# bytedance/DeepSolid

Measured on AMD Instinct MI355X. Metric: local-energy evals/sec, higher is better.
Workload: dtype f64; 1 GPU; bcc_li 24 e- (12,12), total_energy primal (E_kin forward-Laplacian + Ewald), default detnet ((256,32),)*3, 8 dets; batch_per_gpu=4096, global_batch=4096, parallelism=walker-dp1

## Files before the change

deepsolid_amd/_lib.py:

```python
import ctypes as C
import os

_HERE = os.path.dirname(os.path.abspath(__file__))
LIB_PATH = os.environ.get('DEEPSOLID_HIP_LIB') or os.path.join(_HERE, 'libdeepsolid_hip.so')

DS_MAX_LAYERS = 8
DS_MAX_SYM = 6
_PD = C.POINTER(C.c_double)


class SystemDesc(C.Structure):
    _fields_ = [
        ('dtype', C.c_int32), ('n_up', C.c_int32), ('n_dn', C.c_int32), ('n_atoms_prim', C.c_int32),
        ('prim_atoms', _PD), ('prim_a', C.c_double * 9), ('sim_a', C.c_double * 9), ('n_sym', C.c_int32),
        ('prim_AV', C.c_double * (DS_MAX_SYM * 3)), ('prim_BV', C.c_double * (DS_MAX_SYM * 3)),
        ('sim_AV', C.c_double * (DS_MAX_SYM * 3)), ('sim_BV', C.c_double * (DS_MAX_SYM * 3)),
        ('n_layers', C.c_int32), ('hidden_single', C.c_int32 * DS_MAX_LAYERS),
        ('hidden_double', C.c_int32 * DS_MAX_LAYERS), ('n_det', C.c_int32), ('distance_type', C.c_int32),
        ('envelope_type', C.c_int32), ('full_det', C.c_int32), ('use_last_layer', C.c_int32),
        ('bias_orbitals', C.c_int32), ('klist_up', _PD), ('klist_dn', _PD),
        ('n_atoms_sim', C.c_int32), ('sim_atoms', _PD), ('sim_charges', _PD), ('dist_mode', C.c_int32),
        ('n_g', C.c_int32), ('gpoints', _PD), ('gweight', _PD), ('ion_exp_re', _PD), ('ion_exp_im', _PD),
        ('ewald_alpha', C.c_double), ('ee_const', C.c_double), ('ei_const', C.c_double), ('ii_total', C.c_double),
    ]


class ParamBlock(C.Structure):
    _fields_ = [('offset', C.c_int64), ('rows', C.c_int32), ('cols', C.c_int32)]


class KfacBlock(C.Structure):
    _fields_ = [('kind', C.c_int32), ('index', C.c_int32), ('n_param_blocks', C.c_int32), ('param_blocks', C.c_int32 * 3),
                ('has_bias', C.c_int32), ('d_in', C.c_int32), ('d_out', C.c_int32), ('repeats', C.c_int32),
                ('a_offset', C.c_int64), ('g_offset', C.c_int64)]


class HfDesc(C.Structure):
    _PI = C.POINTER(C.c_int32)
    _fields_ = [
        ('a', C.c_double * 9), ('n_atoms', C.c_int32), ('atoms', _PD), ('n_shells', C.c_int32), ('shell_atom', _PI),
        ('shell_l', _PI), ('shell_nprim', _PI), ('exps', _PD), ('coefs', _PD), ('n_k', C.c_int32), ('kpts', _PD),
        ('n_images', C.c_int32), ('images', _PD), ('n_up', C.c_int32), ('n_dn', C.c_int32), ('nocc_up', _PI), ('nocc_dn', _PI),
        ('mo_up', _PD), ('mo_dn', _PD),
    ]


class EcpDesc(C.Structure):
    _PI = C.POINTER(C.c_int32)
    _fields_ = [
        ('a', C.c_double * 9), ('n_atoms', C.c_int32), ('atoms', _PD), ('atom_species', _PI), ('n_species', C.c_int32),
        ('n_l', _PI), ('r_cut_loc', _PD), ('r_cut_nl', _PD), ('term_offset', _PI), ('term_n', _PI), ('term_zeta', _PD),
        ('term_c', _PD), ('n_quad', C.c_int32),
    ]


_VP = C.c_void_p
SIGNATURES = {
    'ds_device_widths': (C.c_int, [C.POINTER(C.c_int32), C.POINTER(C.c_int32), C.c_int32, C.c_int32, C.c_int32, C.c_int32,
                                   C.POINTER(C.c_int32), C.POINTER(C.c_int32), C.POINTER(C.c_int32), C.POINTER(C.c_int32)]),
    'ds_system_create': (C.c_int, [C.POINTER(SystemDesc), C.POINTER(_VP)]),
    'ds_system_destroy': (None, [_VP]),
    'ds_last_error': (C.c_char_p, []),
    'ds_param_count': (C.c_int64, [_VP]),
    'ds_int8_layers': (C.c_int, [_VP]),
    'ds_param_layout': (C.c_int, [_VP, C.POINTER(ParamBlock), C.c_int]),
    'ds_workspace_bytes': (C.c_int64, [_VP, C.c_int64]),
    'ds_logpsi': (C.c_int, [_VP, _VP, _VP, C.c_int64, _VP, _VP, _VP, C.c_int64, _VP]),
    'ds_logpsi_grad': (C.c_int, [_VP, _VP, _VP, C.c_int64, _VP, _VP, _VP, _VP, C.c_int64, _VP]),
    'ds_vjp_workspace_bytes': (C.c_int64, [_VP, C.c_int64]),
    'ds_logpsi_vjp': (C.c_int, [_VP, _VP, _VP, C.c_int64, _VP, _VP, _VP, _VP, _VP, C.c_int64, _VP]),
    'ds_pretrain_workspace_bytes': (C.c_int64, [_VP, C.c_int64]),
    'ds_pretrain_loss_vjp': (C.c_int, [_VP, _VP, _VP, C.c_int64, _VP, _VP, _VP, _VP, _VP, C.c_int64, _VP]),
    'ds_kfac_block_count': (C.c_int, [_VP]),
    'ds_kfac_layout': (C.c_int, [_VP, C.POINTER(KfacBlock), C.c_int]),
    'ds_kfac_workspace_bytes': (C.c_int64, [_VP, C.c_int64]),
    'ds_kfac_factors': (C.c_int, [_VP, _VP, _VP, C.c_int64, _VP, _VP, _VP, C.c_int64, _VP]),
    'ds_kfac_step_workspace_bytes': (C.c_int64, [_VP]),
    'ds_kfac_inverses': (C.c_int, [_VP, _VP, C.c_double, C.c_double, _VP, _VP, C.c_int64, _VP]),
    'ds_kfac_precondition': (C.c_int, [_VP, _VP, _VP, _VP, _VP, _VP, C.c_int64, _VP]),
    'ds_kfac_inverses_sized_workspace_bytes': (C.c_int64, [C.c_int, C.POINTER(C.c_int32), C.POINTER(C.c_int32)]),
    'ds_kfac_inverses_sized': (C.c_int, [C.c_int, C.c_int, C.POINTER(C.c_int32), C.POINTER(C.c_int32), C.POINTER(C.c_int32), _VP,
                                        C.c_double, C.c_double, _VP, _VP, C.c_int64, _VP]),
    'ds_orbitals': (C.c_int, [_VP, _VP, _VP, C.c_int64, _VP, _VP, _VP, C.c_int64, _VP]),
    'ds_ewald': (C.c_int, [_VP, _VP, C.c_int64, _VP, _VP]),
    'ds_local_energy': (C.c_int, [_VP, _VP, _VP, C.c_int64, _VP, _VP, _VP, _VP, _VP, C.c_int64, _VP]),
    'ds_enforce_pbc': (C.c_int, [_PD, C.c_int, _VP, C.c_int64, _VP, _VP, _VP]),
    'ds_observables_workspace_bytes': (C.c_int64, [C.c_int64, C.c_int]),
    'ds_observables': (C.c_int, [_PD, C.c_int, _VP, C.c_int64, C.c_int64, C.POINTER(C.c_int32), C.c_int, C.c_int, _VP, _VP,
                                 C.c_int64, _VP]),
    'ds_realspace_counts': (C.c_int, [_PD, C.POINTER(C.c_int32), _PD, _PD, C.c_double, C.c_int, C.c_int, _VP, C.c_int64, C.c_int64,
                                      C.c_int64, _VP, _VP, _VP]),
    'ds_mh_propose': (C.c_int, [_VP, _VP, _VP, C.c_double, C.c_int64, _VP, _VP]),
    'ds_mh_accept': (C.c_int, [_VP, _VP, _VP, _VP, _VP, _VP, C.c_int64, _VP, _VP]),
    'ds_mh_propose_ex': (C.c_int, [_VP, C.c_int, _VP, _VP, C.c_double, _VP, C.c_int, C.c_int64, _VP, _VP, _VP]),
    'ds_mh_accept_ex': (C.c_int, [_VP, C.c_int, _VP, _VP, _VP, _VP, _VP, _VP, C.c_double, _VP, _VP, C.c_int, C.c_int64, _VP, _VP, _VP]),
    'ds_mcmc_workspace_bytes': (C.c_int64, [_VP, C.c_int64]),
    'ds_mcmc_step': (C.c_int, [_VP, _VP, _VP, _VP, C.c_int64, C.c_int, C.c_double, C.c_uint64, C.c_uint64, _VP, _VP, C.c_int, _VP, _VP,
                              C.c_int64, _VP]),
    'ds_mcmc_step_one_electron': (C.c_int, [_VP, _VP, _VP, _VP, C.c_int64, C.c_int, C.c_int, C.c_double, C.c_uint64, C.c_uint64, _VP, _VP,
                                           C.c_int, _VP, _VP, C.c_int64, _VP]),
    'ds_mcmc_step_importance': (C.c_int, [_VP, _VP, _VP, _VP, C.c_int64, C.c_int, C.c_double, C.c_uint64, C.c_uint64, _VP, _VP, C.c_int,
                                         _VP, _VP, C.c_int64, _VP]),
    'ds_mcmc_step_asymmetric': (C.c_int, [_VP, _VP, _VP, _VP, C.c_int64, C.c_int, C.c_double, _VP, C.c_int, C.c_uint64, C.c_uint64, _VP, _VP,
                                         C.c_int, _VP, _VP, C.c_int64, _VP]),
    'ds_one_body_workspace_bytes': (C.c_int64, [_VP, C.c_int64, C.c_int]),
    'ds_one_body_ratios': (C.c_int, [_VP, _VP, _VP, C.c_int64, C.c_int, C.c_int, C.c_uint64, C.c_uint64, _VP, _VP, C.c_int, _VP, _VP, _VP,
                                     _VP, _VP, C.c_int64, _VP]),
    'ds_spin_exchange_workspace_bytes': (C.c_int64, [_VP, C.c_int64, C.c_int]),
    'ds_spin_exchange_ratios': (C.c_int, [_VP, _VP, _VP, C.c_int64, C.c_int, C.c_int, _VP, _VP, _VP, _VP, _VP, C.c_int64, _VP]),
    'ds_ecp_create': (C.c_int, [C.POINTER(EcpDesc), C.POINTER(_VP)]),
    'ds_ecp_destroy': (None, [_VP]),
    'ds_ecp_workspace_bytes': (C.c_int64, [_VP, _VP, C.c_int64, C.c_int64]),
    'ds_ecp_energy': (C.c_int, [_VP, _VP, _VP, _VP, C.c_int64, C.c_uint64, C.c_uint64, _VP, C.c_int64, _VP, _VP, _VP, _VP, _VP,
                               C.c_int64, _VP]),
    'ds_dmc_workspace_bytes': (C.c_int64, [_VP, C.c_int64]),
    'ds_dmc_step': (C.c_int, [_VP, _VP, _VP, _VP, _VP, _VP, _VP, _VP, C.c_int64, C.c_int, C.c_double, C.c_double, C.c_double, C.c_double,
                             C.c_double, C.c_int, C.c_int, C.c_uint64, C.c_uint64, _VP, _VP, _VP, C.c_int, _VP, _VP, _VP, C.c_int64, _VP]),
    'ds_dmc_noise': (C.c_int, [C.c_int, C.c_int, C.c_int64, C.c_int, C.c_uint64, C.c_uint64, _VP, _VP, _VP, _VP]),
    'ds_dmc_branch_workspace_bytes':(C.c_int64, [C.c_int, C.c_int, C.c_int64]),
    'ds_dmc_branch': (C.c_int, [C.c_int, C.c_int, C.c_int64, C.c_double, _VP, _VP, _VP, _VP, _VP, _VP, _VP, _VP, C.c_int64, _VP]),
    'ds_philox_host': (None,[C.c_uint64, C.c_uint64, C.c_uint64, C.c_uint64, C.c_int, C.POINTER(C.c_uint32)]),
    'ds_energy_stats': (C.c_int, [_VP, _VP, _VP, C.c_int64, _VP, _VP]),
    'ds_debug_stage': (C.c_int64, [_VP, _VP, _VP, C.c_int64, C.c_char_p, _VP, C.c_int64, _VP, C.c_int64, _VP]),
    'ds_profile_enable': (C.c_int, [_VP, C.c_int]),
    'ds_profile_read': (C.c_int, [_VP, C.POINTER(C.c_double), C.POINTER(C.c_int64)]),
    'ds_profile_read_clock': (C.c_int, [_VP, C.POINTER(C.c_double), C.POINTER(C.c_double)]),
    'ds_debug_timeline': (C.c_int, [_VP, C.POINTER(C.c_uint64), C.c_int]),
    'ds_calib_copy': (C.c_int, [_VP, _VP, C.c_int64, _VP]),
    'ds_mfma_f64_peak': (C.c_int64, [C.c_int64, C.c_int, C.c_int, _VP, _VP]),
    'ds_hf_create': (C.c_int, [C.POINTER(HfDesc), C.POINTER(_VP)]),
    'ds_hf_destroy': (None, [_VP]),
    'ds_hf_orbitals': (C.c_int, [_VP, C.c_int, _VP, C.c_int64, _VP, _VP, _VP]),
}

PROF_KINDS = ('features', 'm2_expand', 'two_layer', 'single_first', 'single_hidden', 'orbital', 'det_inverse',
              'det_trace', 'combine', 'ewald', 'shared_term', 'single_lr')

_lib = None


def load():
    global _lib
    if _lib is not None:
        return _lib
    if not os.path.exists(LIB_PATH):
        raise RuntimeError(
            f'{LIB_PATH} is missing: the HIP extension is not built and deepsolid_amd has no CPU '
            'fallback.  Run `make -C deepsolid_amd/csrc` (hipcc, --offload-arch=gfx950).')
    lib = C.CDLL(LIB_PATH)
    for name, (res, args) in SIGNATURES.items():
        fn = getattr(lib, name)
        fn.restype = res
        fn.argtypes = args
    _lib = lib
    return lib


def check(rc, what):
    if rc != 0:
        msg = load().ds_last_error()
        raise RuntimeError(f'{what} failed: {msg.decode() if msg else rc}')
```

deepsolid_amd/csrc/ds_api.hip:

```cpp
#include <cstdarg>

#include "ds_host.h"
#include "ds_tiles.h"

namespace ds {
#define DS_DECL(p) const TileOps<double>* tile_ops_f64_p##p(int); const TileOps<float>* tile_ops_f32_p##p(int);
DS_DECL(0) DS_DECL(1) DS_DECL(2) DS_DECL(3) DS_DECL(4)
#undef DS_DECL
template <> const TileOps<double>* tile_ops<double>(int st) {
    const TileOps<double>* (*parts[])(int) = {tile_ops_f64_p0, tile_ops_f64_p1, tile_ops_f64_p2, tile_ops_f64_p3, tile_ops_f64_p4};
    for (auto f : parts)
        if (const TileOps<double>* o = f(st)) return o;
    return nullptr;
}
template <> const TileOps<float>* tile_ops<float>(int st) {
    const TileOps<float>* (*parts[])(int) = {tile_ops_f32_p0, tile_ops_f32_p1, tile_ops_f32_p2, tile_ops_f32_p3, tile_ops_f32_p4};
    for (auto f : parts)
        if (const TileOps<float>* o = f(st)) return o;
    return nullptr;
}
}

namespace ds {
namespace host {
// ... 186 lines not shown
    for (int c = 0; c < 2; ++c) {
        const size_t n = c < S.n_detch ? S.det_n[c] : 0;
        v.mout_off[c] = mo;
        mo += (size_t)S.K * n * n * 2 * PV;
    }
    v.MOUT = mo; v.MINV = 0; v.TR = 0;
    v.DETS = w.DETS * PV;
    v.PARTM = (size_t)(PV / 5) * h2max * 5 * (S.NP / 16) * ds::PM_SLOTS;
    v.per_walker = measure([&](Arena<double>& a) { carve_value<double>(s, a, 1); });
}

int plan_widths(const int32_t* hs, const int32_t* hd, int n_layers, int n_in_single, int n_in_double, int n_double, int32_t* ps,
                int32_t* pd, int32_t* rs, int32_t* rd) {
    if (n_layers < 1 || n_layers > DS_MAX_LAYERS) return fail("bad n_layers");
    for (int l = 0; l < n_layers; ++l) {
        const int a = hs[l], b = hd[l];
        if (a < 1 || a > 1024) return fail("hidden_single: one-electron widths are supported in 1..1024 (layer %d: %d)", l, a);
        if (l < n_double && (b < 1 || b > 32)) return fail("hidden_double: pair-stream widths are supported in 1..32 (layer %d: %d)", l, b);
        ps[l] = rup(a, 64);
        pd[l] = (b >= 1 && b <= 16) ? 16 : 32;
        rs[l] = a == (l == 0 ? n_in_single : hs[l - 1]);
        rd[l] = l < n_double && b == (l == 0 ? n_in_double : hd[l - 1]);
    }
    return 0;
}

int check_arch(const ds_system_desc* d) {
    if (d->dtype != 0 && d->dtype != 1) return fail("dtype must be 0 (f64) or 1 (f32)");
    if (d->distance_type != 0 && d->distance_type != 1) return fail("Unrecognized distance function.");
    if (d->distance_type == 1 && d->envelope_type != 0) return fail("the 'tri' features support the isotropic envelope only");
    if (d->envelope_type < 0 || d->envelope_type > 2) return fail("unknown envelope_type");
    if (d->n_up < 0 || d->n_dn < 0) return fail("n_up and n_dn must be >= 0");
    if (d->n_up < 1) return fail("internal: n_up must be >= 1 here (ds_system_create swaps a spin-down-only cell)");
    if (d->n_layers < 1 || d->n_layers > DS_MAX_LAYERS) return fail("bad n_layers");
    if (d->n_det < 1 || d->n_det > DS_MAX_DETS) return fail("n_det must be in 1..%d", DS_MAX_DETS);
    if (d->n_sym < 3 || d->n_sym > DS_MAX_SYM) return fail("bad n_sym");
    const int N = d->n_up + d->n_dn, tiles = (3 * N + 2 + 15) / 16, nmat = d->full_det ? N : std::max(d->n_up, d->n_dn);
    if (nmat > 64) return fail("determinant matrices larger than 64 x 64 are not supported (n = %d): the trace kernels keep a matrix row per lane group", nmat);
    if (tiles < 1 || tiles > ds::DS_MAX_TILES)
        return fail("no kernel instance for %d jet-slot tiles (N = %d electrons): supported are N <= 128 (64 with full_det)", tiles, N);
    const int n_double = d->use_last_layer ? d->n_layers : d->n_layers - 1;
    const int nch = d->n_dn > 0 ? 2 : 1;
    for (int l = 0; l < d->n_layers; ++l) {
        if (d->hidden_single[l] % 64 || d->hidden_single[l] < 64 || d->hidden_single[l] > 1024)
            return fail("internal: device width %d of layer %d is not a multiple of 64 in 64..1024", d->hidden_single[l], l);
        if (l < n_double && d->hidden_double[l] != 16 && d->hidden_double[l] != 32)
            return fail("internal: device pair width %d of layer %d is not 16 or 32", d->hidden_double[l], l);
    }
    const int k_orb = d->hidden_single[d->n_layers - 1] + (d->use_last_layer ? nch * d->hidden_double[d->n_layers - 1] : 0);
    if (k_orb % 16) return fail("orbital head with K = %d input rows: the GEMM's operand ring needs K %% 16 == 0", k_orb);
    return 0;
}

template <typename T>
void enforce_pbc(const double* latvec, const double* inv, const void* x, int64_t n_elec, void* out_x, void* out_wrap, hipStream_t st) {
    ds::Lattice<T> L;
    for (int i = 0; i < 9; ++i) { L.a[i] = (T)latvec[i]; L.ainv[i] = (T)inv[i]; }
    hipLaunchKernelGGL((ds::k_enforce_pbc<T>), dim3((unsigned)((n_elec + 255) / 256)), dim3(256), 0, st, L, (const T*)x, (size_t)n_elec, (T*)out_x,
                       (T*)out_wrap);
}

}

void set_last_error(const char* msg) { host::g_err = msg; }

}

using namespace ds::host;

extern "C" {

const char* ds_last_error(void) { return g_err.c_str(); }

int ds_device_widths(const int32_t* hidden_single, const int32_t* hidden_double, int32_t n_layers, int32_t n_in_single, int32_t n_in_double,
                     int32_t n_double, int32_t* dev_single, int32_t* dev_double, int32_t* res_single, int32_t* res_double) {
    if (!hidden_single || !hidden_double || !dev_single || !dev_double || !res_single || !res_double) return fail("null argument");
    return plan_widths(hidden_single, hidden_double, n_layers, n_in_single, n_in_double, n_double, dev_single, dev_double, res_single, res_double);
}

int ds_system_create(const ds_system_desc* ref_desc, ds_system** out) {
    if (!ref_desc || !out) return fail("null argument");
    ds_system_desc dev_desc = *ref_desc;
    int32_t rs[DS_MAX_LAYERS] = {0}, rd[DS_MAX_LAYERS] = {0};
    {
        if (ref_desc->distance_type != 0 && ref_desc->distance_type != 1) return fail("Unrecognized distance function.");
        if (ref_desc->n_layers < 1 || ref_desc->n_layers > DS_MAX_LAYERS) return fail("bad n_layers");
        const int nf = ref_desc->distance_type == 0 ? 4 : 7;
        const int n_double = ref_desc->use_last_layer ? ref_desc->n_layers : ref_desc->n_layers - 1;
        if (int rc = plan_widths(ref_desc->hidden_single, ref_desc->hidden_double, ref_desc->n_layers, nf * ref_desc->n_atoms_prim, nf, n_double,
                                 dev_desc.hidden_single, dev_desc.hidden_double, rs, rd))
            return rc;
    }
    if (dev_desc.n_up == 0 && dev_desc.n_dn > 0) {
        dev_desc.n_up = dev_desc.n_dn;
        dev_desc.n_dn = 0;
        dev_desc.klist_up = dev_desc.klist_dn;
        dev_desc.klist_dn = nullptr;
    }
    if (dev_desc.n_up + dev_desc.n_dn < 1) return fail("n_up + n_dn must be >= 1");
    const ds_system_desc* desc = &dev_desc;
    if (int rc = check_arch(desc)) return rc;
    if (!desc->prim_atoms || !desc->klist_up || (desc->n_dn > 0 && !desc->klist_dn) || !desc->sim_atoms || !desc->sim_charges ||
        (desc->n_g > 0 && (!desc->gpoints || !desc->gweight || !desc->ion_exp_re || !desc->ion_exp_im)))
        return fail("null array pointer in ds_system_desc");
    ds_system* s = new ds_system();
    s->d = *desc;
    for (int l = 0; l < desc->n_layers; ++l) {
        s->ref_single[l] = ref_desc->hidden_single[l];
        s->ref_double[l] = ref_desc->hidden_double[l];
        s->res1[l] = rs[l] != 0;
        s->res2[l] = rd[l] != 0;
    }
    s->dtype = desc->dtype;
    s->use_last = desc->use_last_layer != 0;
    std::vector<double> h64;
    std::vector<float> h32;
    fill_tables<double>(s, desc, s->sd, h64);
    fill_tables<float>(s, desc, s->sf, h32);
    if (hipMalloc(&s->blob64, h64.size() * sizeof(double)) != hipSuccess || hipMalloc(&s->blob32, h32.size() * sizeof(float)) != hipSuccess) {
        delete s;
        return fail("hipMalloc of the system tables failed (is a GPU visible?)");
    }
    if (hipMemcpy(s->blob64, h64.data(), h64.size() * sizeof(double), hipMemcpyHostToDevice) != hipSuccess ||
        hipMemcpy(s->blob32, h32.data(), h32.size() * sizeof(float), hipMemcpyHostToDevice) != hipSuccess) {
        ds_system_destroy(s);
        return fail("upload of the system tables failed");
    }
    relocate<double>(s->sd, (const double*)s->blob64);
    relocate<float>(s->sf, (const float*)s->blob32);
    build_layouts(s);
    {
        int h1max = 0;
        for (int l = 0; l <= s->sd.n_layers; ++l) h1max = std::max(h1max, s->sd.h1[l]);
        if (hipMalloc(&s->lr_w0t, (size_t)h1max * 64 * sizeof(double)) != hipSuccess) {
            ds_system_destroy(s);
            return fail("hipMalloc of the low-rank layer's weight table failed");
        }
    }
    {
        hipDeviceProp_t prop;
        int devid = 0;
        if (hipGetDevice(&devid) == hipSuccess && hipGetDeviceProperties(&prop, devid) == hipSuccess && prop.multiProcessorCount > 0)
            s->n_cu = prop.multiProcessorCount;
    }
    if (hipMalloc((void**)&s->clk_dev, 1024 * sizeof(unsigned long long)) != hipSuccess ||
        hipMemset(s->clk_dev, 0, 1024 * sizeof(unsigned long long)) != hipSuccess) {
        ds_system_destroy(s);
        return fail("hipMalloc of the clock-probe counters failed");
    }
    s->det_valu = getenv("DS_DET_VALU") != nullptr;
    if (const char* e = getenv("DS_VAL_NB")) { const int v = atoi(e); s->val_nb = (v == 1 || v == 2 || v == 4) ? v : 0; }
    s->no_lu_wave = getenv("DS_NO_LU_WAVE") != nullptr;
    s->use_lr = getenv("DS_NO_LOWRANK") == nullptr;
    s->use_pm_skip = getenv("DS_NO_PM_SKIP") == nullptr;
    s->use_pair_expand = getenv("DS_NO_PAIR_EXPAND") == nullptr;
    s->use_g4 = getenv("DS_NO_G4") == nullptr;
    s->use_i8 = getenv("DS_I8") != nullptr && getenv("DS_NO_I8") == nullptr;
    s->use_ldsb = getenv("DS_NO_LDSB") == nullptr;
    s->use_pair_fuse = getenv("DS_NO_PAIR_FUSE") == nullptr;
    s->use_i8_val = getenv("DS_NO_I8_VAL") == nullptr;
    for (int l = 0; l < DS_MAX_LAYERS; ++l) s->i8_prepped[l] = ~(uint64_t)0;
    if (const char* e = getenv("DS_I8_VAL_MIN_TILES")) s->val_i8_min_tiles = atoll(e);
    if (const char* e = getenv("DS_DBG")) s->dbg = atoi(e);
    s->use_wide = getenv("DS_NO_WIDE") == nullptr;
    s->wide_all = getenv("DS_WIDE_ALL") != nullptr;
    {
        const size_t bytes = i8_planes_bytes(s);
        if (bytes && hipMalloc(&s->i8_wp, bytes) != hipSuccess) {
            ds_system_destroy(s);
            return fail("hipMalloc of the int8 layer's weight planes failed");
        }
    }
    if (const char* e = getenv("DS_CHUNK_WALKERS")) s->chunk_cap = std::min<int64_t>(65535, std::max<int64_t>(1, atol(e)));
    *out = s;
    return 0;
}

void ds_system_destroy(ds_system* s) {
    if (!s) return;
    if (s->clk_dev) (void)hipFree(s->clk_dev);
    if (s->lr_w0t) (void)hipFree(s->lr_w0t);
    if (s->i8_wp) (void)hipFree(s->i8_wp);
    if (s->blob64) (void)hipFree(s->blob64);
    if (s->blob32) (void)hipFree(s->blob32);
    delete s;
}

int64_t ds_param_count(const ds_system* s) { return s ? s->nparams : -1; }

int ds_param_layout(const ds_system* s, ds_param_block* blocks, int max_blocks) {
    if (!s) return -1;
    const int n = (int)s->blocks.size();
    for (int i = 0; i < n && i < max_blocks; ++i) blocks[i] = s->blocks[i];
    return n;
}

int64_t ds_workspace_bytes(const ds_system* s, int64_t B) {
    if (!s) return -1;
    const int64_t esz = s->dtype == 0 ? 8 : 4;
    const int64_t budget = workspace_budget();
    const int64_t cap = s->chunk_cap;
    int64_t chunk = std::min<int64_t>(std::max<int64_t>(B, 1), cap);
    chunk = std::max<int64_t>(1, std::min<int64_t>(chunk, budget / ((int64_t)s->ws.per_walker * esz)));
    const int64_t groups = groups_per_pass(B, esz, PassSize{0, s->wsv.per_walker}, budget);
    return std::max((int64_t)s->ws.per_walker * esz * chunk, (int64_t)s->wsv.per_walker * esz * groups) + 256;
}

int ds_enforce_pbc(const double* latvec, int dtype, const void* x, int64_t n_elec, void* out_x, void* out_wrap, void* stream) {
    if (!latvec || !x || !out_x) return fail("null argument");
    if (n_elec <= 0) return 0;
    hipStream_t st = (hipStream_t)stream;
    double inv[9];
    inv3(latvec, inv);
    if (dtype != 0 && dtype != 1) return fail("dtype must be 0 or 1");
    DS_BY_DTYPE(dtype, enforce_pbc, latvec, inv, x, n_elec, out_x, out_wrap, st);
    HIP_OK(hipGetLastError());
    return 0;
}

int ds_profile_enable(ds_system* s, int on) {
    if (!s) return fail("null argument");
    for (auto& v : s->prof_ev) {
        for (auto& p : v) { s->prof_pool.push_back(p.first); s->prof_pool.push_back(p.second); }
        v.clear();
    }
    s->prof_on = on != 0;
    s->prof_only = on >= 2 ? on - 2 : -1;
    if (on) HIP_OK(hipMemset(s->clk_dev, 0, 1024 * sizeof(unsigned long long)));
    return 0;
}

int ds_debug_timeline(ds_system* s, uint64_t* out, int n) {
    if (!s || !out || n < 0 || n > 1022) return fail("bad argument");
    HIP_OK(hipDeviceSynchronize());
    HIP_OK(hipMemcpy(out, s->clk_dev + 2, (size_t)n * sizeof(uint64_t), hipMemcpyDeviceToHost));
    return 0;
}

int ds_profile_read_clock(ds_system* s, double* shader_cycles, double* ref_ticks) {
    if (!s || !shader_cycles || !ref_ticks) return fail("null argument");
    unsigned long long h[2] = {0, 0};
    HIP_OK(hipDeviceSynchronize());
    HIP_OK(hipMemcpy(h, s->clk_dev, sizeof h, hipMemcpyDeviceToHost));
    *shader_cycles = (double)h[0];
    *ref_ticks = (double)h[1];
    return 0;
}

int ds_profile_read(ds_system* s, double* ms_total, int64_t* launches) {
    if (!s || !ms_total || !launches) return fail("null argument");
    if (s->prof_failed) { s->prof_failed = false; return fail("profiling: a HIP event could not be created or recorded; the timings are incomplete"); }
    for (int k = 0; k < DS_PROF_KINDS; ++k) {
        double tot = 0;
        for (auto& p : s->prof_ev[k]) {
            HIP_OK(hipEventSynchronize(p.second));
            float ms = 0;
            HIP_OK(hipEventElapsedTime(&ms, p.first, p.second));
            tot += ms;
        }
        ms_total[k] = tot;
        launches[k] = (int64_t)s->prof_ev[k].size();
    }
    return 0;
}

int ds_calib_copy(const void* src, void* dst, int64_t n_elems, void* stream) {
    if (!src || !dst) return fail("null argument");
    hipLaunchKernelGGL(ds::k_calib_copy, dim3(256 * 8), dim3(256), 0, (hipStream_t)stream, (const double*)src, (double*)dst, (size_t)n_elems);
    HIP_OK(hipGetLastError());
    return 0;
}

int64_t ds_mfma_f64_peak(int64_t iters, int blocks_per_cu, int n_acc, void* scratch, void* stream) {
    const int blocks = 256 * blocks_per_cu;
    hipStream_t st = (hipStream_t)stream;
    switch (n_acc) {
        case 1: hipLaunchKernelGGL(ds::k_mfma_peak<1>, dim3(blocks), dim3(256), 0, st, (long)iters, (double*)scratch); break;
        case 2: hipLaunchKernelGGL(ds::k_mfma_peak<2>, dim3(blocks), dim3(256), 0, st, (long)iters, (double*)scratch); break;
        case 4: hipLaunchKernelGGL(ds::k_mfma_peak<4>, dim3(blocks), dim3(256), 0, st, (long)iters, (double*)scratch); break;
        case 8: hipLaunchKernelGGL(ds::k_mfma_peak<8>, dim3(blocks), dim3(256), 0, st, (long)iters, (double*)scratch); break;
        case 16: hipLaunchKernelGGL(ds::k_mfma_peak<16>, dim3(blocks), dim3(256), 0, st, (long)iters, (double*)scratch); break;
        default: fail("n_acc must be 1, 2, 4, 8 or 16"); return -1;
    }
    return (int64_t)blocks * 4 * iters * n_acc * 2048;
}

}
```

deepsolid_amd/csrc/ds_chain.hip:

```cpp
#include "ds_host.h"
#include "ds_tiles.h"

namespace ds {
namespace host {

template <typename T> inline unsigned m2_split(int K2, int N) {
    unsigned z = 1;
    while (z < 8 && K2 % (2 * z) == 0 && (size_t)(K2 / z) * 5 * N * sizeof(T) > 8192) z *= 2;
    return z;
}

enum Stop { STOP_NONE = 0, STOP_G0, STOP_G1, STOP_G2, STOP_G3, STOP_H2_0, STOP_H2_1, STOP_H2_2, STOP_MEAN0, STOP_Q,
            STOP_MOUT, STOP_MINV, STOP_DETS, STOP_TR };

template <typename T> struct DumpReq { int stop; T* out; int64_t cap; int64_t written; };

template <typename T>
int copy_out(DumpReq<T>* dr, const T* src, size_t n, hipStream_t st) {
    size_t m = std::min<size_t>(n, (size_t)dr->cap);
    HIP_OK(hipMemcpyAsync(dr->out, src, m * sizeof(T), hipMemcpyDeviceToDevice, st));
    dr->written = (int64_t)m;
    return 0;
}

enum class LayerKind {
    Dense,
    DenseRes,
    L0Stats,
    L0Epi9Means,
    LowRank1,
    Int8
};
struct PairPlan {
    bool res, res_sep;
    bool expand;
    bool write_out;
    unsigned xz; int EW, NW; size_t xlds;
};
struct LayerPlan {
    LayerKind kind;
    bool res_sep;
    bool wide;
    bool pm_mask;
    bool pm_unwritten;
    int prof_kind;
    PairPlan pair;
};
enum class OrbKind { Orb3, Wide, Ldsb, Gemm };
template <typename T> struct ChainPlan {
    const ds::TileOps<T>* to;
    bool lr_on;
    int lr_nc;
    int g4;
    LayerPlan layer[DS_MAX_LAYERS];
    OrbKind orb[2];
    int count(LayerKind k, int n_layers) const {
        int n = 0;
        for (int l = 0; l < n_layers; ++l) n += layer[l].kind == k ? 1 : 0;
        return n;
    }
};

template <typename T>
int plan_chain(const ds_system* s, bool dump, ChainPlan<T>* p) {
    const ds::SysDev<double>& S = s->sd;
    const ds::TileOps<T>* to = p->to = ds::tile_ops<T>(S.P / 16);
    if (!to) return fail("no kernel instance for %d slot tiles (N = %d electrons)", S.P / 16, S.N);
    const int ST = to->ST;
    const bool wide = s->use_wide && to->gemm_wide != nullptr;
    auto gemm_wide = [&](int epi) { return wide && (s->wide_all || ds::gemm_wide_faster<T>(epi)); };
    const int K0loc = S.h1[0] + S.nch * S.h2[0], K0sh = S.nch * S.h1[0];
    p->lr_nc = std::max(2, (K0loc + K0sh + 4 + 15) / 16);
    p->lr_on = !dump && s->use_lr && S.n_layers >= 2 && !s->res1[0] && p->lr_nc <= 4 && S.h1[1] % 16 == 0 && (S.nch * S.h2[1]) % 4 == 0 &&
               3 * (K0loc + K0sh + 4) <= S.h1[1] && p->lr_nc * S.h1[1] < (S.h1[1] - K0loc - K0sh - 4) * ST;
    const int used = S.D - 16 * (ST - 1);
    p->g4 = !s->use_g4 ? 0 : (ST == 5 && used > 8 && used <= 12) ? 3 : (ST == 10 && used <= 4) ? 1 : 0;
    for (int l = 0; l < S.n_layers; ++l) {
        const int Kh = S.h1[l], K2 = S.h2[l], Nout = S.h1[l + 1], Kloc = Kh + S.nch * K2;
        LayerPlan& lp = p->layer[l];
        lp = LayerPlan{};
        if (Nout % 64 || Nout > 1024) return fail("hidden_single must be a multiple of 64 and <= 1024 (got %d)", Nout);
        if (l < S.n_double) {
            PairPlan& pp = lp.pair;
            const int K2o = S.h2[l + 1];
            if (K2o != 32 && K2o != 16) return fail("hidden_double must be 16 or 32 (got %d)", K2o);
            if (K2 % 4) return fail("pair-stream width %d is not a multiple of 4", K2);
            pp.res_sep = s->res2[l] && l == 0;
            pp.res = s->res2[l] && !pp.res_sep;
            pp.xz = (!pp.res && K2o == 32) ? 2 : 1;
            pp.write_out = l + 1 < S.n_double || s->use_last;
            pp.EW = (pp.write_out && S.N % 16 == 8 && pp.xz == 2) ? 2 : 1;
            pp.NW = (pp.EW * S.N + 15) / 16;
            pp.xlds = ((size_t)(K2o / pp.xz) * 5 * pp.EW * S.N + (size_t)pp.EW * S.nch * (K2o / pp.xz) * 5) * sizeof(T);
            pp.expand = !dump && s->use_pair_expand && !pp.res_sep && l + 1 < S.n_layers && pp.NW <= 8 && pp.xlds <= 150 * 1024;
        }
        const bool res = s->res1[l];
        lp.res_sep = res && l == 0 && (Kloc % 16 != 0 || S.nf * S.A != Nout);
        if (res && !lp.res_sep && Kloc % 16) return fail("residual layer with K = %d: the GEMM's operand ring needs K %% 16 == 0", Kloc);
        if (p->lr_on && l == 1) {
            lp.kind = LayerKind::LowRank1;
            lp.wide = wide && (s->wide_all || ds::lr_wide_faster<T>(p->lr_nc));
        } else if (p->lr_on && l == 0) {
            const bool one_kernel = to->layer0_stats && ds::layer0_stats_instance(ST, K0loc / 4);
            lp.kind = one_kernel ? LayerKind::L0Stats : LayerKind::L0Epi9Means;
            lp.wide = !one_kernel && gemm_wide(9);
        } else if (int8_energy_layer(s, l)) {
            lp.kind = LayerKind::Int8;
        } else if (res && !lp.res_sep) {
            lp.kind = LayerKind::DenseRes;
            lp.wide = gemm_wide(2);
        } else {
            lp.kind = LayerKind::Dense;
            lp.wide = gemm_wide(1);
        }
        lp.prof_kind = l == 0 ? DS_PROF_SINGLE_FIRST : (lp.kind == LayerKind::LowRank1 ? DS_PROF_SINGLE_LR : DS_PROF_SINGLE_HIDDEN);
        lp.pm_mask = s->use_pm_skip && (l == 0 || (lp.kind == LayerKind::DenseRes && Kh % 16 == 0 && K2 % 16 == 0));
        lp.pm_unwritten = !dump && l >= 1 && !lp.wide &&
                          (lp.kind == LayerKind::LowRank1 ? s->use_pm_skip : (lp.pm_mask && ds::pm_instance<T>(ST)));
    }
    const int Korb = S.h1[S.n_layers] + (s->use_last ? S.nch * S.h2[S.n_layers] : 0);
    if (Korb % 16) return fail("orbital head with K = %d: the GEMM's operand ring needs K %% 16 == 0", Korb);
    for (int sp = 0; sp < S.nch; ++sp) {
        const int OC = S.ocols[sp];
        if (to->gemm_orb3 && OC % 256 != 0 && OC % 192 == 0) p->orb[sp] = OrbKind::Orb3;
        else if (gemm_wide(5)) p->orb[sp] = OrbKind::Wide;
        else if (to->orbital_lb && s->use_ldsb && OC % 64 == 0) p->orb[sp] = OrbKind::Ldsb;
        else p->orb[sp] = OrbKind::Gemm;
    }
    return 0;
}

template <typename T>
int run_chain(ds_system* s, const T* params, const T* x, int64_t Bc, Arena<T> ws, hipStream_t st, T* out_ke, T* out_logabs,
              T* out_phase, DumpReq<T>* dr, T* out_grad = nullptr) {
    const ds::SysDev<T>& S = dev<T>(s);
    const WsLayout& L = s->ws;
    const Carve<T> c = carve<T>(s, ws, Bc);
    if (!ws.ok) return carve_fail("forward-Laplacian chain");
    auto blk = [&](int i) { return params + s->blocks[i].offset; };
    const int stop = dr ? dr->stop : STOP_NONE;
    ChainPlan<T> plan;
    if (int rc = plan_chain<T>(s, dr != nullptr, &plan)) return rc;
    const ds::TileOps<T>* to = plan.to;
    const int NB = to->NB, ST = to->ST, lr_nc = plan.lr_nc;
    const bool lr_on = plan.lr_on;
    const int K0loc = S.h1[0] + S.nch * S.h2[0], K0sh = S.nch * S.h1[0];
    {
        ProfScope ps(s, DS_PROF_FEATURES, st);
        size_t sh = (size_t)(9 * S.N) * sizeof(T) + (size_t)S.N * S.A * S.nf * sizeof(ds::Jet5<T>);
        hipLaunchKernelGGL((ds::k_features<T>), dim3((unsigned)Bc), dim3(256), sh, st, S, x, blk(s->i_pi[0]), blk(s->i_sg[0]),
                           blk(s->i_pi[S.nch - 1]), blk(s->i_sg[S.nch - 1]), lr_on ? c.XL : c.G[0], lr_on ? K0loc : S.ldk, c.MEAN[0], c.H2[0], c.Q);
    }
    if (lr_on) {
        const int n = S.h1[1] * 16 * lr_nc;
        hipLaunchKernelGGL((ds::k_lr_w0t<T>), dim3((unsigned)((n + 255) / 256)), dim3(256), 0, st, blk(s->i_wloc[0]), blk(s->i_wsh[0]), K0loc, K0sh,
                           S.h1[1], 16 * lr_nc, (T*)s->lr_w0t);
    }
    if (stop == STOP_MEAN0) return copy_out(dr, c.MEAN[0], (size_t)S.nch * S.h1[0] * S.P * Bc, st);
    if (stop == STOP_H2_0) return copy_out(dr, c.H2[0], (size_t)S.h2[0] * 5 * S.NP * Bc, st);
    if (stop == STOP_Q) return copy_out(dr, c.Q, L.Q * Bc, st);
    int gi = 0, hi = 0;
    for (int l = 0; l < S.n_layers; ++l) {
        const LayerPlan& lp = plan.layer[l];
        const int Kh = S.h1[l], K2 = S.h2[l], Nout = S.h1[l + 1];
        if (!(l > 0 && plan.layer[l - 1].pair.expand)) {
            ProfScope ps(s, DS_PROF_M2_EXPAND, st);
            const bool xl = lr_on && l == 0;
            hipLaunchKernelGGL((ds::k_m2_expand<T>), dim3(S.N, (unsigned)Bc, m2_split<T>(K2, S.N)), dim3(256), (size_t)(K2 * 5 * S.N + S.nch * K2 * 5) / m2_split<T>(K2, S.N) * sizeof(T), st, S,
                               c.H2[hi], K2, xl ? c.XL : c.G[gi], Kh, xl ? K0loc : S.ldk, lp.pm_unwritten ? 1 : 0);
        }
        if (stop == STOP_G0 + l) return copy_out(dr, c.G[gi], L.G * Bc, st);
        if (l < S.n_double) {
            const PairPlan& pp = lp.pair;
            const int K2o = S.h2[l + 1];
            const T* W2 = blk(s->i_w2[l]); const T* b2 = blk(s->i_b2[l]);
            ProfScope ps(s, DS_PROF_TWO_LAYER, st);
            if (pp.expand) {
#define DS_TWOX(NT2, RES) hipLaunchKernelGGL((ds::k_two_layer_expand<T, NT2, RES>), dim3(S.N / pp.EW, (unsigned)Bc, pp.xz), dim3(64 * pp.NW), pp.xlds, st, S, c.H2[hi], K2, W2, b2, \
                                             pp.write_out ? c.H2[hi ^ 1] : (T*)nullptr, c.G[gi ^ 1], S.h1[l + 1], S.ldk, plan.layer[l + 1].pm_unwritten ? 1 : 0, pp.EW)
                if (K2o == 32 && pp.res) DS_TWOX(2, true);
                else if (pp.res) DS_TWOX(1, true);
                else DS_TWOX(1, false);
#undef DS_TWOX
            } else {
                const dim3 grid((S.NP / 16 + 3) / 4, (unsigned)Bc);
#define DS_TWO(NT2, RES) hipLaunchKernelGGL((ds::k_two_layer<T, NT2, RES, false>), grid, dim3(256), 0, st, S, c.H2[hi], K2, W2, b2, c.H2[hi ^ 1])
                if (K2o == 32) { if (pp.res) DS_TWO(2, true); else DS_TWO(2, false); }
                else { if (pp.res) DS_TWO(1, true); else DS_TWO(1, false); }
#undef DS_TWO
            }
            if (pp.res_sep)
                launch_pair_res_add<T>(dim3((unsigned)(((size_t)K2o * 5 * S.NP + 255) / 256), (unsigned)Bc), st, c.H2[hi], K2, c.H2[hi ^ 1], K2o, S.nf, S.NP);
        }
        const int Kloc = Kh + S.nch * K2, Ksh = S.nch * Kh;
        {
            dim3 block; unsigned gz;
            gemm_geom(Nout, NB, &block, &gz, ST);
            dim3 wblock; unsigned wgz;
            gemm_geom(Nout, 4, &wblock, &wgz, 6);
            const size_t gws = (size_t)S.N * S.ldk * S.P, gts = (size_t)S.ldk * S.P;
            const bool lr1 = lp.kind == LayerKind::LowRank1;
            T* Sl = lr1 ? c.ZB + (size_t)Bc * S.h1[1] * S.P : c.ZB;
            {
                ProfScope ps(s, DS_PROF_SHARED_TERM, st);
                if (l == 0 || lr1) {
                    const ds::GemmArgs<T> ga{nullptr, 0, 0, nullptr, 0, l == 0 ? c.MEAN[0] : c.MEAN[1], (size_t)Ksh * S.P, blk(s->i_wsh[l]), Ksh, 0,
                                             Sl, (size_t)Nout * S.P, 0, Nout, S.P, nullptr, blk(s->i_b[l]), ds::OrbEpi<T>{}};
                    to->gemm(6, dim3(1, (unsigned)Bc, gz), block, st, ga);
                } else {
                    dim3 sblock; unsigned sgz;
                    gemm_geom(Nout, NB, &sblock, &sgz);
                    if (ST > 10 && sblock.x > 512) { sblock = dim3(512); sgz = (unsigned)((Nout / (16 * NB) + 7) / 8); }
                    to->shared_term(dim3(1, (unsigned)Bc, sgz), sblock, 2 * 16 * S.P * sizeof(T), st, S, c.G[gi], blk(s->i_wsh[l]), Kh, Sl, Nout, S.P,
                                    blk(s->i_b[l]), 0);
                }
            }
            ProfScope ps(s, lp.prof_kind, st);
            const T* Xin = (lr_on && l == 0) ? c.XL : c.G[gi];
            const size_t xws = (lr_on && l == 0) ? (size_t)S.N * K0loc * S.P : gws, xts = (lr_on && l == 0) ? (size_t)K0loc * S.P : gts;
            const dim3 lgrid(S.N * gz, (unsigned)Bc, 1), wgrid(S.N * wgz, (unsigned)Bc, 1);
            auto layer_gemm = [&](int epi, const ds::GemmArgs<T>& g) {
                if (lp.wide) to->gemm_wide(epi, wgrid, wblock, st, g); else to->gemm(epi, lgrid, block, st, g);
            };
            ds::GemmArgs<T> ga{Xin, xws, xts, blk(s->i_wloc[l]), Kloc, nullptr, 0, nullptr, 0, S.N, c.G[gi ^ 1], gws, gts, Nout, S.P, c.ZB, blk(s->i_b[l]),
                               ds::OrbEpi<T>{}};
            if (lp.pm_mask) { ga.oe.pm_k0 = Kh / 4; ga.oe.pm_ks = K2 / 4; ga.oe.pm_nup = S.n_up; ga.oe.pm_nch = S.nch; }
            switch (lp.kind) {
            case LayerKind::LowRank1: {
                const ds::LrArgs<T> la{c.XL, (size_t)S.N * K0loc * S.P, (size_t)K0loc * S.P, c.MEAN[0], (size_t)K0sh * S.P, K0loc, K0sh,
                                       (const T*)s->lr_w0t, c.G[gi], gws, gts, blk(s->i_wloc[l]), Kh, S.nch * K2, c.G[gi ^ 1], gws, gts, Sl,
                                       Nout, S.P, S.N, c.YO, L.YO, blk(s->i_wloc[0]), c.ZB, s->dbg >> 8, S.n_up, S.nch};
                if (lp.wide) to->layer1_lr_wide(lr_nc, s->res1[l], wgrid, wblock, st, la); else to->layer1_lr(lr_nc, s->res1[l], lgrid, block, st, la);
                break;
            }
            case LayerKind::L0Stats:
                to->layer0_stats(K0loc / 4, dim3(S.nch * (unsigned)((Nout + 63) / 64), (unsigned)Bc), st, S, c.XL, (size_t)S.N * K0loc * S.P,
                                 (size_t)K0loc * S.P, blk(s->i_wloc[0]), c.ZB, Nout, S.P, c.YO, c.MEAN[1]);
                break;
            case LayerKind::L0Epi9Means: {
                ga.Z = c.YO; ga.zws = L.YO; ga.zts = (size_t)2 * Nout;
                layer_gemm(9, ga);
                constexpr int STC = 5;
                const unsigned nfb = (unsigned)((Nout + 63) / 64), nck = (unsigned)((S.P / 16 + STC - 1) / STC);
                hipLaunchKernelGGL((ds::k_layer0_means<T, STC>), dim3(S.nch * nfb * nck, (unsigned)Bc), dim3(256), 0, st, S, c.XL,
                                   (size_t)S.N * K0loc * S.P, (size_t)K0loc * S.P, blk(s->i_wloc[0]), K0loc, c.ZB, Nout, S.P, c.YO, c.MEAN[1]);
                break;
            }
            case LayerKind::Int8: {
                launch_layer_i8(s, l, false, (const double*)blk(s->i_wloc[l]), Kloc, Nout, (const double*)c.G[gi], gts, (const double*)Sl,
                                (double*)c.G[gi ^ 1], (int)(Bc * S.N), st);
                break;
            }
            case LayerKind::DenseRes:
                ga.oe.dbg = s->dbg & 3;
                ga.oe.g4 = plan.g4;
                if (l > 0 && s->prof_on && (s->prof_only < 0 || s->prof_only == DS_PROF_SINGLE_HIDDEN)) { ga.oe.clk = s->clk_dev; ga.oe.dbg = s->dbg; }
                layer_gemm(2, ga);
                break;
            case LayerKind::Dense:
                layer_gemm(1, ga);
                if (lp.res_sep)
                    launch_layer_res_add<T>(dim3(S.N, (unsigned)Bc), st, Xin, xws, xts, c.G[gi ^ 1], gws, gts, S.nf * S.A, Nout, S.P);
                break;
            }
        }
        gi ^= 1;
        if (l < S.n_double) {
            hi ^= 1;
            if (stop == STOP_H2_1 + l) return copy_out(dr, c.H2[hi], (size_t)S.h2[l + 1] * 5 * S.NP * Bc, st);
        }
    }
    if (stop == STOP_G0 + S.n_layers) return copy_out(dr, c.G[gi], L.G * Bc, st);
    const int Kl = S.h1[S.n_layers], K2l = S.h2[S.n_layers];
    if (s->use_last) {
        ProfScope ps(s, DS_PROF_M2_EXPAND, st);
        hipLaunchKernelGGL((ds::k_m2_expand<T>), dim3(S.N, (unsigned)Bc, m2_split<T>(K2l, S.N)), dim3(256), (size_t)(K2l * 5 * S.N + S.nch * K2l * 5) / m2_split<T>(K2l, S.N) * sizeof(T), st, S,
                           c.H2[hi], K2l, c.G[gi], Kl, S.ldk, 0);
    }
    for (int sp = 0; sp < S.nch; ++sp) {
        const int ns = sp == 0 ? S.n_up : S.n_dn, i0 = sp == 0 ? 0 : S.n_up, OC = S.ocols[sp];
        const int Korb = Kl + (s->use_last ? S.nch * K2l : 0);
        dim3 block; unsigned gz;
        gemm_geom(OC, NB, &block, &gz, ST);
        if (s->use_last) {
            ProfScope ps(s, DS_PROF_SHARED_TERM, st);
            to->shared_term(dim3(1, (unsigned)Bc, gz), block, 2 * 16 * S.P * sizeof(T), st, S, c.G[gi], blk(s->i_wsh_orb[sp]), Kl, c.ZB, OC, S.P,
                            (const T*)nullptr, 0);
        }
        ProfScope ps(s, DS_PROF_ORBITAL, st);
        const int ch = S.mat_ch[sp];
        ds::OrbEpi<T> oe{c.Q, c.MOUT, L.MOUT, L.mout_off[ch], S.N, i0, S.nparam[sp], S.nparam_max, S.norb[sp], S.det_n[ch],
                         S.row_off[sp], S.bias_orb ? blk(s->i_borb[sp]) : (const T*)nullptr, nullptr};
        oe.g4 = plan.g4;
        const ds::GemmArgs<T> ga{c.G[gi] + (size_t)i0 * S.ldk * S.P, (size_t)S.N * S.ldk * S.P, (size_t)S.ldk * S.P, blk(s->i_worb[sp]), Korb,
                                 nullptr, 0, nullptr, 0, ns, nullptr, 0, 0, OC, S.P, s->use_last ? (const T*)c.ZB : (const T*)nullptr, nullptr, oe};
        dim3 ob; unsigned oz;
        switch (plan.orb[sp]) {
        case OrbKind::Orb3:
            gemm_geom(OC, 3, &ob, &oz);
            to->gemm_orb3(dim3(ns * oz, (unsigned)Bc, 1), ob, st, ga);
            break;
        case OrbKind::Wide:
            gemm_geom(OC, 4, &ob, &oz, 6);
            to->gemm_wide(5, dim3(ns * oz, (unsigned)Bc, 1), ob, st, ga);
            break;
        case OrbKind::Ldsb:
            to->orbital_lb(dim3(ns * (unsigned)(OC / 64), (unsigned)Bc, 1), st, ga);
            break;
        case OrbKind::Gemm:
            to->gemm(5, dim3(ns * gz, (unsigned)Bc, 1), block, st, ga);
            break;
        }
    }
    if (stop == STOP_MOUT) return copy_out(dr, c.MOUT, L.MOUT * Bc, st);
    for (int ch = 0; ch < S.n_detch; ++ch) {
        ProfScope ps(s, DS_PROF_DET_INVERSE, st);
        launch_det_inverse<T>(s, S, c, ch, Bc, st);
    }
    if (stop == STOP_MINV) return copy_out(dr, c.MINV, L.MINV * Bc, st);
    for (int ch = 0; ch < S.n_detch; ++ch) {
        ProfScope ps(s, DS_PROF_DET_TRACE, st);
        if (int rc = launch_det_trace<T>(s, S, c, ch, Bc, st)) return rc;
    }
    if (stop == STOP_DETS) return copy_out(dr, c.DETS, L.DETS * Bc, st);
    if (stop == STOP_TR) return copy_out(dr, c.TR, L.TR * Bc, st);
    {
        ProfScope ps(s, DS_PROF_COMBINE, st);
        hipLaunchKernelGGL((ds::k_combine<T>), dim3((unsigned)Bc), dim3(64), 0, st, S, c.TR, L.TR, L.tr_off[1], c.DETS, L.DETS,
                           L.dets_off[1], out_ke, out_logabs, out_phase, out_grad);
    }
    HIP_OK(hipGetLastError());
    return 0;
}

template <typename T>
int local_energy_impl(ds_system* s, const void* params, const void* x, int64_t B, void* out_ke, void* out_ewald, void* out_logabs,
                      void* out_phase, void* ws, int64_t ws_bytes, hipStream_t st) {
    const ds::SysDev<T>& S = dev<T>(s);
    int64_t chunk = ws_bytes / (int64_t)(s->ws.per_walker * sizeof(T));
    if (chunk < 1) return fail("workspace too small: %lld bytes < %zu per walker", (long long)ws_bytes, s->ws.per_walker * sizeof(T));
    chunk = std::min<int64_t>(chunk, 65535);
    for (int64_t b0 = 0; b0 < B; b0 += chunk) {
        const int64_t Bc = std::min(chunk, B - b0);
        const T* xb = (const T*)x + b0 * 3 * S.N;
        int rc = run_chain<T>(s, (const T*)params, xb, Bc, arena_of<T>(ws, ws_bytes), st, out_ke ? (T*)out_ke + 2 * b0 : nullptr,
                              out_logabs ? (T*)out_logabs + b0 : nullptr, out_phase ? (T*)out_phase + 2 * b0 : nullptr, nullptr);
        if (rc) return rc;
    }
    if (out_ewald) {
        T* tmp = (T*)ws;
        for (int64_t b0 = 0; b0 < B; b0 += chunk) {
            const int64_t Bc = std::min(chunk, B - b0);
            size_t sh = ds::ewald_lds_bytes(S);
            ProfScope ps(s, DS_PROF_EWALD, st);
            hipLaunchKernelGGL((ds::k_ewald<T>), dim3((unsigned)Bc), dim3(256), sh, st, S, (const T*)x + b0 * 3 * S.N, tmp);
            hipLaunchKernelGGL((ds::k_sum3<T>), dim3((unsigned)((Bc + 255) / 256)), dim3(256), 0, st, tmp, Bc, (T*)out_ewald + b0);
        }
    }
    HIP_OK(hipGetLastError());
    return 0;
}

template <typename T>
int logpsi_grad_impl(ds_system* s, const void* params, const void* x, int64_t B, void* out_logabs, void* out_phase, void* out_grad,
                     void* ws, int64_t ws_bytes, hipStream_t st) {
    const ds::SysDev<T>& S = dev<T>(s);
    const int64_t chunk = std::min<int64_t>(ws_bytes / (int64_t)(s->ws.per_walker * sizeof(T)), 65535);
    if (chunk < 1) return fail("workspace too small");
    for (int64_t b0 = 0; b0 < B; b0 += chunk) {
        const int64_t Bc = std::min(chunk, B - b0);
        int rc = run_chain<T>(s, (const T*)params, (const T*)x + b0 * 3 * S.N, Bc, arena_of<T>(ws, ws_bytes), st, nullptr, out_logabs ? (T*)out_logabs + b0 : nullptr,
                              out_phase ? (T*)out_phase + 2 * b0 : nullptr, nullptr, (T*)out_grad + b0 * 3 * S.N * 2);
        if (rc) return rc;
    }
    return 0;
}
template <typename T>
int energy_grad_impl(ds_system* s, const void* params, const void* x, int64_t B, void* out_ke, void* out_ew3, void* out_logabs,
                     void* out_phase, void* out_grad, void* ws, int64_t ws_bytes, hipStream_t st) {
    const ds::SysDev<T>& S = dev<T>(s);
    const int64_t chunk = std::min<int64_t>(ws_bytes / (int64_t)(s->ws.per_walker * sizeof(T)), 65535);
    if (chunk < 1) return fail("workspace too small: %lld bytes < %zu per walker", (long long)ws_bytes, s->ws.per_walker * sizeof(T));
    for (int64_t b0 = 0; b0 < B; b0 += chunk) {
        const int64_t Bc = std::min(chunk, B - b0);
        int rc = run_chain<T>(s, (const T*)params, (const T*)x + b0 * 3 * S.N, Bc, arena_of<T>(ws, ws_bytes), st, (T*)out_ke + 2 * b0,
                              (T*)out_logabs + b0, (T*)out_phase + 2 * b0, nullptr, (T*)out_grad + b0 * 3 * S.N * 2);
        if (rc) return rc;
    }
    {
        ProfScope ps(s, DS_PROF_EWALD, st);
        hipLaunchKernelGGL((ds::k_ewald<T>), dim3((unsigned)B), dim3(256), ds::ewald_lds_bytes(S), st, S, (const T*)x, (T*)out_ew3);
    }
    HIP_OK(hipGetLastError());
    return 0;
}
int energy_grad_forward(ds_system* s, const void* params, const void* x, int64_t B, void* out_ke, void* out_ew3, void* out_logabs,
                        void* out_phase, void* out_grad, void* ws, int64_t ws_bytes, hipStream_t st) {
    return DS_BY_DTYPE(s->dtype, energy_grad_impl, s, params, x, B, out_ke, out_ew3, out_logabs, out_phase, out_grad, ws, ws_bytes, st);
}

template <typename T> void ewald_triple(ds_system* s, const void* x, int64_t B, void* out, hipStream_t st) {
    const ds::SysDev<T>& S = dev<T>(s);
    size_t sh = ds::ewald_lds_bytes(S);
    hipLaunchKernelGGL((ds::k_ewald<T>), dim3((unsigned)B), dim3(256), sh, st, S, (const T*)x, (T*)out);
}

template <typename T>
int64_t debug_stage_impl(ds_system* s, const void* params, const void* x, int64_t B, int stop, void* out, int64_t out_elems, void* ws,
                         int64_t ws_bytes, hipStream_t st) {
    DumpReq<T> dr{stop, (T*)out, out_elems, 0};
    const int rc = run_chain<T>(s, (const T*)params, (const T*)x, B, arena_of<T>(ws, ws_bytes), st, nullptr, nullptr, nullptr, &dr);
    return rc ? -1 : dr.written;
}

int logpsi_grad_forward(ds_system* s, const void* params, const void* x, int64_t B, void* out_logabs, void* out_phase, void* out_grad,
                        void* ws, int64_t ws_bytes, hipStream_t st) {
    return DS_BY_DTYPE(s->dtype, logpsi_grad_impl, s, params, x, B, out_logabs, out_phase, out_grad, ws, ws_bytes, st);
}

int int8_energy_layers(const ds_system* s, bool dump) {
    ChainPlan<double> plan;
    return plan_chain<double>(s, dump, &plan) == 0 ? plan.count(LayerKind::Int8, s->sd.n_layers) : 0;
}

template <typename T> void launch_pair_res_add(dim3 grid, hipStream_t st, const T* Hin, int Kin, T* Hout, int Kout, int n_res, int NP) {
    hipLaunchKernelGGL((ds::k_pair_res_add<T>), grid, dim3(256), 0, st, Hin, Kin, Hout, Kout, n_res, NP);
}

template <typename T>
void launch_layer_res_add(dim3 grid, hipStream_t st, const T* Xin, size_t x_ws, size_t x_ts, T* Gout, size_t g_ws, size_t g_ts, int n_res,
                          int Nout, int P) {
    hipLaunchKernelGGL((ds::k_layer_res_add<T>), grid, dim3(256), 0, st, Xin, x_ws, x_ts, Gout, g_ws, g_ts, n_res, Nout, P);
}

#define DS_INST(T)                                                                                      \
    template void launch_pair_res_add<T>(dim3, hipStream_t, const T*, int, T*, int, int, int);          \
    template void launch_layer_res_add<T>(dim3, hipStream_t, const T*, size_t, size_t, T*, size_t, size_t, int, int, int);
DS_INST(double) DS_INST(float)
#undef DS_INST

}
}

using namespace ds::host;

extern "C" {

int ds_int8_layers(const ds_system* s) {
    if (!s) return -1;
    return int8_energy_layers(s, false);
}

int ds_local_energy(ds_system* s, const void* params, const void* x, int64_t B, void* out_ke, void* out_ewald, void* out_logabs,
                    void* out_phase, void* ws, int64_t ws_bytes, void* stream) {
    if (s) ++s->call_seq;
    if (!s || !params || !x || !ws) return fail("null argument");
    if (B <= 0) return 0;
    hipStream_t st = (hipStream_t)stream;
    return DS_BY_DTYPE(s->dtype, local_energy_impl, s, params, x, B, out_ke, out_ewald, out_logabs, out_phase, ws, ws_bytes, st);
}

int ds_logpsi_grad(ds_system* s, const void* params, const void* x, int64_t B, void* out_logabs, void* out_phase, void* out_grad,
                   void* ws, int64_t ws_bytes, void* stream) {
    if (s) ++s->call_seq;
    if (!s || !params || !x || !ws || !out_grad) return fail("null argument");
    if (B <= 0) return 0;
    hipStream_t st = (hipStream_t)stream;
    return logpsi_grad_forward(s, params, x, B, out_logabs, out_phase, out_grad, ws, ws_bytes, st);
}

int ds_ewald(ds_system* s, const void* x, int64_t B, void* out, void* stream) {
    if (!s || !x || !out) return fail("null argument");
    if (B <= 0) return 0;
    hipStream_t st = (hipStream_t)stream;
    DS_BY_DTYPE(s->dtype, ewald_triple, s, x, B, out, st);
    HIP_OK(hipGetLastError());
    return 0;
}

int64_t ds_debug_stage(ds_system* s, const void* params, const void* x, int64_t B, const char* stage, void* out, int64_t out_elems,
                       void* ws, int64_t ws_bytes, void* stream) {
    if (s) ++s->call_seq;
    if (!s || !params || !x || !stage || !out || !ws) { fail("null argument"); return -1; }
    static const struct { const char* name; int stop; } names[] = {
        {"g0", STOP_G0}, {"g1", STOP_G1}, {"g2", STOP_G2}, {"g3", STOP_G3}, {"h2_0", STOP_H2_0}, {"h2_1", STOP_H2_1},
        {"h2_2", STOP_H2_2}, {"mean0", STOP_MEAN0}, {"q", STOP_Q}, {"mout", STOP_MOUT},
        {"minv", STOP_MINV}, {"dets", STOP_DETS}, {"tr", STOP_TR}};
    int stop = -1;
    for (auto& n : names)
        if (!strcmp(n.name, stage)) stop = n.stop;
    if (stop < 0) { fail("unknown stage '%s'", stage); return -1; }
    hipStream_t st = (hipStream_t)stream;
    const int64_t esz = s->dtype == 0 ? 8 : 4;
    const int64_t chunk = ws_bytes / (int64_t)(s->ws.per_walker * esz);
    if (chunk < B) { fail("debug stage needs the whole batch in one chunk"); return -1; }
    return DS_BY_DTYPE(s->dtype, debug_stage_impl, s, params, x, B, stop, out, out_elems, ws, ws_bytes, st);
}

}
```

deepsolid_amd/csrc/ds_gemm.h:

```cpp
#pragma once
#include <type_traits>

#include "ds_kernels.h"

#ifndef DS_SADD
#define DS_SADD 1
#endif
#ifndef DS_SADD_NSF
#define DS_SADD_NSF 2
#endif

namespace ds {

template <typename T> __device__ __forceinline__ int orb_col(int p, int part) {
    const int t = p >> 3, q = p & 3, r = 2 * ((p >> 2) & 1) + part;
    return 16 * t + acc_row<T>(q << 4, r);
}

template <typename T> struct OrbEpi {
    const T* Q;
    T* MOUT;
    size_t mout_stride, mout_off;
    int N, i0, nparam, nparam_max;
    int norb, n, row0;
// ... 422 lines not shown
        else step(u, k);
    };
    if (gemm_uses_ring(EPI) || ((EPI == 6 || EPI == 7) && (nks & 3) == 0)) {
#pragma unroll
        for (int u = 0; u < NSET; ++u) load_set(u);
        stamp();
        int ks = 0;
        if (NSET == 4) {
            for (; ks + 4 < ((PMASK && pm_k0 < nks) ? pm_k0 + 1 : nks); ks += 4) {
#pragma unroll
                for (int u = 0; u < 4; ++u) { step(u, ks + u); load_set(u); }
            }
            if constexpr (PMASK) {
                for (; ks + 4 < nks; ks += 4) {
                    const unsigned m = tmask[(ks - pm_k0) >= oe.pm_ks ? 1 : 0];
#pragma unroll
                    for (int u = 0; u < 4; ++u) { step_m(u, m); load_set(u); }
                }
            }
            if constexpr (SADD) {
                const T* Sp0 = Sb + (size_t)w * Nout * P + lr;
                auto srow = [&](int q) { return Sp0 + (size_t)(n0 + 16 * (q >> 2) + acc_row<T>(lane, q & 3)) * P; };
                auto lfull = [&](int q) {
                    const T* p = srow(q);
#pragma unroll
                    for (int s = 0; s < ST; ++s) sfull[q][s] = p[16 * s];
                    s0[q] = sfull[q][0];
                };
                const unsigned mlast = (PMASK && pm_k0 < nks) ? pm_mask(ks) : ~0u;
#pragma unroll
                for (int u = 0; u < 4; ++u) {
                    if constexpr (PMASK) step_m(u, mlast); else step(u, ks + u);
#pragma unroll
                    for (int q = 0; q < NB * 4; ++q)
                        if ((q & 3) == u) { if (q < NSF) lfull(q); else s0[q] = srow(q)[0]; }
                }
            } else if constexpr (PMASK) {
                const unsigned m = pm_k0 < nks ? pm_mask(ks) : ~0u;
#pragma unroll
                for (int u = 0; u < 4; ++u) { park(u, ks + u); step_m(u, m); }
            } else {
#pragma unroll
                for (int u = 0; u < 4; ++u) step(u, ks + u);
            }
        } else {
            for (; ks + 2 * NSET <= nks && (!PMASK || ks + NSET <= pm_k0); ks += NSET) {
#pragma unroll
                for (int u = 0; u < NSET; ++u) { step(u, ks + u); load_set(u); }
            }
            if constexpr (PMASK) {
                for (; ks + 2 * NSET <= nks; ks += NSET) {
#pragma unroll
                    for (int u = 0; u < NSET; ++u) { step_g(u, ks + u); load_set(u); }
                }
            }
#pragma unroll
            for (int u = 0; u < NSET; ++u) {
                step_g(u, ks + u);
                if (ks + u + NSET < nks) load_set(u);
            }
            ks += NSET;
#pragma unroll
            for (int u = 0; u < NSET; ++u)
                if (ks + u < nks) step_g(u, ks + u);
        }
    } else {
        if constexpr (PM0) {
            for (int ks = 0; ks < nks; ++ks) { load_set(0); step_m(0, pm_k0 < nks ? (ks < pm_k0 ? own0 : pm_mask(ks)) : ~0u); }
        } else {
            for (int ks = 0; ks < nks; ++ks) { load_set(0); step(0, ks); }
        }
    }
    if constexpr (G4 > 0) {
        if constexpr (GQ_STASH) gq[GQS * (lr >> 2)] = T(0);
#pragma unroll
        for (int a = 0; a < NB; ++a) {
            acc[a][ST - 1][0] = quads_to_tile<G4, 0>(c4[a]);
            acc[a][ST - 1][1] = quads_to_tile<G4, 1>(c4[a]);
            acc[a][ST - 1][2] = quads_to_tile<G4, 2>(c4[a]);
            acc[a][ST - 1][3] = quads_to_tile<G4, 3>(c4[a]);
        }
    }
    stamp();
    if (EPI == 0 || EPI == 6 || EPI == 7) {
        T* Zp = Z + (size_t)w * z_walker_stride + (EPI == 7 ? (size_t)tile * z_tile_stride : (size_t)tile * Nout * P);
#pragma unroll
        for (int a = 0; a < NB; ++a)
#pragma unroll
            for (int r = 0; r < 4; ++r) {
                const int n = n0 + 16 * a + acc_row<T>(lane, r);
                const T bn = EPI == 0 ? T(0) : bias[n];
#pragma unroll
                for (int s = 0; s < ST; ++s)
                    Zp[(size_t)n * P + 16 * s + lr] = acc[a][s][r] + ((EPI == 7 || (EPI == 6 && s == 0 && lr == 0)) ? bn : T(0));
            }
    } else if (EPI == 5) {
        orbital_epilogue<T, NB, ST>(acc, oe, tile, w, n0, lane, Sb, Nout, P);
    } else if (EPI == 8) {
        const int i = oe.i0 + tile;
        T* Mw = oe.MOUT + (size_t)w * oe.mout_stride + oe.mout_off;
#pragma unroll
        for (int a = 0; a < NB; ++a)
#pragma unroll
            for (int ab = 0; ab < 2; ++ab) {
                const int p = 8 * (n0 / 16 + a) + lq + 4 * ab;
                if (p >= oe.nparam) continue;
                const T* q = oe.Q + ((size_t)(w * oe.N + i) * oe.nparam_max + p) * 2 * P + lr;
                T* mo = Mw + (((size_t)((p / oe.norb) * oe.n + oe.row0 + tile) * oe.n + p % oe.norb) * 2) * P + lr;
                const int cr = n0 + 16 * a + acc_row<T>(lane, 2 * ab), ci = n0 + 16 * a + acc_row<T>(lane, 2 * ab + 1);
#pragma unroll
                for (int s = 0; s < ST; ++s) {
                    Cx<T> phi(acc[a][s][2 * ab], acc[a][s][2 * ab + 1]);
                    if (Sb) { phi.re += Sb[((size_t)w * Nout + cr) * P + 16 * s + lr]; phi.im += Sb[((size_t)w * Nout + ci) * P + 16 * s + lr]; }
                    if (oe.bias) { phi.re += oe.bias[p]; phi.im += oe.bias[oe.nparam + p]; }
                    const Cx<T> v = phi * Cx<T>(q[16 * s], q[P + 16 * s]);
                    mo[16 * s] = v.re;
                    mo[P + 16 * s] = v.im;
                }
            }
    } else if (EPI == 2 && DS_EXP(oe.dbg & 1)) {
        T v = 0;
#pragma unroll
        for (int a = 0; a < NB; ++a)
#pragma unroll
            for (int s = 0; s < ST; ++s) v += acc[a][s][0] + acc[a][s][1] + acc[a][s][2] + acc[a][s][3];
        if (v == T(12345.678)) Z[0] = v;
    } else {
        const T* Gi = X + (size_t)w * x_walker_stride + (size_t)tile * x_tile_stride + lr;
        T* Go = Z + (size_t)w * z_walker_stride + (size_t)tile * z_tile_stride + lr;
        if constexpr (SADD) layer_epilogue_sadd<T, NB, ST, NA, NSF>(acc, Gi, Go, stash, n0, lane, P, Sb + (size_t)w * Nout * P + lr, sfull, s0);
        else layer_epilogue<T, NB, ST, EPI, NA>(acc, Gi, Go, stash, n0, lane, P);
    }
    stamp();
    if (EPI == 2 && DS_EXP(oe.clk != nullptr) && wave == 0 && lane == 0) {
        atomicAdd(oe.clk, (unsigned long long)(clock64() - clk_c0));
        atomicAdd(oe.clk + 1, (unsigned long long)(wall_clock64() - clk_r0));
    }
}

template <typename T> struct LrArgs {
    const T* XL; size_t xl_ws, xl_ts;
    const T* M0; size_t m0_ws;
    int K0loc, K0sh;
    const T* W0T;
    const T* G1; size_t g_ws, g_ts;
    const T* W1; int Kh, Km2;
    T* Gout; size_t go_ws, go_ts;
    const T* S1;
    int Nout, P, n_tiles;
    const T* YO; size_t yo_ws;
    const T* W0; const T* S0;
    int dbg;
    int n_up, nch;
};
template <int NB, int NC, int NG = 0> constexpr int lr_ncp() { return 16 * NC + 4 * NG + 1; }
template <typename T, int NB, int NC, int NG = 0> inline size_t lr_lds_bytes(unsigned threads, int Kh) {
    return ((size_t)2 * Kh + (size_t)(threads / 64) * 16 * NB * lr_ncp<NB, NC, NG>()) * sizeof(T);
}

template <typename T, int NB, int ST, int NC, bool RES, int NG = 0>
__global__ void __launch_bounds__((ST > 5 ? 256 : 1024 / NB), (ST <= 10 ? 2 : 1)) k_layer1_lr(LrArgs<T> A) {
    typedef typename Acc4<T>::type acc_t;
    static_assert(NG == 0 || sizeof(T) == 8, "column groups: float64 only");
    constexpr int NCP = lr_ncp<NB, NC, NG>(), LDW = 16 * (NC + (NG > 0 ? 1 : 0));
    int tile = blockIdx.x, w = blockIdx.y;
    if ((gridDim.y & 7) == 0) {
        const unsigned b = blockIdx.y * gridDim.x + blockIdx.x, q = b >> 3;
        w = (q / gridDim.x) * 8 + (b & 7);
        tile = q % gridDim.x;
    }
    const int wave = __builtin_amdgcn_readfirstlane(threadIdx.x >> 6), lane = threadIdx.x & 63;
    int zb = 0;
    if (gridDim.x > (unsigned)A.n_tiles) {
        const int gzf = gridDim.x / A.n_tiles;
        zb = tile % gzf;
        tile /= gzf;
    }
    const int lr = lane & 15, lq = lane >> 4, n0 = (zb * (blockDim.x >> 6) + wave) * 16 * NB;
    const int P = A.P, Nout = A.Nout, Kh = A.Kh, K0 = A.K0loc + A.K0sh;
    extern __shared__ __attribute__((aligned(16))) char lr_smem[];
    T* yl = reinterpret_cast<T*>(lr_smem);
    T* Cl = yl + 2 * Kh + (size_t)wave * (16 * NB * NCP);
    const T* G1t = A.G1 + (size_t)w * A.g_ws + (size_t)tile * A.g_ts;
    {
        typedef T vec2 __attribute__((ext_vector_type(2)));
        const T* yo = A.YO + (size_t)w * A.yo_ws + (size_t)tile * 2 * Kh;
        for (int n = threadIdx.x; n < Kh; n += blockDim.x)
            *reinterpret_cast<vec2*>(yl + 2 * n) = *reinterpret_cast<const vec2*>(yo + 2 * n);
    }
    __syncthreads();
    if (n0 >= Nout) return;
    acc_t c1[NB][NC];
    T c4[NB][NG > 0 ? NG : 1];
#pragma unroll
    for (int a = 0; a < NB; ++a) {
#pragma unroll
        for (int s = 0; s < NC; ++s) c1[a][s] = acc_t{0, 0, 0, 0};
#pragma unroll
        for (int g = 0; g < NG; ++g) c4[a][g] = 0;
    }
    {
        T av[4][NB], wv[4][NC], w4[4][NG > 0 ? NG : 1];
        const T* Wl = A.W1 + n0 + (size_t)lq * Nout + lr;
        const T* Tl = A.W0T + lq * LDW + lr;
        const T* T4 = A.W0T + lq * LDW + 16 * NC + (lr & 3);
        auto load_set = [&](int u) {
#pragma unroll
            for (int a = 0; a < NB; ++a) av[u][a] = Wl[16 * a];
#pragma unroll
            for (int s = 0; s < NC; ++s) wv[u][s] = Tl[16 * s];
#pragma unroll
            for (int g = 0; g < NG; ++g) w4[u][g] = T4[4 * g];
            Wl += (size_t)4 * Nout;
            Tl += 4 * LDW;
            T4 += 4 * LDW;
        };
        auto step = [&](int u, int ks) {
            typedef T vec2 __attribute__((ext_vector_type(2)));
            const vec2 yo = *reinterpret_cast<const vec2*>(yl + 2 * (4 * ks + lq));
            const T y = yo[0], d1 = 1 - y * y;
            T bv[NC];
#pragma unroll
            for (int s = 0; s < NC; ++s) {
                const int c = 16 * s + lr;
                bv[s] = c == K0 ? y : (c == K0 + 1 ? yo[1] : d1 * wv[u][s]);
            }
#pragma unroll
            for (int a = 0; a < NB; ++a)
#pragma unroll
                for (int s = 0; s < NC; ++s) c1[a][s] = mfma16(av[u][a], bv[s], c1[a][s]);
            if constexpr (NG > 0) {
#pragma unroll
                for (int g = 0; g < NG; ++g) {
                    const int c = 16 * NC + 4 * g + (lr & 3);
                    const T b4 = c == K0 ? y : (c == K0 + 1 ? yo[1] : d1 * w4[u][g]);
#pragma unroll
                    for (int a = 0; a < NB; ++a) c4[a][g] = __builtin_amdgcn_mfma_f64_4x4x4f64(av[u][a], b4, c4[a][g], 0, 0, 0);
                }
            }
        };
        const int nks = DS_EXP(A.dbg & 2) ? 4 : Kh / 4;
#pragma unroll
        for (int u = 0; u < 4; ++u) load_set(u);
        int ks = 0;
        for (; ks + 4 < nks; ks += 4) {
#pragma unroll
            for (int u = 0; u < 4; ++u) { step(u, ks + u); load_set(u); }
        }
#pragma unroll
        for (int u = 0; u < 4; ++u) step(u, ks + u);
    }
#pragma unroll
    for (int a = 0; a < NB; ++a)
#pragma unroll
        for (int s = 0; s < NC; ++s)
#pragma unroll
            for (int r = 0; r < 4; ++r) Cl[(16 * a + acc_row<T>(lane, r)) * NCP + 16 * s + lr] = c1[a][s][r];
#pragma unroll
    for (int a = 0; a < NB; ++a)
#pragma unroll
        for (int g = 0; g < NG; ++g) Cl[(16 * a + 4 * ((lane >> 2) & 3) + lq) * NCP + 16 * NC + 4 * g + (lane & 3)] = c4[a][g];
    __builtin_amdgcn_fence(__ATOMIC_ACQ_REL, "wavefront");
    __builtin_amdgcn_wave_barrier();
    acc_t acc[NB][ST];
    if (DS_EXP(A.dbg & 8)) {
#pragma unroll
        for (int a = 0; a < NB; ++a)
#pragma unroll
            for (int s = 0; s < ST; ++s) acc[a][s] = acc_t{0, 0, 0, 0};
    } else {
        const T* Sp0 = A.S1 + (size_t)w * Nout * P + lr;
#pragma unroll
        for (int a = 0; a < NB; ++a)
#pragma unroll
            for (int r = 0; r < 4; ++r) {
                const int n = n0 + 16 * a + acc_row<T>(lane, r);
#pragma unroll
                for (int s = 0; s < ST; ++s) acc[a][s][r] = Sp0[n * P + 16 * s];
            }
    }
    const T* Ca = Cl + lr * NCP + lq;
    {
        constexpr int NSET = ring_sets<T, NB, ST>();
        T av[NSET][NB], bv[NSET][ST];
        const int nm2 = A.Km2 / 4, nl = A.K0loc / 4, nk = DS_EXP(A.dbg & 4) ? 4 : nm2 + K0 / 4;
        const T* Wm = A.W1 + (size_t)(Kh + lq) * Nout + n0 + lr;
        const T* Xm = G1t + (size_t)(Kh + lq) * P + lr;
        const T* Xl = A.XL + (size_t)w * A.xl_ws + (size_t)tile * A.xl_ts + (size_t)lq * P + lr;
        const T* Ml = A.M0 + (size_t)w * A.m0_ws + (size_t)lq * P + lr;
        int kl = 0;
        auto load_set = [&](int u) {
            const int km = kl < nm2 ? kl : nm2 - 1;
            const T* wp = Wm + (size_t)(4 * km) * Nout;
            const T* xp = kl < nm2 ? Xm + (size_t)(4 * kl) * P : (kl - nm2 < nl ? Xl + (size_t)(4 * (kl - nm2)) * P : Ml + (size_t)(4 * (kl - nm2 - nl)) * P);
#pragma unroll
            for (int a = 0; a < NB; ++a) av[u][a] = wp[16 * a];
#pragma unroll
            for (int s = 0; s < ST; ++s) bv[u][s] = xp[16 * s];
            ++kl;
        };
        unsigned tmask[2], lmask[2];
        const unsigned own = (1u << ((2 + 3 * tile) >> 4)) | (1u << ((4 + 3 * tile) >> 4));
        {
            const int n_dn = A.n_tiles - A.n_up;
#pragma unroll
            for (int sp = 0; sp < 2; ++sp) {
                const int j0 = sp == 0 ? 0 : A.n_up, ns = (sp == 0 || A.nch == 1) ? (A.nch == 1 ? A.n_tiles : A.n_up) : n_dn;
                const int lo = (2 + 3 * j0) >> 4, hi = (4 + 3 * (j0 + ns - 1)) >> 4;
                lmask[sp] = own | (((2u << hi) - 1u) & ~((1u << lo) - 1u));
                tmask[sp] = 1u | lmask[sp];
            }
        }
        const int nm2s = A.nch > 1 ? nm2 / 2 : nm2;
        const int h10 = A.K0sh / A.nch / 4, h20 = (nl - h10) / A.nch;
        auto low_mask = [&](int kk) -> unsigned {
            if (kk < h10) return own;
            if (kk < nl) return lmask[(kk - h10) >= h20 ? 1 : 0];
            return lmask[(kk - nl) >= h10 ? 1 : 0];
        };
        auto step = [&](int u, int k) {
            const bool low = k >= nm2;
            const int c = low ? 4 * (k - nm2) : 0;
            const unsigned m = low ? (sizeof(T) == 8 ? low_mask(k - nm2) : ~0u) : tmask[k < nm2s ? 0 : 1];
            T b0 = bv[u][0];
            b0 = (low && lr < 2) ? T(0) : b0;
            T aa[NB];
#pragma unroll
            for (int a = 0; a < NB; ++a) {
                const T cl = Ca[16 * a * NCP + c];
                aa[a] = low ? cl : av[u][a];
            }
#pragma unroll
            for (int s = 0; s < ST; ++s)
                if ((m >> s) & 1) {
#pragma unroll
                    for (int a = 0; a < NB; ++a) acc[a][s] = mfma16(aa[a], s == 0 ? b0 : bv[u][s], acc[a][s]);
                }
        };
#pragma unroll
        for (int u = 0; u < NSET; ++u) load_set(u);
        int ks = 0;
        for (; ks + 2 * NSET <= nk; ks += NSET) {
#pragma unroll
            for (int u = 0; u < NSET; ++u) { step(u, ks + u); load_set(u); }
        }
#pragma unroll
        for (int u = 0; u < NSET; ++u) {
            if (ks + u < nk) step(u, ks + u);
            if (ks + u + NSET < nk) load_set(u);
        }
        ks += NSET;
#pragma unroll
        for (int u = 0; u < NSET; ++u)
            if (ks + u < nk) step(u, ks + u);
        const T one = (lq == 0 && lr == 0) || (lq == 1 && lr == 1) ? T(1) : T(0);
#pragma unroll
        for (int a = 0; a < NB; ++a) acc[a][0] = mfma16(Ca[16 * a * NCP + K0], one, acc[a][0]);
    }
    T* Got = A.Gout + (size_t)w * A.go_ws + (size_t)tile * A.go_ts + lr;
    if (DS_EXP(A.dbg & 1)) {
        T v = 0;
#pragma unroll
        for (int a = 0; a < NB; ++a)
#pragma unroll
            for (int s = 0; s < ST; ++s) v += acc[a][s][0] + acc[a][s][1] + acc[a][s][2] + acc[a][s][3];
        if (v == T(12345.678)) Got[0] = v;
        return;
    }
    if constexpr (RES) {
        const T* Xl = A.XL + (size_t)w * A.xl_ws + (size_t)tile * A.xl_ts + (size_t)lq * P + lr;
        const T* S0p = A.S0 + (size_t)w * Kh * P + lr;
        unsigned rm_sp[2];
        const unsigned rm_own = (1u << ((2 + 3 * tile) >> 4)) | (1u << ((4 + 3 * tile) >> 4));
        {
#pragma unroll
            for (int sp = 0; sp < 2; ++sp) {
                const int j0 = sp == 0 ? 0 : A.n_up, ns = (sp == 0 || A.nch == 1) ? (A.nch == 1 ? A.n_tiles : A.n_up) : A.n_tiles - A.n_up;
                const int lo = (2 + 3 * j0) >> 4, hi = (4 + 3 * (j0 + ns - 1)) >> 4;
                rm_sp[sp] = rm_own | (((2u << hi) - 1u) & ~((1u << lo) - 1u));
            }
        }
        const int rh10 = A.K0sh / A.nch / 4, rh20 = (A.K0loc / 4 - rh10) / A.nch;
        auto rmask = [&](int ks) -> unsigned { return sizeof(T) == 4 ? ~0u : (ks < rh10 ? rm_own : rm_sp[(ks - rh10) >= rh20 ? 1 : 0]); };
        auto rf = [&](int a) {
            const T rs2 = T(0.70710678118654752440);
#pragma unroll
            for (int c0 = 0; c0 < ST; c0 += 5) {
                constexpr int CWMAX = ST < 5 ? ST : 5;
                const int cw = ST - c0 < 5 ? ST - c0 : 5;
                acc_t racc[CWMAX];
#pragma unroll
                for (int rr = 0; rr < 4; ++rr) {
                    const int n = n0 + 16 * a + acc_row<T>(lane, rr);
#pragma unroll
                    for (int s = 0; s < CWMAX; ++s)
                        if (s < cw) racc[s][rr] = S0p[(size_t)n * P + 16 * (c0 + s)];
                }
                for (int ks = 0; ks < A.K0loc / 4; ++ks) {
                    const T av = A.W0[(size_t)(4 * ks + lq) * Kh + n0 + 16 * a + lr];
                    const unsigned mr = rmask(ks) >> c0;
#pragma unroll
                    for (int s = 0; s < CWMAX; ++s)
                        if (s < cw && ((mr >> s) & 1)) racc[s] = mfma16(av, Xl[(size_t)(4 * ks) * P + 16 * (c0 + s)], racc[s]);
                }
#pragma unroll
                for (int r = 0; r < 4; ++r) {
                    const int n = n0 + 16 * a + acc_row<T>(lane, r);
                    typedef T vec2 __attribute__((ext_vector_type(2)));
                    const vec2 yo = *reinterpret_cast<const vec2*>(yl + 2 * n);
                    const T d1 = 1 - yo[0] * yo[0];
#pragma unroll
                    for (int s = 0; s < CWMAX; ++s)
                        if (s < cw) {
                            T hv = d1 * racc[s][r];
                            if (c0 + s == 0) hv = lr == 0 ? yo[0] : (lr == 1 ? yo[1] : hv);
                            __builtin_nontemporal_store((hv + acc[a][c0 + s][r]) * rs2, &Got[(size_t)n * P + 16 * (c0 + s)]);
                        }
                }
            }
        };
        layer_epilogue<T, NB, ST, 2, 0>(acc, (const T*)nullptr, Got, (const T*)nullptr, n0, lane, P, rf);
    } else
        layer_epilogue<T, NB, ST, 1, 0>(acc, (const T*)nullptr, Got, (const T*)nullptr, n0, lane, P);
}

template <typename T, int STC>
__global__ void __launch_bounds__(256, (sizeof(T) == 8 ? 3 : 4))
k_layer0_means(SysDev<T> S, const T* __restrict__ XL, size_t xl_ws, size_t xl_ts, const T* __restrict__ W0, int K0loc,
               const T* __restrict__ S0, int Nout, int P, const T* __restrict__ YO, T* __restrict__ MEAN1) {
    typedef typename Acc4<T>::type acc_t;
    typedef T vec2 __attribute__((ext_vector_type(2)));
    const int ntile = P / 16, nck = (ntile + STC - 1) / STC, nfb = gridDim.x / (S.nch * nck);
    const int chunk = blockIdx.x % nck, fb = (blockIdx.x / nck) % nfb, sp = blockIdx.x / (nck * nfb), w = blockIdx.y;
    const int wave = threadIdx.x >> 6, lane = threadIdx.x & 63, lr = lane & 15, lq = lane >> 4;
    const int n0 = (fb * 4 + wave) * 16, nks = K0loc / 4, t0 = chunk * STC;
    if (n0 >= Nout) return;
    const int i0 = sp == 0 ? 0 : S.n_up, ns = sp == 0 ? S.n_up : S.n_dn;
    const T* W0p = W0 + (size_t)lq * Nout + n0 + lr;
    acc_t s0[STC], macc[STC];
#pragma unroll
    for (int s = 0; s < STC; ++s) {
        const int t = t0 + s < ntile ? t0 + s : ntile - 1;
#pragma unroll
        for (int r = 0; r < 4; ++r) s0[s][r] = S0[(size_t)w * Nout * P + (size_t)(n0 + acc_row<T>(lane, r)) * P + 16 * t + lr];
        macc[s] = acc_t{0, 0, 0, 0};
    }
    const int h10 = S.h1[0] / 4, h20 = S.h2[0] / 4;
    unsigned prange[2];
#pragma unroll
    for (int sp2 = 0; sp2 < 2; ++sp2) {
        const int j0 = sp2 == 0 ? 0 : S.n_up, nsp = sp2 == 0 ? S.n_up : (S.n_dn > 0 ? S.n_dn : S.n_up);
        const int lo = (2 + 3 * j0) >> 4, hi = (4 + 3 * (j0 + nsp - 1)) >> 4;
        prange[sp2] = ((2u << hi) - 1u) & ~((1u << lo) - 1u);
    }
    for (int e = 0; e < ns; ++e) {
        const int i = i0 + e;
        const T* Xl = XL + (size_t)w * xl_ws + (size_t)i * xl_ts + (size_t)lq * P + lr;
        const T* yo = YO + ((size_t)w * S.N + i) * 2 * Nout;
        vec2 yv[4];
#pragma unroll
        for (int r = 0; r < 4; ++r) yv[r] = *reinterpret_cast<const vec2*>(yo + 2 * (n0 + acc_row<T>(lane, r)));
        acc_t acc[STC];
#pragma unroll
        for (int s = 0; s < STC; ++s) acc[s] = s0[s];
        const unsigned own = 1u | (1u << ((2 + 3 * i) >> 4)) | (1u << ((4 + 3 * i) >> 4));
        for (int ks = 0; ks < nks; ++ks) {
            const T wv = W0p[(size_t)(4 * ks) * Nout];
            T xv[STC];
#pragma unroll
            for (int s = 0; s < STC; ++s) xv[s] = Xl[(size_t)(4 * ks) * P + 16 * (t0 + s < ntile ? t0 + s : ntile - 1)];
            const unsigned m = sizeof(T) == 8 ? ((ks < h10 ? own : (own | prange[(ks - h10) >= h20 ? 1 : 0])) >> t0) : ~0u;
#pragma unroll
            for (int s = 0; s < STC; ++s)
                if ((m >> s) & 1) acc[s] = mfma16(wv, xv[s], acc[s]);
        }
#pragma unroll
        for (int r = 0; r < 4; ++r) {
            const T y = yv[r][0], d1 = 1 - y * y;
#pragma unroll
            for (int s = 0; s < STC; ++s) {
                T o = d1 * acc[s][r];
                if (s == 0 && chunk == 0) o = lr == 0 ? y : (lr == 1 ? yv[r][1] : o);
                macc[s][r] += o;
            }
        }
    }
    const T inv = T(1) / T(ns);
    T* Mp = MEAN1 + ((size_t)w * S.nch + sp) * Nout * P + lr;
#pragma unroll
    for (int r = 0; r < 4; ++r) {
        const int n = n0 + acc_row<T>(lane, r);
#pragma unroll
        for (int s = 0; s < STC; ++s)
            if (t0 + s < ntile) Mp[(size_t)n * P + 16 * (t0 + s)] = macc[s][r] * inv;
    }
}

template <typename T, int ST, int NKS>
__global__ void __launch_bounds__(256, 2)
k_layer0_stats(SysDev<T> S, const T* __restrict__ XL, size_t xl_ws, size_t xl_ts, const T* __restrict__ W0,
               const T* __restrict__ S0, int Nout, int P, T* __restrict__ YO, T* __restrict__ MEAN1) {
    typedef typename Acc4<T>::type acc_t;
    const int nfb = gridDim.x / S.nch, sp = blockIdx.x / nfb, fb = blockIdx.x - sp * nfb, w = blockIdx.y;
    const int wave = threadIdx.x >> 6, lane = threadIdx.x & 63, lr = lane & 15, lq = lane >> 4;
    const int n0 = (fb * 4 + wave) * 16;
    if (n0 >= Nout) return;
    const int i0 = sp == 0 ? 0 : S.n_up, ns = sp == 0 ? S.n_up : S.n_dn;
    T wv[NKS];
#pragma unroll
    for (int ks = 0; ks < NKS; ++ks) wv[ks] = W0[(size_t)(4 * ks + lq) * Nout + n0 + lr];
    acc_t s0[ST], macc[ST];
#pragma unroll
    for (int t = 0; t < ST; ++t) {
#pragma unroll
        for (int r = 0; r < 4; ++r) s0[t][r] = S0[(size_t)w * Nout * P + (size_t)(n0 + acc_row<T>(lane, r)) * P + 16 * t + lr];
        macc[t] = acc_t{0, 0, 0, 0};
    }
    const T* Xw = XL + (size_t)w * xl_ws + (size_t)lq * P + lr;
    T xn[NKS][ST];
    auto load_x = [&](int i) {
        const T* Xl = Xw + (size_t)i * xl_ts;
#pragma unroll
        for (int ks = 0; ks < NKS; ++ks)
#pragma unroll
            for (int t = 0; t < ST; ++t) xn[ks][t] = Xl[(size_t)(4 * ks) * P + 16 * t];
    };
    load_x(i0);
    const int h10 = S.h1[0] / 4, h20 = S.h2[0] / 4;
    unsigned prange[2];
#pragma unroll
    for (int sp2 = 0; sp2 < 2; ++sp2) {
        const int j0 = sp2 == 0 ? 0 : S.n_up, nsp = sp2 == 0 ? S.n_up : (S.n_dn > 0 ? S.n_dn : S.n_up);
        const int lo = (2 + 3 * j0) >> 4, hi = (4 + 3 * (j0 + nsp - 1)) >> 4;
        prange[sp2] = ((2u << hi) - 1u) & ~((1u << lo) - 1u);
    }
    for (int e = 0; e < ns; ++e) {
        const int i = i0 + e;
        acc_t acc[ST];
#pragma unroll
        for (int t = 0; t < ST; ++t) acc[t] = s0[t];
        T xc[NKS][ST];
#pragma unroll
        for (int ks = 0; ks < NKS; ++ks)
#pragma unroll
            for (int t = 0; t < ST; ++t) xc[ks][t] = xn[ks][t];
        load_x(i0 + (e + 1 < ns ? e + 1 : e));
        const unsigned own = 1u | (1u << ((2 + 3 * i) >> 4)) | (1u << ((4 + 3 * i) >> 4));
#pragma unroll
        for (int ks = 0; ks < NKS; ++ks) {
            const unsigned m = ks < h10 ? own : (own | prange[(ks - h10) >= h20 ? 1 : 0]);
#pragma unroll
            for (int t = 0; t < ST; ++t)
                if ((m >> t) & 1) acc[t] = mfma16(wv[ks], xc[ks][t], acc[t]);
        }
        T* yo = YO + ((size_t)w * S.N + i) * 2 * Nout;
        T zsel = 0;
#pragma unroll
        for (int r = 0; r < 4; ++r) {
            const T v = row16_bcast<0>(acc[0][r]);
            zsel = lr == r ? v : zsel;
        }
        const T yall = ds_tanh(zsel);
#pragma unroll
        for (int r = 0; r < 4; ++r) {
            const int n = n0 + acc_row<T>(lane, r);
            T ss = 0;
#pragma unroll
            for (int t = 0; t < ST; ++t) ss += (16 * t + lr >= 2) ? acc[t][r] * acc[t][r] : T(0);
            ss = row16_sum(ss);
            const T y = row16_bcast_dyn<4>(yall, r), d1 = 1 - y * y, d2 = -2 * y * d1;
            const T oL = d1 * row16_bcast<1>(acc[0][r]) + d2 * ss;
            if (lr < 2) yo[2 * n + lr] = lr == 0 ? y : oL;
#pragma unroll
            for (int t = 0; t < ST; ++t) {
                T o = d1 * acc[t][r];
                if (t == 0) o = lr == 0 ? y : (lr == 1 ? oL : o);
                macc[t][r] += o;
            }
        }
    }
    const T inv = T(1) / T(ns);
    T* Mp = MEAN1 + ((size_t)w * S.nch + sp) * Nout * P + lr;
#pragma unroll
    for (int r = 0; r < 4; ++r) {
        const int n = n0 + acc_row<T>(lane, r);
#pragma unroll
        for (int t = 0; t < ST; ++t) Mp[(size_t)n * P + 16 * t] = macc[t][r] * inv;
    }
}

template <typename T>
__global__ void k_lr_w0t(const T* __restrict__ Wloc0, const T* __restrict__ Wsh0, int K0loc, int K0sh, int Kh, int NCW, T* __restrict__ W0T) {
    const int idx = blockIdx.x * blockDim.x + threadIdx.x;
    if (idx >= Kh * NCW) return;
    const int n = idx / NCW, c = idx - n * NCW;
    W0T[idx] = c < K0loc ? Wloc0[(size_t)c * Kh + n] : (c < K0loc + K0sh ? Wsh0[(size_t)(c - K0loc) * Kh + n] : T(0));
}

template <typename T, int NB, int ST>
__global__ void __launch_bounds__((ST > 10 ? 512 : 1024 / NB), (NB == 4 ? 2 : 1))
k_shared_term(SysDev<T> S, const T* __restrict__ G, const T* __restrict__ Wsh, int Kh, T* __restrict__ Sb, int Nout, int P,
              const T* __restrict__ bias, int bias_all_slots) {
    typedef typename Acc4<T>::type acc_t;
    constexpr int KC = 16;
    extern __shared__ __attribute__((aligned(32))) char smem_raw[];
    T* mbuf = reinterpret_cast<T*>(smem_raw);
    const int w = blockIdx.y, tid = threadIdx.x, nthr = blockDim.x, wave = tid >> 6, lane = tid & 63;
    const int lr = lane & 15, lq = lane >> 4, n0 = (blockIdx.z * (nthr >> 6) + wave) * 16 * NB;
    const bool active = n0 < Nout;
    const T* Gw = G + (size_t)w * S.N * S.ldk * P;
    const int nchunk = S.nch * Kh / KC;
    acc_t acc[NB][ST];
#pragma unroll
    for (int a = 0; a < NB; ++a)
#pragma unroll
        for (int s = 0; s < ST; ++s) acc[a][s] = acc_t{0, 0, 0, 0};
    auto fill = [&](int c, T* dst) {
        const int sp = (c * KC) / Kh, k0 = (c * KC) % Kh;
        const int i0 = sp == 0 ? 0 : S.n_up, ns = sp == 0 ? S.n_up : S.n_dn;
        const T inv = T(1) / T(ns);
        const T* g0 = Gw + ((size_t)i0 * S.ldk + k0) * P;
        typedef T vec4 __attribute__((ext_vector_type(4)));
        for (int e = tid; e < KC * P / 4; e += nthr) {
            vec4 v = {0, 0, 0, 0};
#pragma unroll 6
            for (int i = 0; i < ns; ++i) v += *reinterpret_cast<const vec4*>(g0 + (size_t)i * S.ldk * P + 4 * e);
            *reinterpret_cast<vec4*>(dst + 4 * e) = v * inv;
        }
    };
    fill(0, mbuf);
    __syncthreads();
    for (int c = 0; c < nchunk; ++c) {
        const T* cur = mbuf + (c & 1) * KC * P;
        if (c + 1 < nchunk) fill(c + 1, mbuf + ((c + 1) & 1) * KC * P);
        if (active) {
            const T* Wp = Wsh + (size_t)(c * KC + lq) * Nout + n0 + lr;
#pragma unroll
            for (int ks = 0; ks < KC / 4; ++ks) {
                T av[NB], bv[ST];
#pragma unroll
                for (int a = 0; a < NB; ++a) av[a] = Wp[(size_t)(4 * ks) * Nout + 16 * a];
#pragma unroll
                for (int s = 0; s < ST; ++s) bv[s] = cur[(4 * ks + lq) * P + 16 * s + lr];
#pragma unroll
                for (int a = 0; a < NB; ++a)
#pragma unroll
                    for (int s = 0; s < ST; ++s) acc[a][s] = mfma16(av[a], bv[s], acc[a][s]);
            }
        }
        __syncthreads();
    }
    if (!active) return;
    T* Sp = Sb + (size_t)w * Nout * P;
#pragma unroll
    for (int a = 0; a < NB; ++a)
#pragma unroll
        for (int r = 0; r < 4; ++r) {
            const int n = n0 + 16 * a + acc_row<T>(lane, r);
            const T bn = bias ? bias[n] : T(0);
#pragma unroll
            for (int s = 0; s < ST; ++s) Sp[(size_t)n * P + 16 * s + lr] = acc[a][s][r] + ((bias_all_slots || (s == 0 && lr == 0)) ? bn : T(0));
        }
}

}
```

deepsolid_amd/csrc/ds_host.h:

```cpp
#pragma once
#include "ds_base.h"
#include "ds_value.h"

namespace ds {
namespace host {

template <typename I> inline I rup(I x, int m) { return (x + m - 1) / m * m; }

template <typename T> struct Arena {
    T* base = nullptr;
    size_t cap = SIZE_MAX, used = 0;
    bool ok = true;
    T* take(size_t n) { T* p = base ? base + used : nullptr; used += n; ok = ok && used <= cap; return p; }
    void align(size_t k) { take((k - used % k) % k); }
    template <typename F> void part(T* buf, size_t n, F&& carve) { Arena a{buf, n}; carve(a); ok = ok && a.ok; }
};
template <typename T> Arena<T> arena_of(void* ws, int64_t ws_bytes) { return Arena<T>{(T*)ws, (size_t)std::max<int64_t>(ws_bytes, 0) / sizeof(T)}; }
template <typename F> size_t measure(F&& layout) { Arena<double> a; layout(a); return a.used; }

struct PassSize { size_t fixed, per_group; };
inline int64_t groups_per_pass(int64_t B, int64_t esz, const PassSize& z, int64_t budget) {
    const int64_t groups = std::min<int64_t>((std::max<int64_t>(B, 1) + ds::PV - 1) / ds::PV, 64);
    return std::max<int64_t>(1, std::min<int64_t>(groups, budget / ((int64_t)z.per_group * esz)));
}
inline int64_t groups_that_fit(int64_t ws_bytes, int64_t esz, const PassSize& z) {
    return (ws_bytes / esz - (int64_t)z.fixed) / (int64_t)z.per_group;
}

inline int carve_fail(const char* what) { return fail("internal: %s: workspace carve exceeds its size", what); }

struct WsLayout {
    size_t G, MEAN, ZB, H2, Q, MOUT, MINV, DETS, TR;
    size_t PARTM = 0;
    size_t XL = 0;
    size_t YO = 0;
    size_t mout_off[2], minv_off[2], dets_off[2], tr_off[2];
    size_t per_walker;
};

}
}

struct ds_system {
    ds_system_desc d;
    int dtype;
    ds::SysDev<double> sd;
    ds::SysDev<float> sf;
    void* blob64 = nullptr;
    void* blob32 = nullptr;
    std::vector<ds_param_block> blocks;
    int64_t nparams = 0;
    ds::host::WsLayout ws;
    ds::host::WsLayout wsv;
    std::vector<int> i_wloc, i_wsh, i_b, i_w2, i_b2, i_worb, i_wsh_orb, i_borb, i_pi, i_sg;
    bool use_last = false;
    int32_t ref_single[DS_MAX_LAYERS] = {0}, ref_double[DS_MAX_LAYERS] = {0};
    bool res1[DS_MAX_LAYERS] = {false}, res2[DS_MAX_LAYERS] = {false};
    bool no_lu_wave = false;
    int val_nb = 0;
    bool det_valu = false;
    int64_t chunk_cap = 4096;
    bool use_g4 = true;
    bool use_pair_expand = true;
    bool use_pm_skip = true;
    bool use_lr = true;
    void* lr_w0t = nullptr;
    int64_t val_i8_min_tiles = 512;
    bool use_i8_val = true;
    bool use_pair_fuse = true;
    bool use_ldsb = true;
    bool use_i8 = false;
    void* i8_wp = nullptr;
    uint64_t call_seq = 0;
    uint64_t i8_prepped[DS_MAX_LAYERS];
    int n_cu = 256;
    bool use_wide = true;
    bool wide_all = false;
    int dbg = 0;
    bool prof_on = false;
    int prof_only = -1;
    std::vector<std::pair<hipEvent_t, hipEvent_t>> prof_ev[DS_PROF_KINDS];
    std::vector<hipEvent_t> prof_pool;
    unsigned long long* clk_dev = nullptr;
    bool prof_failed = false;
};

namespace ds {
namespace host {

struct ProfScope {
    ds_system* s; int kind; hipStream_t st; hipEvent_t e0 = nullptr, e1 = nullptr;
    static hipEvent_t get(ds_system* s) {
        if (!s->prof_pool.empty()) { hipEvent_t e = s->prof_pool.back(); s->prof_pool.pop_back(); return e; }
        hipEvent_t e = nullptr;
        if (hipEventCreate(&e) != hipSuccess) { s->prof_failed = true; return nullptr; }
        return e;
    }
    ProfScope(ds_system* s_, int kind_, hipStream_t st_) : s(s_), kind(kind_), st(st_) {
        if (s->prof_on && (s->prof_only < 0 || s->prof_only == kind)) {
            e0 = get(s); e1 = get(s);
            if (!e0 || !e1 || hipEventRecord(e0, st) != hipSuccess) { s->prof_failed = true; recycle(); }
        }
    }
    void recycle() {
        if (e0) s->prof_pool.push_back(e0);
        if (e1) s->prof_pool.push_back(e1);
        e0 = e1 = nullptr;
    }
    ~ProfScope() {
        if (e0) {
            if (hipEventRecord(e1, st) == hipSuccess) s->prof_ev[kind].push_back({e0, e1});
            else { s->prof_failed = true; recycle(); }
        }
    }
};

template <typename T> ds::SysDev<T>& dev(ds_system* s);
template <> inline ds::SysDev<double>& dev<double>(ds_system* s) { return s->sd; }
template <> inline ds::SysDev<float>& dev<float>(ds_system* s) { return s->sf; }

template <typename T> struct Carve {
    T *G[2], *MEAN[2], *ZB, *H2[2], *Q, *MOUT, *MINV, *DETS, *TR, *XL, *YO;
};
template <typename T> Carve<T> carve(const ds_system* s, Arena<T>& a, int64_t Bc) {
    const WsLayout& w = s->ws;
    Carve<T> c;
    for (T*& g : c.G) g = a.take(w.G * Bc);
    for (T*& m : c.MEAN) m = a.take(w.MEAN * Bc);
    c.ZB = a.take(w.ZB * Bc);
    for (T*& h : c.H2) h = a.take(w.H2 * Bc);
    c.Q = a.take(w.Q * Bc);
    c.MOUT = a.take(w.MOUT * Bc); c.MINV = a.take(w.MINV * Bc);
    c.DETS = a.take(w.DETS * Bc); c.TR = a.take(w.TR * Bc);
    c.XL = a.take(w.XL * Bc); c.YO = a.take(w.YO * Bc);
    return c;
}

template <typename T> struct ValBufs {
    T* Gl[DS_MAX_LAYERS + 1];
    T* H2l[DS_MAX_LAYERS + 1];
    T *MEAN0, *MEANS, *ZB, *Q, *MOUT, *DETS, *PARTM;
    T* PHI[2];
    T* SORB[2];
    T* MINV;
    T* PM[DS_MAX_LAYERS];
    bool pm_fit;
    bool keep;
};

template <typename T>
ValBufs<T> carve_value(const ds_system* s, Arena<T>& a, int64_t ng) {
    const ds::SysDev<double>& S = s->sd;
    const WsLayout& L = s->wsv;
    ValBufs<T> b{};
    T* G[2]; T* MEAN[2]; T* H2[2];
    for (T*& g : G) g = a.take(L.G * ng);
    for (T*& m : MEAN) m = a.take(L.MEAN * ng);
    b.ZB = a.take(L.ZB * ng);
    for (T*& h : H2) h = a.take(L.H2 * ng);
    b.Q = a.take(L.Q * ng); b.MOUT = a.take(L.MOUT * ng);
    b.DETS = a.take(L.DETS * ng); b.PARTM = a.take(L.PARTM * ng);
    b.MEAN0 = MEAN[0]; b.MEANS = MEAN[1];
    for (int l = 0; l <= S.n_layers; ++l) { b.Gl[l] = G[l & 1]; b.H2l[l] = H2[l & 1]; }
    for (int sp = 0; sp < 2; ++sp)
        a.part(b.ZB, L.ZB * ng, [&](Arena<T>& z) {
            b.PHI[sp] = z.take((size_t)(sp == 0 ? S.n_up : S.n_dn) * S.ocols[sp] * ds::PV * ng);
            b.SORB[sp] = z.take((size_t)S.ocols[sp] * ds::PV * ng);
        });
    Arena<T> idle{H2[1], L.H2 * ng};
    b.PM[0] = b.PARTM;
    for (int l = 1; l < S.n_double && l < DS_MAX_LAYERS; ++l) b.PM[l] = idle.take(L.PARTM * ng);
    b.pm_fit = idle.ok;
    b.MINV = nullptr;
    return b;
}

inline void gemm_geom(int Nout, int NB, dim3* block, unsigned* gz, int ST = 0) {
    const int nw = Nout / (16 * NB), wmax = (NB == 3 || ST > 5) ? 4 : 1024 / NB / 64;
    int wpb = nw < wmax ? nw : wmax;
    for (int c = wpb - wpb % 4; c >= 4; c -= 4)
        if (nw % c == 0) { wpb = c; break; }
    *block = dim3(wpb * 64);
    *gz = (unsigned)((nw + wpb - 1) / wpb);
}


int64_t workspace_budget();

int logpsi_forward(ds_system* s, const void* params, const void* x, int64_t B, void* out_logabs, void* out_phase, void* ws, int64_t ws_bytes,
                   hipStream_t st);
template <typename T>
int run_value_chain(ds_system* s, const T* params, const T* x, int64_t Bc, const ValBufs<T>& vb, hipStream_t st, T* out_logabs, T* out_phase);
template <typename T>
void launch_gemm_plain(dim3 grid, dim3 block, hipStream_t st, const T* X, size_t x_walker_stride, size_t x_tile_stride, const T* W, int K,
                       const T* X2, size_t x2_walker_stride, const T* W2, int K2, int n_tiles, T* Z, size_t z_walker_stride,
                       size_t z_tile_stride, int Nout, int P, const T* Sb, const T* bias, const ds::OrbEpi<T>& oe);
bool int8_energy_layer(const ds_system* s, int l);
bool int8_value_layer(const ds_system* s, int l);
size_t i8_planes_bytes(const ds_system* s);
void launch_layer_i8(ds_system* s, int l, bool value_epilogue, const double* Wloc, int Kloc, int Nout, const double* Gin, size_t tile_stride,
                     const double* Sb, double* Gout, int ntiles, hipStream_t st);

template <typename T> void launch_spin_mean(dim3 grid, hipStream_t st, const ds::SysDev<T>& S, const T* G, int Kh, T* MEAN);

int logpsi_grad_forward(ds_system* s, const void* params, const void* x, int64_t B, void* out_logabs, void* out_phase, void* out_grad,
                        void* ws, int64_t ws_bytes, hipStream_t st);
int energy_grad_forward(ds_system* s, const void* params, const void* x, int64_t B, void* out_ke, void* out_ew3, void* out_logabs,
                        void* out_phase, void* out_grad, void* ws, int64_t ws_bytes, hipStream_t st);
int int8_energy_layers(const ds_system* s, bool dump);
template <typename T> void launch_pair_res_add(dim3 grid, hipStream_t st, const T* Hin, int Kin, T* Hout, int Kout, int n_res, int NP);
template <typename T>
void launch_layer_res_add(dim3 grid, hipStream_t st, const T* Xin, size_t x_ws, size_t x_ts, T* Gout, size_t g_ws, size_t g_ts, int n_res,
                          int Nout, int P);

template <typename T>
void launch_det_inverse(const ds_system* s, const ds::SysDev<T>& S, const Carve<T>& c, int ch, int64_t Bc, hipStream_t st);
template <typename T>
int launch_det_trace(const ds_system* s, const ds::SysDev<T>& S, const Carve<T>& c, int ch, int64_t Bc, hipStream_t st);
template <typename T>
void launch_det_value(const ds_system* s, const ds::SysDev<T>& S, const ValBufs<T>& vb, int64_t Bc, hipStream_t st);

}
}
```

deepsolid_amd/csrc/ds_tiles.h:

```cpp
#pragma once
#include "ds_gemm.h"
#include "ds_wide.h"
#include "ds_ldsb.h"

namespace ds {

template <typename T> struct GemmArgs {
    const T* X; size_t xws, xts; const T* W; int K; const T* X2; size_t x2ws; const T* W2; int K2; int n_tiles;
    T* Z; size_t zws, zts; int Nout, P; const T* Sb; const T* bias; OrbEpi<T> oe;
};

template <typename T> struct TileOps {
    int NB, ST;
    void (*gemm)(int epi, dim3 grid, dim3 block, hipStream_t st, const GemmArgs<T>& a);
    void (*gemm_orb3)(dim3 grid, dim3 block, hipStream_t st, const GemmArgs<T>& a);
    void (*shared_term)(dim3 grid, dim3 block, size_t lds, hipStream_t st, const SysDev<T>& S, const T* G, const T* Wsh, int Kh, T* Sb,
                        int Nout, int P, const T* bias, int bias_all_slots);
    void (*layer1_lr)(int nc, bool res, dim3 grid, dim3 block, hipStream_t st, const LrArgs<T>& a);
    void (*layer0_stats)(int nks, dim3 grid, hipStream_t st, const SysDev<T>& S, const T* XL, size_t xl_ws, size_t xl_ts, const T* W0,
                         const T* S0, int Nout, int P, T* YO, T* MEAN1);
    void (*gemm_wide)(int epi, dim3 grid, dim3 block, hipStream_t st, const GemmArgs<T>& a);
    void (*layer1_lr_wide)(int nc, bool res, dim3 grid, dim3 block, hipStream_t st, const LrArgs<T>& a);
    void (*orbital_lb)(dim3 grid, hipStream_t st, const GemmArgs<T>& a);
};

constexpr int DS_MAX_TILES = 25;
constexpr int tile_nb(int st, int elem_bytes) { return st <= 5 ? 4 : (st <= 10 ? 2 : (elem_bytes == 4 ? 2 : 1)); }

constexpr bool layer0_stats_instance(int st, int nks) { return st <= 5 && nks >= 2 && nks <= 4; }
template <typename T> constexpr bool gemm_wide_faster(int epi) { return sizeof(T) == 8 || epi == 1 || epi == 9; }
template <typename T> constexpr bool lr_wide_faster(int nc) { return sizeof(T) == 8 && nc <= 2; }

template <typename T> const TileOps<T>* tile_ops(int st_tiles);

template <typename T>
bool launch_det_inv_wave(int n, dim3 grid, hipStream_t st, const SysDev<T>& S, const T* MOUT, size_t mout_stride, size_t mout_off, int ch, int es,
                         T* MINV, size_t minv_stride, size_t minv_off, T* DETS, size_t dets_stride, size_t dets_off, int P);

}
```

deepsolid_amd/csrc/ds_tiles_inst.hip:

```cpp
#include <hip/hip_runtime.h>

#include "ds_tiles.h"

#if DS_F32
typedef float DS_T;
#else
typedef double DS_T;
#endif

#if DS_PART == 0
#define DS_ST_LIST(X) X(1) X(2) X(3) X(4) X(5)
#elif DS_PART == 1
#define DS_ST_LIST(X) X(6) X(7) X(8) X(9) X(10)
#elif DS_PART == 2
#define DS_ST_LIST(X) X(11) X(12) X(13) X(14) X(15)
#elif DS_PART == 3
#define DS_ST_LIST(X) X(16) X(17) X(18) X(19) X(20)
#elif DS_PART == 4
#define DS_ST_LIST(X) X(21) X(22) X(23) X(24) X(25)
#else
#error "DS_PART must be 0..4"
#endif

namespace ds {

template <typename T, int NB, int ST> struct TileImpl {
    static void gemm(int epi, dim3 grid, dim3 block, hipStream_t st, const GemmArgs<T>& a) {
#define DS_G(E, LDS) hipLaunchKernelGGL((k_jet_gemm<T, NB, ST, E>), grid, block, (LDS), st, a.X, a.xws, a.xts, a.W, a.K, a.X2, a.x2ws, a.W2, a.K2, \
                                        a.n_tiles, a.Z, a.zws, a.zts, a.Nout, a.P, a.Sb, a.bias, a.oe)
        switch (epi) {
            case 1: DS_G(1, 0); break;
            case 2:
                if constexpr (NB == 4 && ST == 5 && sizeof(T) == 8) {
                    if (a.oe.g4 == 3) {
                        hipLaunchKernelGGL((k_jet_gemm<T, NB, ST, 2, 3>), grid, block, (gemm_stash_bytes<T, NB, ST>(block.x)), st, a.X, a.xws, a.xts, a.W, a.K, a.X2, a.x2ws,
                                           a.W2, a.K2, a.n_tiles, a.Z, a.zws, a.zts, a.Nout, a.P, a.Sb, a.bias, a.oe);
                        break;
                    }
                }
                if constexpr (NB == 2 && ST == 10 && sizeof(T) == 8) {
                    if (a.oe.g4 == 1) {
                        hipLaunchKernelGGL((k_jet_gemm<T, NB, ST, 2, 1>), grid, block, (gemm_stash_bytes<T, NB, ST>(block.x)), st, a.X, a.xws, a.xts, a.W, a.K, a.X2, a.x2ws, a.W2, a.K2,
                                           a.n_tiles, a.Z, a.zws, a.zts, a.Nout, a.P, a.Sb, a.bias, a.oe);
                        break;
                    }
                }
                DS_G(2, (gemm_stash_bytes<T, NB, ST>(block.x)));
                break;
            case 5:
                if constexpr (ST == 10 && sizeof(T) == 8) {
                    if (a.oe.g4 == 1) {
                        hipLaunchKernelGGL((k_jet_gemm<T, NB, ST, 5, 1>), grid, block, (block.x / 64) * 64 * sizeof(T), st, a.X, a.xws, a.xts, a.W, a.K, a.X2, a.x2ws, a.W2, a.K2,
                                           a.n_tiles, a.Z, a.zws, a.zts, a.Nout, a.P, a.Sb, a.bias, a.oe);
                        break;
                    }
                }
                DS_G(5, 0);
                break;
            case 6: DS_G(6, 0); break;
            case 9: DS_G(9, 0); break;
            default: break;
        }
#undef DS_G
    }
    static void gemm_orb3(dim3 grid, dim3 block, hipStream_t st, const GemmArgs<T>& a) {
        if constexpr (ST == 5 && sizeof(T) == 8) {
            if (a.oe.g4 == 3) {
                hipLaunchKernelGGL((k_jet_gemm<T, 3, ST, 5, 3>), grid, block, (block.x / 64) * 64 * sizeof(T), st, a.X, a.xws, a.xts, a.W, a.K, a.X2, a.x2ws, a.W2, a.K2,
                                   a.n_tiles, a.Z, a.zws, a.zts, a.Nout, a.P, a.Sb, a.bias, a.oe);
                return;
            }
        }
        if constexpr (ST <= 5)
            hipLaunchKernelGGL((k_jet_gemm<T, 3, ST, 5>), grid, block, 0, st, a.X, a.xws, a.xts, a.W, a.K, a.X2, a.x2ws, a.W2, a.K2, a.n_tiles, a.Z,
                               a.zws, a.zts, a.Nout, a.P, a.Sb, a.bias, a.oe);
    }
    static void shared_term(dim3 grid, dim3 block, size_t lds, hipStream_t st, const SysDev<T>& S, const T* G, const T* Wsh, int Kh, T* Sb,
                            int Nout, int P, const T* bias, int bias_all_slots) {
        hipLaunchKernelGGL((k_shared_term<T, NB, ST>), grid, block, lds, st, S, G, Wsh, Kh, Sb, Nout, P, bias, bias_all_slots);
    }
    static void layer1_lr(int nc, bool res, dim3 grid, dim3 block, hipStream_t st, const LrArgs<T>& a) {
        if constexpr (sizeof(T) == 8 && ST <= 10) {
            const int rem = a.K0loc + a.K0sh + 4 - 16 * (nc - 1);
            if (nc >= 2 && nc <= 3 && (rem == 4 || rem == 8)) {
#define DS_LRG(NCV, NGV, RESV) hipLaunchKernelGGL((k_layer1_lr<T, NB, ST, NCV, RESV, NGV>), grid, block, (lr_lds_bytes<T, NB, NCV, NGV>(block.x, a.Kh)), st, a)
                if (nc == 2) { if (rem == 4) { if (res) DS_LRG(1, 1, true); else DS_LRG(1, 1, false); } else { if (res) DS_LRG(1, 2, true); else DS_LRG(1, 2, false); } }
                else { if (rem == 4) { if (res) DS_LRG(2, 1, true); else DS_LRG(2, 1, false); } else { if (res) DS_LRG(2, 2, true); else DS_LRG(2, 2, false); } }
#undef DS_LRG
                return;
            }
        }
#define DS_LR(NCV, RESV) hipLaunchKernelGGL((k_layer1_lr<T, NB, ST, NCV, RESV>), grid, block, (lr_lds_bytes<T, NB, NCV>(block.x, a.Kh)), st, a)
        if (nc <= 2) { if (res) DS_LR(2, true); else DS_LR(2, false); }
        else if (nc == 3) { if (res) DS_LR(3, true); else DS_LR(3, false); }
        else { if (res) DS_LR(4, true); else DS_LR(4, false); }
#undef DS_LR
    }
    static void layer0_stats(int nks, dim3 grid, hipStream_t st, const SysDev<T>& S, const T* XL, size_t xl_ws, size_t xl_ts, const T* W0,
                             const T* S0, int Nout, int P, T* YO, T* MEAN1) {
        if constexpr (ST <= 5) {
#define DS_L0S(NKSV) hipLaunchKernelGGL((k_layer0_stats<T, ST, NKSV>), grid, dim3(256), 0, st, S, XL, xl_ws, xl_ts, W0, S0, Nout, P, YO, MEAN1)
            if (nks == 2) DS_L0S(2);
            else if (nks == 3) DS_L0S(3);
            else if (nks == 4) DS_L0S(4);
#undef DS_L0S
        }
    }
    static constexpr int STCW = sizeof(T) == 4 ? 5 : 4, STCO = sizeof(T) == 4 ? 7 : 4;
    static void gemm_wide(int epi, dim3 grid, dim3 block, hipStream_t st, const GemmArgs<T>& a) {
        if constexpr (ST > 10) {
#define DS_GW(STCV, E, LDS) hipLaunchKernelGGL((k_jet_gemm_wide<T, STCV, E>), grid, block, (LDS), st, a.X, a.xws, a.xts, a.W, a.K, a.n_tiles, a.Z, a.zws, a.zts, \
                                               a.Nout, a.P, a.Sb, a.oe)
            switch (epi) {
                case 1: DS_GW(STCW, 1, 0); break;
                case 2: DS_GW(STCW, 2, (wide_stash_bytes<T, STCW>(block.x))); break;
                case 5: DS_GW(STCO, 5, 0); break;
                case 9: DS_GW(STCW, 9, 0); break;
                default: break;
            }
#undef DS_GW
        }
    }
    static void layer1_lr_wide(int nc, bool res, dim3 grid, dim3 block, hipStream_t st, const LrArgs<T>& a) {
        if constexpr (ST > 10) {
#define DS_LRW(NCV, RESV) hipLaunchKernelGGL((k_layer1_lr_wide<T, STCW, NCV, RESV>), grid, block, (lr_lds_bytes<T, 4, NCV>(block.x, a.Kh)), st, a)
            if (nc <= 2) { if (res) DS_LRW(2, true); else DS_LRW(2, false); }
            else if (nc == 3) { if (res) DS_LRW(3, true); else DS_LRW(3, false); }
            else { if (res) DS_LRW(4, true); else DS_LRW(4, false); }
#undef DS_LRW
        }
    }
    static void orbital_lb(dim3 grid, hipStream_t st, const GemmArgs<T>& a) {
        if constexpr (ST > 10 && sizeof(T) == 4)
            hipLaunchKernelGGL((k_jet_gemm_lb<T, ST, 5, 4>), grid, dim3(256), ldsb_bytes<T>(a.P), st, a.X, a.xws, a.xts, a.W, a.K, a.n_tiles, a.Z, a.zws,
                               a.zts, a.Nout, a.P, a.Sb, a.oe);
    }
    static const TileOps<T>* ops() {
        static const TileOps<T> o = {NB, ST, &gemm, (ST <= 5 ? &gemm_orb3 : nullptr), &shared_term, &layer1_lr, (ST <= 5 ? &layer0_stats : nullptr),
                                      (ST > 10 ? &gemm_wide : nullptr), (ST > 10 ? &layer1_lr_wide : nullptr),
                                      ((ST > 10 && sizeof(T) == 4) ? &orbital_lb : nullptr)};
        return &o;
    }
};

#define DS_CAT2(a, b, c) a##b##c
#define DS_CAT(a, b, c) DS_CAT2(a, b, c)
#if DS_F32
#define DS_PART_FN DS_CAT(tile_ops_f32_p, DS_PART, )
#else
#define DS_PART_FN DS_CAT(tile_ops_f64_p, DS_PART, )
#endif

const TileOps<DS_T>* DS_PART_FN(int st_tiles) {
    switch (st_tiles) {
#define DS_CASE(STV) case STV: return TileImpl<DS_T, tile_nb(STV, (int)sizeof(DS_T)), STV>::ops();
        DS_ST_LIST(DS_CASE)
#undef DS_CASE
        default: return nullptr;
    }
}

}
```

deepsolid_amd/csrc/ds_value.hip:

```cpp
#include "ds_host.h"
#include "ds_i8.h"

namespace ds {
namespace host {

inline int val_nb(int forced, int64_t wgs64) { return forced ? forced : (wgs64 >= 1024 ? 4 : (wgs64 >= 448 ? 2 : 1)); }
inline void val_geom(int Nout, int NB, dim3* block, unsigned* gz) {
    if (NB >= 3) { gemm_geom(Nout, NB, block, gz); return; }
    *block = dim3(256);
    *gz = (unsigned)((Nout + 64 * NB - 1) / (64 * NB));
}

inline int m2_rc(int K2) { return K2 % 16 == 0 ? 16 : K2; }

inline bool i8_shape(const ds_system* s, int l) {
    const ds::SysDev<double>& S = s->sd;
    return s->dtype == 0 && l >= 1 && s->res1[l] && S.h1[l + 1] == ds::i8::NOUT && S.h1[l] + S.nch * S.h2[l] == 320;
}
bool int8_energy_layer(const ds_system* s, int l) { return s->use_i8 && s->sd.P == ds::i8::P && i8_shape(s, l); }
bool int8_value_layer(const ds_system* s, int l) { return s->use_i8_val && ds::PV == ds::i8::P && i8_shape(s, l); }

inline size_t i8_slot_bytes() { return ds::i8::wp_bytes(64 * 5) + ds::i8::NOUT * sizeof(double); }
inline void i8_prepare(ds_system* s, int l, const double* Wloc, int Kloc, int Nout, hipStream_t st, uint8_t** wp, double** sw) {
    *wp = (uint8_t*)s->i8_wp + (size_t)l * i8_slot_bytes();
    *sw = (double*)(*wp + ds::i8::wp_bytes(64 * 5));
    if (s->i8_prepped[l] != s->call_seq) {
        hipLaunchKernelGGL(ds::i8::k_i8_prep_w, dim3(ds::i8::NOUT / 16), dim3(256), 0, st, Wloc, Kloc, Nout, *wp, *sw);
        s->i8_prepped[l] = s->call_seq;
    }
}

size_t i8_planes_bytes(const ds_system* s) {
    bool need = int8_energy_layers(s, true) > 0;
    for (int l = 1; l < s->sd.n_layers; ++l) need = need || int8_value_layer(s, l);
    return need ? (size_t)DS_MAX_LAYERS * i8_slot_bytes() : 0;
}

void launch_layer_i8(ds_system* s, int l, bool value_epilogue, const double* Wloc, int Kloc, int Nout, const double* Gin, size_t tile_stride,
                     const double* Sb, double* Gout, int ntiles, hipStream_t st) {
    uint8_t* wp; double* sw;
    i8_prepare(s, l, Wloc, Kloc, Nout, st, &wp, &sw);
    const dim3 grid((unsigned)std::min<int64_t>(ntiles, s->n_cu));
    if (value_epilogue)
        hipLaunchKernelGGL((ds::i8::k_layer_i8<5, 4>), grid, dim3(512), ds::i8::lds_bytes(), st, Gin, tile_stride, (const uint4*)wp, sw, Sb, s->sd.N,
                           Gout, ntiles);
    else
        hipLaunchKernelGGL((ds::i8::k_layer_i8<5, 2>), grid, dim3(512), ds::i8::lds_bytes(), st, Gin, tile_stride, (const uint4*)wp, sw, Sb, s->sd.N,
                           Gout, ntiles);
}

template <typename T>
int run_value_chain(ds_system* s, const T* params, const T* x, int64_t Bc, const ValBufs<T>& vb, hipStream_t st, T* out_logabs,
                    T* out_phase) {
    const ds::SysDev<T>& S = dev<T>(s);
    const WsLayout& L = s->wsv;
    const int PV = ds::PV;
    const int64_t ng = (Bc + PV - 1) / PV;
    T* ZB = vb.ZB; T* Q = vb.Q; T* MOUT = vb.MOUT; T* DETS = vb.DETS;
    auto blk = [&](int i) { return params + s->blocks[i].offset; };
    const unsigned fsplit = (unsigned)std::min<int64_t>(256, std::max<int64_t>(ds::FV_SPLIT, (2048 + ng - 1) / ng));
    hipLaunchKernelGGL((ds::k_features_val<T, 0>), dim3((unsigned)ng, fsplit), dim3(256), 0, st, S, x, (long)Bc, blk(s->i_pi[0]),
                       blk(s->i_sg[0]), blk(s->i_pi[S.nch - 1]), blk(s->i_sg[S.nch - 1]), vb.Gl[0], vb.MEAN0, vb.H2l[0], Q);
    hipLaunchKernelGGL((ds::k_features_val<T, 1>), dim3((unsigned)ng, fsplit), dim3(256), 0, st, S, x, (long)Bc, blk(s->i_pi[0]),
                       blk(s->i_sg[0]), blk(s->i_pi[S.nch - 1]), blk(s->i_sg[S.nch - 1]), vb.Gl[0], vb.MEAN0, vb.H2l[0], Q);
    const size_t gws = (size_t)S.N * S.ldk * PV, gts = (size_t)S.ldk * PV;
    const bool fuse_means = S.n_up >= 8 && (S.n_dn >= 8 || S.n_dn == 0) && !(S.n_double >= 1 && s->res2[0]);
    bool fuse_pairs = fuse_means && !vb.keep && s->use_pair_fuse && S.n_double >= 1 && S.n_double <= ds::PS_MAX_LAYERS && !s->res2[0] &&
                      S.h2[0] % 4 == 0 && (S.h2[1] == 16 || S.h2[1] == 32) && vb.pm_fit;
    for (int l = 1; l < S.n_double; ++l) fuse_pairs = fuse_pairs && S.h2[l + 1] == S.h2[1];
    auto pm_of = [&](int l) -> T* { return fuse_pairs ? vb.PM[l] : vb.PARTM; };
    if (fuse_pairs) {
        ds::PairStreamArgs<T> pa{};
        pa.H0 = vb.H2l[0]; pa.Kin0 = S.h2[0]; pa.nl = S.n_double;
        for (int l = 0; l < S.n_double; ++l) { pa.W[l] = blk(s->i_w2[l]); pa.b[l] = blk(s->i_b2[l]); pa.res[l] = s->res2[l] ? 1 : 0; pa.PM[l] = pm_of(l); }
        dim3 grid((S.NP / 16 + 3) / 4, (unsigned)(ng * (PV / 5)));
        if (S.h2[1] == 32) hipLaunchKernelGGL((ds::k_pair_stream_val<T, 2>), grid, dim3(256), 0, st, S, pa);
        else hipLaunchKernelGGL((ds::k_pair_stream_val<T, 1>), grid, dim3(256), 0, st, S, pa);
    }
    for (int l = 0; l < S.n_layers; ++l) {
        const int Kh = S.h1[l], K2 = S.h2[l], Nout = S.h1[l + 1];
        T* Gin = vb.Gl[l]; T* Gout = vb.Gl[l + 1];
        T* Hin = vb.H2l[l < S.n_double ? l : S.n_double];
        if (l > 0 && l <= S.n_double && fuse_means)
            hipLaunchKernelGGL((ds::k_m2_combine_val<T>), dim3(S.N, (unsigned)ng, (unsigned)(S.nch * K2 / m2_rc(K2))), dim3(256), (size_t)m2_rc(K2) * PV * sizeof(T), st, S, pm_of(l - 1), K2, Gin, Kh, m2_rc(K2));
        else
            hipLaunchKernelGGL((ds::k_m2_expand_val<T>), dim3(S.N, (unsigned)ng), dim3(256), 0, st, S, Hin, K2, Gin, Kh);
        if (l < S.n_double && !fuse_pairs) {
            const int K2o = S.h2[l + 1];
            if (K2o != 32 && K2o != 16) return fail("hidden_double must be 16 or 32 (got %d)", K2o);
            dim3 grid((S.NP / 16 + 3) / 4, (unsigned)(ng * (PV / 5)));
            const bool res_sep = s->res2[l] && l == 0;
            const bool res = s->res2[l] && !res_sep;
            const T* W2 = blk(s->i_w2[l]); const T* b2 = blk(s->i_b2[l]);
            T* Hnext = (fuse_means && !vb.keep && l + 1 == S.n_double) ? (T*)nullptr : vb.H2l[l + 1];
            T* pmv = fuse_means ? vb.PARTM : (T*)nullptr;
#define DS_TWO(NT2, RES) hipLaunchKernelGGL((ds::k_two_layer<T, NT2, RES, true>), grid, dim3(256), 0, st, S, Hin, K2, W2, b2, Hnext, pmv)
            if (K2o == 32) { if (res) DS_TWO(2, true); else DS_TWO(2, false); }
            else { if (res) DS_TWO(1, true); else DS_TWO(1, false); }
#undef DS_TWO
            if (res_sep)
                launch_pair_res_add<T>(dim3((unsigned)(((size_t)K2o * 5 * S.NP + 255) / 256), (unsigned)(ng * (PV / 5))), st, Hin, K2, Hnext, K2o, S.nf, S.NP);
        }
        if (Nout % 64 || Nout > 1024) return fail("hidden_single must be a multiple of 64 and <= 1024 (got %d)", Nout);
        const int Kloc = Kh + S.nch * K2, Ksh = S.nch * Kh;
        const bool res_sep = s->res1[l] && l == 0 && (Kloc % 16 != 0 || S.nf * S.A != Nout);
        if (s->res1[l] && !res_sep && Kloc % 16) return fail("residual layer with K = %d: the GEMM's operand ring needs K %% 16 == 0", Kloc);
        dim3 block; unsigned gz;
        gemm_geom(Nout, 4, &block, &gz);
        const int nbh = val_nb(s->val_nb, (int64_t)S.N * ng * gz / (sizeof(T) == 4 ? 2 : 1));
        if (l == 0)
            hipLaunchKernelGGL((ds::k_jet_gemm<T, 4, 5, 7>), dim3(1, (unsigned)ng, gz), block, 0, st, (const T*)nullptr, (size_t)0, (size_t)0,
                               (const T*)nullptr, 0, vb.MEAN0, (size_t)Ksh * PV, blk(s->i_wsh[l]), Ksh, 0, ZB, (size_t)Nout * PV, (size_t)0, Nout, PV,
                               (const T*)nullptr, blk(s->i_b[l]), ds::OrbEpi<T>{});
        else {
            launch_spin_mean<T>(dim3((unsigned)((Ksh * PV + 255) / 256), (unsigned)ng), st, S, Gin, Kh, vb.MEANS);
            if (nbh < 4 && Ksh % 16 == 0)
                hipLaunchKernelGGL((ds::k_jet_gemm<T, 1, 1, 7>), dim3(PV / 16, (unsigned)ng, (unsigned)(Nout / 64)), dim3(256), 0, st, (const T*)nullptr, (size_t)0, (size_t)16,
                                   (const T*)nullptr, 0, vb.MEANS, (size_t)Ksh * PV, blk(s->i_wsh[l]), Ksh, 0, ZB, (size_t)Nout * PV, (size_t)16, Nout, PV,
                                   (const T*)nullptr, blk(s->i_b[l]), ds::OrbEpi<T>{});
            else
                hipLaunchKernelGGL((ds::k_jet_gemm<T, 1, 5, 7>), dim3(1, (unsigned)ng, (unsigned)(Nout / 64)), dim3(256), 0, st, (const T*)nullptr, (size_t)0, (size_t)0,
                                   (const T*)nullptr, 0, vb.MEANS, (size_t)Ksh * PV, blk(s->i_wsh[l]), Ksh, 0, ZB, (size_t)Nout * PV, (size_t)0, Nout, PV,
                                   (const T*)nullptr, blk(s->i_b[l]), ds::OrbEpi<T>{});
        }
#define DS_VHID(NBV) { dim3 hb; unsigned hz; val_geom(Nout, NBV, &hb, &hz); \
            hipLaunchKernelGGL((ds::k_jet_gemm<T, NBV, 5, 4>), dim3(S.N, (unsigned)ng, hz), hb, (ds::gemm_stash_bytes<T, NBV, 5>(hb.x)), st, Gin, gws, gts, blk(s->i_wloc[l]), Kloc, \
                               (const T*)nullptr, (size_t)0, (const T*)nullptr, 0, S.N, Gout, gws, gts, Nout, PV, ZB, blk(s->i_b[l]), ds::OrbEpi<T>{}); }
        if (sizeof(T) == 8 && int8_value_layer(s, l) && (int64_t)S.N * ng >= (int64_t)s->val_i8_min_tiles) {
            launch_layer_i8(s, l, true, (const double*)blk(s->i_wloc[l]), Kloc, Nout, (const double*)Gin, gts, (const double*)ZB, (double*)Gout,
                                  (int)(S.N * ng), st);
        } else if (s->res1[l] && !res_sep) {
            if (nbh == 4) DS_VHID(4) else if (nbh == 2) DS_VHID(2) else DS_VHID(1)
        } else {
#undef DS_VHID
            hipLaunchKernelGGL((ds::k_jet_gemm<T, 4, 5, 3>), dim3(S.N, (unsigned)ng, gz), block, 0, st, Gin, gws, gts, blk(s->i_wloc[l]), Kloc,
                               (const T*)nullptr, (size_t)0, (const T*)nullptr, 0, S.N, Gout, gws, gts, Nout, PV, ZB, blk(s->i_b[l]), ds::OrbEpi<T>{});
            if (res_sep)
                launch_layer_res_add<T>(dim3(S.N, (unsigned)ng), st, (const T*)Gin, gws, gts, Gout, gws, gts, S.nf * S.A, Nout, PV);
        }
    }
    T* Gl = vb.Gl[S.n_layers];
    const int Kl = S.h1[S.n_layers], K2l = S.h2[S.n_layers];
    if (s->use_last) {
        if (fuse_means) hipLaunchKernelGGL((ds::k_m2_combine_val<T>), dim3(S.N, (unsigned)ng, (unsigned)(S.nch * K2l / m2_rc(K2l))), dim3(256), (size_t)m2_rc(K2l) * PV * sizeof(T), st, S, pm_of(S.n_double - 1), K2l, Gl, Kl, m2_rc(K2l));
        else hipLaunchKernelGGL((ds::k_m2_expand_val<T>), dim3(S.N, (unsigned)ng), dim3(256), 0, st, S, vb.H2l[S.n_double], K2l, Gl, Kl);
    }
    for (int sp = 0; sp < S.nch; ++sp) {
        const int ns = sp == 0 ? S.n_up : S.n_dn, i0 = sp == 0 ? 0 : S.n_up, OC = S.ocols[sp];
        const int Korb = Kl + (s->use_last ? S.nch * K2l : 0);
        if (Korb % 16) return fail("orbital head with K = %d: the GEMM's operand ring needs K %% 16 == 0", Korb);
        dim3 oblock; unsigned ogz;
        gemm_geom(OC, 4, &oblock, &ogz);
        T* Sorb = vb.SORB[sp];
        if (s->use_last)
            hipLaunchKernelGGL((ds::k_shared_term<T, 4, 5>), dim3(1, (unsigned)ng, ogz), oblock, 2 * 16 * PV * sizeof(T), st, S, Gl,
                               blk(s->i_wsh_orb[sp]), Kl, Sorb, OC, PV, (const T*)nullptr, 0);
        if (vb.keep) {
            launch_gemm_plain<T>(dim3(ns, (unsigned)ng, ogz), oblock, st, Gl + (size_t)i0 * S.ldk * PV,
                               gws, gts, blk(s->i_worb[sp]), Korb, (const T*)nullptr, (size_t)0, (const T*)nullptr, 0, ns, vb.PHI[sp], (size_t)ns * OC * PV, (size_t)0,
                               OC, PV, (const T*)nullptr, (const T*)nullptr, ds::OrbEpi<T>{});
            if (MOUT)
                hipLaunchKernelGGL((ds::k_orbital_epilogue_val<T>), dim3(ns, (unsigned)ng), dim3(256), 0, st, S, vb.PHI[sp], (size_t)ns * OC * PV, Q, MOUT, sp,
                                   L.MOUT, L.mout_off[S.mat_ch[sp]], S.bias_orb ? blk(s->i_borb[sp]) : (const T*)nullptr,
                                   s->use_last ? (const T*)Sorb : (const T*)nullptr);
            continue;
        }
        ds::OrbEpi<T> oe{Q, MOUT, L.MOUT, L.mout_off[S.mat_ch[sp]], S.N, i0, S.nparam[sp], S.nparam_max, S.norb[sp], S.det_n[S.mat_ch[sp]],
                         S.row_off[sp], S.bias_orb ? blk(s->i_borb[sp]) : (const T*)nullptr, nullptr};
#define DS_VORB(NBV, BLK, GZ) hipLaunchKernelGGL((ds::k_jet_gemm<T, NBV, 5, 8>), dim3(ns, (unsigned)ng, GZ), BLK, 0, st, Gl + (size_t)i0 * S.ldk * PV, \
                           gws, gts, blk(s->i_worb[sp]), Korb, (const T*)nullptr, (size_t)0, (const T*)nullptr, 0, ns, (T*)nullptr, (size_t)0, (size_t)0, \
                           OC, PV, s->use_last ? (const T*)Sorb : (const T*)nullptr, (const T*)nullptr, oe)
        const bool w48 = OC % 256 != 0 && OC % 192 == 0;
        const int nbo = val_nb(s->val_nb, (int64_t)ns * ng * (w48 ? OC / 192 : ogz) / (sizeof(T) == 4 ? 2 : 1));
        if (nbo < 4) DS_VORB(1, dim3(256), (unsigned)((OC + 63) / 64));
        else if (w48) DS_VORB(3, dim3(256), (unsigned)(OC / 192));
        else DS_VORB(4, oblock, ogz);
#undef DS_VORB
    }
    if (out_logabs || out_phase || vb.MINV) {
        const size_t dstride = s->ws.DETS;
        launch_det_value<T>(s, S, vb, Bc, st);
        if (out_logabs || out_phase)
            hipLaunchKernelGGL((ds::k_combine_val<T>), dim3((unsigned)((Bc + 255) / 256)), dim3(256), 0, st, S, DETS, dstride, s->ws.dets_off[1], (long)Bc,
                               out_logabs, out_phase);
    }
    HIP_OK(hipGetLastError());
    return 0;
}

template <typename T>
int logpsi_impl(ds_system* s, const void* params, const void* x, int64_t B, void* out_logabs, void* out_phase, void* ws, int64_t ws_bytes,
                hipStream_t st) {
    const ds::SysDev<T>& S = dev<T>(s);
    const int64_t cg = groups_that_fit(ws_bytes, sizeof(T), PassSize{0, s->wsv.per_walker});
    if (cg < 1) return fail("workspace too small for the value chain: %lld bytes < %zu per group", (long long)ws_bytes, s->wsv.per_walker * sizeof(T));
    const int64_t chunk = cg * ds::PV;
    for (int64_t b0 = 0; b0 < B; b0 += chunk) {
        const int64_t Bc = std::min(chunk, B - b0);
        Arena<T> a = arena_of<T>(ws, ws_bytes);
        const ValBufs<T> vb = carve_value<T>(s, a, (Bc + ds::PV - 1) / ds::PV);
        if (!a.ok) return carve_fail("value chain");
        int rc = run_value_chain<T>(s, (const T*)params, (const T*)x + b0 * 3 * S.N, Bc, vb, st, out_logabs ? (T*)out_logabs + b0 : nullptr,
                                    out_phase ? (T*)out_phase + 2 * b0 : nullptr);
        if (rc) return rc;
    }
    return 0;
}

template <typename T>
int orbitals_impl(ds_system* s, const void* params, const void* x, int64_t B, void* out_up, void* out_dn, void* ws, int64_t ws_bytes,
                  hipStream_t st) {
    const ds::SysDev<T>& S = dev<T>(s);
    const int64_t cg = groups_that_fit(ws_bytes, sizeof(T), PassSize{0, s->wsv.per_walker});
    if (cg < 1) return fail("workspace too small for the value chain");
    const int64_t chunk = cg * ds::PV;
    for (int64_t b0 = 0; b0 < B; b0 += chunk) {
        const int64_t Bc = std::min(chunk, B - b0);
        Arena<T> a = arena_of<T>(ws, ws_bytes);
        const ValBufs<T> vb = carve_value<T>(s, a, (Bc + ds::PV - 1) / ds::PV);
        if (!a.ok) return carve_fail("value chain");
        T* mout = vb.MOUT;
        int rc = run_value_chain<T>(s, (const T*)params, (const T*)x + b0 * 3 * S.N, Bc, vb, st, nullptr, nullptr);
        if (rc) return rc;
        for (int sp = 0; sp < S.n_detch; ++sp) {
            const int n = S.det_n[sp];
            T* o = (T*)(sp == 0 ? out_up : out_dn);
            if (!o) continue;
            const size_t per = (size_t)S.K * n * n * 2;
            hipLaunchKernelGGL((ds::k_gather_val<T>), dim3((unsigned)((per + 255) / 256), (unsigned)Bc), dim3(256), 0, st, mout, s->wsv.MOUT,
                               s->wsv.mout_off[sp], per, (long)b0, (long)Bc, o);
        }
    }
    HIP_OK(hipGetLastError());
    return 0;
}

int logpsi_forward(ds_system* s, const void* params, const void* x, int64_t B, void* out_logabs, void* out_phase, void* ws, int64_t ws_bytes,
                   hipStream_t st) {
    return DS_BY_DTYPE(s->dtype, logpsi_impl, s, params, x, B, out_logabs, out_phase, ws, ws_bytes, st);
}

template <typename T>
void launch_gemm_plain(dim3 grid, dim3 block, hipStream_t st, const T* X, size_t x_walker_stride, size_t x_tile_stride, const T* W, int K,
                       const T* X2, size_t x2_walker_stride, const T* W2, int K2, int n_tiles, T* Z, size_t z_walker_stride,
                       size_t z_tile_stride, int Nout, int P, const T* Sb, const T* bias, const ds::OrbEpi<T>& oe) {
    hipLaunchKernelGGL((ds::k_jet_gemm<T, 4, 5, 0>), grid, block, 0, st, X, x_walker_stride, x_tile_stride, W, K, X2, x2_walker_stride, W2, K2,
                       n_tiles, Z, z_walker_stride, z_tile_stride, Nout, P, Sb, bias, oe);
}

#define DS_INST(T)                                                                                                                   \
    template int run_value_chain<T>(ds_system*, const T*, const T*, int64_t, const ValBufs<T>&, hipStream_t, T*, T*);                    \
    template void launch_gemm_plain<T>(dim3, dim3, hipStream_t, const T*, size_t, size_t, const T*, int, const T*, size_t, const T*, int, \
                                       int, T*, size_t, size_t, int, int, const T*, const T*, const ds::OrbEpi<T>&);
DS_INST(double) DS_INST(float)
#undef DS_INST

}
}

using namespace ds::host;

extern "C" {

int ds_logpsi(ds_system* s, const void* params, const void* x, int64_t B, void* out_logabs, void* out_phase, void* ws,
              int64_t ws_bytes, void* stream) {
    if (s) ++s->call_seq;
    if (!s || !params || !x || !ws) return fail("null argument");
    if (B <= 0) return 0;
    hipStream_t st = (hipStream_t)stream;
    return logpsi_forward(s, params, x, B, out_logabs, out_phase, ws, ws_bytes, st);
}

int ds_orbitals(ds_system* s, const void* params, const void* x, int64_t B, void* out_up, void* out_dn, void* ws, int64_t ws_bytes,
                void* stream) {
    if (s) ++s->call_seq;
    if (!s || !params || !x || !ws || !out_up) return fail("null argument");
    if (B <= 0) return 0;
    hipStream_t st = (hipStream_t)stream;
    return DS_BY_DTYPE(s->dtype, orbitals_impl, s, params, x, B, out_up, out_dn, ws, ws_bytes, st);
}

}
```

deepsolid_amd/device.py:

```python
import ctypes as C

import numpy as np
import torch

from . import _lib
from .params import ParamMap

_DTYPES = {torch.float64: 0, torch.float32: 1}


def _pd(a):
    return a.ctypes.data_as(C.POINTER(C.c_double))


def _ptr(t):
    return C.c_void_p(t.data_ptr()) if t is not None else C.c_void_p(0)


def _stream():
    return C.c_void_p(torch.cuda.current_stream().cuda_stream)


def _require_gpu():
    if not torch.cuda.is_available():
# ... 438 lines not shown
                raise ValueError(f'shifts must be ({B}, {M}, 3), got {tuple(shifts.shape)}')
        ratios = torch.empty(B, M, 2, dtype=self.dtype, device=self.device) if want_ratios else None
        out_s = torch.empty(B, M, 3, dtype=self.dtype, device=self.device) if want_shifts else None
        n_bad = torch.zeros(2, dtype=torch.int64, device=self.device)
        ws = self._workspace('ds_one_body_workspace_bytes', int(B), M, max_bytes=max_bytes) if B >= 1 and M >= 1 else \
            self.workspace(max(B, 1))
        _lib.check(self.lib.ds_one_body_ratios(self.handle, _ptr(p), _ptr(x), B, M, int(first_electron), int(seed) & (2 ** 64 - 1),
                                               int(offset) & (2 ** 64 - 1), _ptr(shifts), _ptr(kv), n_k, _ptr(nk_sums), _ptr(ratios),
                                               _ptr(out_s), _ptr(n_bad), _ptr(ws), ws.numel(), _stream()), 'ds_one_body_ratios')
        return dict(nk_sums=nk_sums, n_bad=n_bad, ratios=torch.view_as_complex(ratios) if want_ratios else None, shifts=out_s)

    def spin_exchange_ratios(self, params, x, n_pairs=None, first_pair=0, sums=None, want_ratios=False, want_walker=False,
                             max_bytes=None):
        x = self._check_x(x)
        B = x.shape[0]
        M = self.nelec[0] * self.nelec[1] if n_pairs is None else int(n_pairs)
        p = self.pack_params(params)
        if sums is None:
            sums = torch.zeros(4, dtype=torch.float64, device=self.device)
        elif not (sums.is_cuda and sums.dtype == torch.float64 and sums.is_contiguous() and tuple(sums.shape) == (4,)):
            raise ValueError('sums must be a contiguous float64 device tensor of shape (4,)')
        ratios = torch.empty(B, M, 2, dtype=self.dtype, device=self.device) if want_ratios and M >= 1 else None
        walker = torch.empty(B, 2, dtype=torch.float64, device=self.device) if want_walker else None
        n_bad = torch.zeros(1, dtype=torch.int64, device=self.device)
        ws = self._workspace('ds_spin_exchange_workspace_bytes', int(B), M, max_bytes=max_bytes) if B >= 1 and M >= 1 else \
            self.workspace(max(B, 1))
        _lib.check(self.lib.ds_spin_exchange_ratios(self.handle, _ptr(p), _ptr(x), B, M, int(first_pair), _ptr(sums), _ptr(ratios),
                                                    _ptr(walker), _ptr(n_bad), _ptr(ws), ws.numel(), _stream()),
                   'ds_spin_exchange_ratios')
        return dict(sums=sums, n_bad=n_bad, ratios=torch.view_as_complex(ratios) if ratios is not None else None,
                    walker=torch.view_as_complex(walker) if want_walker else None)

    def dmc_state(self, x, weight=None):
        x = self._check_x(x).clone()
        B = x.shape[0]
        f64 = dict(dtype=torch.float64, device=self.device)
        w = torch.ones(B, **f64) if weight is None else torch.as_tensor(weight).to(**f64).reshape(B).clone()
        return dict(x=x, logabs=torch.zeros(B, dtype=self.dtype, device=self.device),
                    phase=torch.zeros(B, 2, dtype=self.dtype, device=self.device), drift=torch.zeros_like(x),
                    eloc=torch.zeros(B, **f64), weight=w)

    def _check_dmc_state(self, state):
        B = state['x'].shape[0]
        shapes = dict(x=((B, 3 * self.n), self.dtype), logabs=((B,), self.dtype), phase=((B, 2), self.dtype),
                      drift=((B, 3 * self.n), self.dtype), eloc=((B,), torch.float64), weight=((B,), torch.float64))
        for k, (shape, dt) in shapes.items():
            t = state[k]
            if not (t.is_cuda and t.dtype == dt and t.is_contiguous() and tuple(t.shape) == shape):
                raise ValueError(f'DMC state entry {k!r} must be a contiguous {dt} device tensor of shape {shape}')
        return B

    def dmc_step(self, params, state, steps, tau, tau_eff=None, e_trial=0.0, e_ref=0.0, e_cut=0.0, node_mode=0, branch_every=1,
                 seed=0, offset=0, normals=None, uniforms=None, comb_uniforms=None, state_valid=True, want_parents=False,
                 max_bytes=None):
        B = self._check_dmc_state(state)
        steps = int(steps)
        p = self.pack_params(params)
        given = [t is not None for t in (normals, uniforms, comb_uniforms)]
        if all(given):
            normals = normals.to(device=self.device, dtype=self.dtype).contiguous()
            uniforms = uniforms.to(device=self.device, dtype=self.dtype).contiguous()
            comb_uniforms = comb_uniforms.to(device=self.device, dtype=torch.float64).contiguous()
            if tuple(normals.shape) != (steps, B, 3 * self.n) or tuple(uniforms.shape) != (steps, B) or tuple(comb_uniforms.shape) != (steps,):
                raise ValueError('explicit noise must be normals (steps, B, 3N), uniforms (steps, B) and comb_uniforms (steps,)')
        stats = torch.zeros(max(steps, 1), 9, dtype=torch.float64, device=self.device)
        parents = torch.empty(max(steps, 1), B, dtype=torch.int32, device=self.device) if want_parents else None
        ws = self._workspace('ds_dmc_workspace_bytes', int(B), max_bytes=max_bytes) if 1 <= B <= 2 ** 20 else self.workspace(1)
        _lib.check(self.lib.ds_dmc_step(
            self.handle, _ptr(p), _ptr(state['x']), _ptr(state['logabs']), _ptr(state['phase']), _ptr(state['drift']),
            _ptr(state['eloc']), _ptr(state['weight']), B, steps, float(tau), float(tau if tau_eff is None else tau_eff),
            float(e_trial), float(e_ref), float(e_cut), int(node_mode), int(branch_every), int(seed) & (2 ** 64 - 1),
            int(offset) & (2 ** 64 - 1), _ptr(normals), _ptr(uniforms), _ptr(comb_uniforms), int(bool(state_valid)), _ptr(stats),
            _ptr(parents), _ptr(ws), ws.numel(), _stream()), 'ds_dmc_step')
        return dict(stats=stats, parents=parents)

    def dmc_noise(self, B, steps, seed=0, offset=0):
        nz = torch.empty(steps, B, 3 * self.n, dtype=self.dtype, device=self.device)
        un = torch.empty(steps, B, dtype=self.dtype, device=self.device)
        xi = torch.empty(steps, dtype=torch.float64, device=self.device)
        _lib.check(self.lib.ds_dmc_noise(0 if self.dtype == torch.float64 else 1, self.n, int(B), int(steps), int(seed) & (2 ** 64 - 1),
                                         int(offset) & (2 ** 64 - 1), _ptr(nz), _ptr(un), _ptr(xi), _stream()), 'ds_dmc_noise')
        return nz, un, xi

    def dmc_branch(self, state, xi, want_parents=True):
        B = self._check_dmc_state(state)
        need = int(self.lib.ds_dmc_branch_workspace_bytes(0 if self.dtype == torch.float64 else 1, self.n, B))
        if need < 0:
            need = 256
        if self._ws is None or self._ws.numel() < need:
            self._ws = None
            self._ws = torch.empty(need, dtype=torch.uint8, device=self.device)
        parents = torch.empty(B, dtype=torch.int32, device=self.device) if want_parents else None
        _lib.check(self.lib.ds_dmc_branch(0 if self.dtype == torch.float64 else 1, self.n, B, float(xi), _ptr(state['x']),
                                          _ptr(state['logabs']), _ptr(state['phase']), _ptr(state['drift']), _ptr(state['eloc']),
                                          _ptr(state['weight']), _ptr(parents), _ptr(self._ws), self._ws.numel(), _stream()),
                   'ds_dmc_branch')
        return parents

    def ecp_energy(self, params, x, ecp, seed=0, offset=0, rotations=None, pair_capacity=None, want_pairs=False, want_ratios=False,
                   want_rotations=False, max_bytes=None):
        import re
        x = self._check_x(x)
        B = x.shape[0]
        if not isinstance(ecp, EcpTables):
            tables = ecp.__dict__.get('_ds_tables')
            if tables is None or tables.device != self.device:
                tables = ecp.__dict__['_ds_tables'] = EcpTables(ecp, device=self.device)
            ecp = tables
        p = self.pack_params(params)
        if rotations is not None:
            rotations = rotations.to(device=self.device, dtype=torch.float64).contiguous()
            if tuple(rotations.shape) != (B, 3, 3):
                raise ValueError(f'rotations must be ({B}, 3, 3), got {tuple(rotations.shape)}')
        cap = B * self.n if pair_capacity is None else int(pair_capacity)
        energy = torch.empty(B, 3, dtype=torch.float64, device=self.device)
        pairs = torch.empty(B, dtype=torch.int64, device=self.device) if want_pairs or want_ratios else None
        rot = torch.empty(B, 3, 3, dtype=torch.float64, device=self.device) if want_rotations else None
        for attempt in range(2):
            ratios = torch.empty(max(cap, 1) * ecp.n_quad, 2, dtype=self.dtype, device=self.device) if want_ratios else None
            ws = self._workspace('ds_ecp_workspace_bytes', ecp.handle, B, cap, max_bytes=max_bytes)
            rc = self.lib.ds_ecp_energy(self.handle, ecp.handle, _ptr(p), _ptr(x), B, int(seed) & (2 ** 64 - 1), int(offset) & (2 ** 64 - 1),
                                        _ptr(rotations), cap, _ptr(energy), _ptr(pairs), _ptr(ratios), _ptr(rot), _ptr(ws), ws.numel(),
                                        _stream())
            if rc != 0 and attempt == 0:
                m = re.search(r'pair capacity exceeded: the walkers have (\d+) pairs', self.lib.ds_last_error().decode())
                if m:
                    cap = int(m.group(1))
                    continue
            _lib.check(rc, 'ds_ecp_energy')
            break
        return dict(e_loc=energy[:, 0], e_nl=torch.complex(energy[:, 1], energy[:, 2]), pairs=pairs if want_pairs else None,
                    rotations=rot, pair_capacity=cap,
                    ratios=torch.view_as_complex(ratios)[:int(pairs.sum()) * ecp.n_quad] if want_ratios else None)

    def energy_stats(self, ke, ew):
        out = torch.empty(8, dtype=torch.float64, device=self.device)
        _lib.check(self.lib.ds_energy_stats(self.handle, _ptr(ke), _ptr(ew), ke.shape[0], _ptr(out), _stream()), 'ds_energy_stats')
        return out

    def profile(self, on=True, only=None):
        mode = 0 if not on else (1 if only is None else 2 + _lib.PROF_KINDS.index(only))
        _lib.check(self.lib.ds_profile_enable(self.handle, mode), 'ds_profile_enable')

    def profile_read(self):
        n = len(_lib.PROF_KINDS)
        ms = (C.c_double * n)()
        cnt = (C.c_int64 * n)()
        _lib.check(self.lib.ds_profile_read(self.handle, ms, cnt), 'ds_profile_read')
        return {k: (float(ms[i]), int(cnt[i])) for i, k in enumerate(_lib.PROF_KINDS)}

    def int8_layers(self):
        return int(self.lib.ds_int8_layers(self.handle))

    def profile_clock(self):
        cyc, ticks = C.c_double(0), C.c_double(0)
        _lib.check(self.lib.ds_profile_read_clock(self.handle, C.byref(cyc), C.byref(ticks)), 'ds_profile_read_clock')
        return cyc.value, ticks.value, (cyc.value / ticks.value * 0.1 if ticks.value > 0 else None)

    def debug_stage(self, params, x, stage, n_elems):
        x = self._check_x(x)
        p = self.pack_params(params)
        ws = self.workspace(x.shape[0])
        out = torch.zeros(int(n_elems), dtype=self.dtype, device=self.device)
        n = self.lib.ds_debug_stage(self.handle, _ptr(p), _ptr(x), x.shape[0], stage.encode(), _ptr(out), out.numel(),
                                    _ptr(ws), ws.numel(), _stream())
        if n < 0:
            raise RuntimeError(f'ds_debug_stage({stage}): {self.lib.ds_last_error().decode()}')
        return out[:n]


def observable_sums(recvec, x, q_int, pol_direction):
    _require_gpu()
    if not x.is_cuda:
        raise RuntimeError('observable_sums: walkers must live on the ROCm device (no CPU path)')
    if x.dtype not in _DTYPES:
        raise TypeError(f'observable_sums: walkers must be float64 or float32, got {x.dtype}')
    if x.dim() != 2 or x.shape[1] % 3:
        raise ValueError(f'observable_sums: walkers must have shape (B, 3N), got {tuple(x.shape)}')
    if x.shape[0] < 1:
        raise ValueError('observable_sums: empty walker batch (the observables are batch means)')
    lib = _lib.load()
    x = x.contiguous()
    rv = np.ascontiguousarray(np.asarray(recvec, dtype=np.float64).reshape(3, 3))
    q = np.ascontiguousarray(np.asarray(q_int, dtype=np.int32).reshape(-1, 3))
    B, n_q = x.shape[0], q.shape[0]
    need = lib.ds_observables_workspace_bytes(B, n_q)
    ws = torch.empty(max(int(need), 8) // 8, dtype=torch.float64, device=x.device)
    out = torch.empty(2 + 3 * n_q, dtype=torch.float64, device=x.device)
    _lib.check(lib.ds_observables(_pd(rv), _DTYPES[x.dtype], _ptr(x), B, x.shape[1] // 3,
                                  q.ctypes.data_as(C.POINTER(C.c_int32)), n_q, int(pol_direction), _ptr(out), _ptr(ws),
                                  ws.numel() * 8, _stream()), 'ds_observables')
    return out


def realspace_counts(x, n_up, dens=None, fold_lattice=None, pair=None, latvec=None, r_max=None):
    _require_gpu()
    if not x.is_cuda:
        raise RuntimeError('realspace_counts: walkers must live on the ROCm device (no CPU path)')
    if x.dtype not in _DTYPES:
        raise TypeError(f'realspace_counts: walkers must be float64 or float32, got {x.dtype}')
    if x.dim() != 2 or x.shape[1] % 3:
        raise ValueError(f'realspace_counts: walkers must have shape (B, 3N), got {tuple(x.shape)}')
    if x.shape[0] < 1:
        raise ValueError('realspace_counts: empty walker batch')
    if dens is None and pair is None:
        raise ValueError('realspace_counts: neither a density nor a pair buffer was given')
    for name, buf, lead in (('dens', dens, 2), ('pair', pair, 3)):
        if buf is None:
            continue
        if not (isinstance(buf, torch.Tensor) and buf.dtype == torch.int64 and buf.is_contiguous()):
            raise TypeError(f'realspace_counts: {name} must be a contiguous int64 tensor')
        if buf.device != x.device:
            raise RuntimeError(f'realspace_counts: {name} lives on {buf.device}, the walkers on {x.device}')
        if buf.dim() != (4 if lead == 2 else 2) or buf.shape[0] != lead:
            raise ValueError(f'realspace_counts: {name} must have shape ' + ('(2, g0, g1, g2)' if lead == 2 else '(3, n_r)')
                             + f', got {tuple(buf.shape)}')
    lib = _lib.load()
    x = x.contiguous()
    f8 = lambda v: np.ascontiguousarray(np.asarray(v, dtype=np.float64).reshape(3, 3))
    fold_inv = grid = a = a_inv = None
    n_r, rm = 0, 0.0
    if dens is not None:
        if fold_lattice is None:
            raise ValueError('realspace_counts: the density needs fold_lattice')
        fold_inv = np.ascontiguousarray(np.linalg.inv(f8(fold_lattice)))
        grid = np.asarray(dens.shape[1:], dtype=np.int32)
    if pair is not None:
        if latvec is None or r_max is None:
            raise ValueError('realspace_counts: the pair counts need latvec and r_max')
        a = f8(latvec)
        a_inv = np.ascontiguousarray(np.linalg.inv(a))
        n_r, rm = int(pair.shape[1]), float(r_max)
    _lib.check(lib.ds_realspace_counts(_pd(fold_inv) if fold_inv is not None else None,
                                       grid.ctypes.data_as(C.POINTER(C.c_int32)) if grid is not None else None,
                                       _pd(a) if a is not None else None, _pd(a_inv) if a_inv is not None else None, rm, n_r,
                                       _DTYPES[x.dtype], _ptr(x), x.shape[0], x.shape[1] // 3, int(n_up), _ptr(dens), _ptr(pair),
                                       _stream()), 'ds_realspace_counts')


class HfOrbitalTables:

    def __init__(self, a, atoms, shell_atom, shell_l, shell_nprim, exps, coefs, kpts, images, nocc, mo, device=None):
        _require_gpu()
        self.lib = _lib.load()
        self.device = torch.device('cuda', torch.cuda.current_device()) if device is None else torch.device(device)
        f8 = lambda v, shape: np.ascontiguousarray(np.asarray(v, dtype=np.float64).reshape(shape))
        i4 = lambda v: np.ascontiguousarray(np.asarray(v, dtype=np.int32).reshape(-1))
        pi = lambda v: v.ctypes.data_as(C.POINTER(C.c_int32))
        a, atoms, kpts, images = f8(a, (3, 3)), f8(atoms, (-1, 3)), f8(kpts, (-1, 3)), f8(images, (-1, 3))
        shell_atom, shell_l, shell_nprim = i4(shell_atom), i4(shell_l), i4(shell_nprim)
        exps, coefs = f8(exps, -1), f8(coefs, -1)
        nocc = [i4(n) for n in nocc]
        mo = [np.ascontiguousarray(np.asarray(m, dtype=np.complex128)) for m in mo]
        self.nelec = tuple(int(m.shape[1]) for m in mo)
        d = _lib.HfDesc()
        d.a[:] = a.reshape(-1).tolist()
        d.n_atoms, d.atoms = atoms.shape[0], _pd(atoms)
        d.n_shells, d.shell_atom, d.shell_l, d.shell_nprim = shell_l.shape[0], pi(shell_atom), pi(shell_l), pi(shell_nprim)
        d.exps, d.coefs = _pd(exps), _pd(coefs)
        d.n_k, d.kpts = kpts.shape[0], _pd(kpts)
        d.n_images, d.images = images.shape[0], _pd(images)
        d.n_up, d.n_dn = self.nelec
        d.nocc_up, d.nocc_dn = pi(nocc[0]), pi(nocc[1])
        d.mo_up, d.mo_dn = (m.view(np.float64).ctypes.data_as(C.POINTER(C.c_double)) if m.size else None for m in mo)
        self.handle = C.c_void_p()
        with torch.cuda.device(self.device):
            _lib.check(self.lib.ds_hf_create(C.byref(d), C.byref(self.handle)), 'ds_hf_create')

    def __del__(self):
        h, self.handle = getattr(self, 'handle', None), None
        if h:
            try:
                self.lib.ds_hf_destroy(h)
            except Exception:
                pass

    def orbitals(self, x):
        if not x.is_cuda or x.device != self.device:
            raise RuntimeError(f'HfOrbitalTables.orbitals: walkers must live on {self.device} (no CPU path)')
        if x.dtype not in _DTYPES:
            raise TypeError(f'HfOrbitalTables.orbitals: walkers must be float64 or float32, got {x.dtype}')
        n = sum(self.nelec)
        if x.dim() != 2 or x.shape[1] != 3 * n:
            raise ValueError(f'HfOrbitalTables.orbitals: walkers must have shape (B, {3 * n}), got {tuple(x.shape)}')
        x = x.contiguous()
        B = x.shape[0]
        outs = [torch.empty(B, ns, ns, 2, dtype=torch.float64, device=x.device) for ns in self.nelec]
        if B:
            with torch.cuda.device(self.device):
                _lib.check(self.lib.ds_hf_orbitals(self.handle, _DTYPES[x.dtype], _ptr(x), B, _ptr(outs[0] if self.nelec[0] else None),
                                                   _ptr(outs[1] if self.nelec[1] else None), _stream()), 'ds_hf_orbitals')
        return [torch.view_as_complex(o) for o in outs]


class EcpTables:

    def __init__(self, ecp, device=None):
        _require_gpu()
        self.lib = _lib.load()
        self.device = torch.device('cuda', torch.cuda.current_device()) if device is None else torch.device(device)
        self.ecp = ecp
        self.n_quad = int(ecp.n_quad)
        d, self._keep = ecp_desc(ecp)
        self.handle = C.c_void_p()
        with torch.cuda.device(self.device):
            _lib.check(self.lib.ds_ecp_create(C.byref(d), C.byref(self.handle)), 'ds_ecp_create')
# ... 30 lines not shown
```

include/deepsolid_hip.h:

```cpp
#ifndef DEEPSOLID_HIP_H
#define DEEPSOLID_HIP_H

#include <stddef.h>
#include <stdint.h>

#ifdef __cplusplus
extern "C" {
#endif

#define DS_MAX_LAYERS 8
#define DS_MAX_SYM 6

typedef struct ds_system ds_system;

typedef struct ds_system_desc {
    int32_t dtype;
    int32_t n_up, n_dn;
    int32_t n_atoms_prim;
    const double* prim_atoms;
    double prim_a[9];
    double sim_a[9];
    int32_t n_sym;
    double prim_AV[DS_MAX_SYM * 3], prim_BV[DS_MAX_SYM * 3];
    double sim_AV[DS_MAX_SYM * 3], sim_BV[DS_MAX_SYM * 3];
    int32_t n_layers;
    int32_t hidden_single[DS_MAX_LAYERS];
    int32_t hidden_double[DS_MAX_LAYERS];
    int32_t n_det;
    int32_t distance_type;
    int32_t envelope_type;
    int32_t full_det;
    int32_t use_last_layer;
    int32_t bias_orbitals;
    const double* klist_up;
    const double* klist_dn;
    int32_t n_atoms_sim;
    const double* sim_atoms;
    const double* sim_charges;
    int32_t dist_mode;
    int32_t n_g;
    const double* gpoints;
    const double* gweight;
    const double* ion_exp_re;
    const double* ion_exp_im;
    double ewald_alpha;
    double ee_const;
    double ei_const;
    double ii_total;
} ds_system_desc;

typedef struct ds_param_block {
    int64_t offset;
    int32_t rows, cols;
} ds_param_block;

int ds_device_widths(const int32_t* hidden_single, const int32_t* hidden_double, int32_t n_layers, int32_t n_in_single,
                     int32_t n_in_double, int32_t n_double, int32_t* dev_single, int32_t* dev_double, int32_t* res_single,
                     int32_t* res_double);

int ds_system_create(const ds_system_desc* desc, ds_system** out);
void ds_system_destroy(ds_system* sys);
const char* ds_last_error(void);

int ds_int8_layers(const ds_system* sys);

int64_t ds_param_count(const ds_system* sys);
int ds_param_layout(const ds_system* sys, ds_param_block* blocks, int max_blocks);

int64_t ds_workspace_bytes(const ds_system* sys, int64_t B);

int ds_logpsi(ds_system* sys, const void* params, const void* x, int64_t B,
              void* out_logabs, void* out_phase, void* ws, int64_t ws_bytes, void* stream);

int ds_logpsi_grad(ds_system* sys, const void* params, const void* x, int64_t B,
                   void* out_logabs, void* out_phase, void* out_grad, void* ws, int64_t ws_bytes, void* stream);

int64_t ds_vjp_workspace_bytes(const ds_system* sys, int64_t B);
int ds_logpsi_vjp(ds_system* sys, const void* params, const void* x, int64_t B, const void* cot, void* grad,
                  void* out_logabs, void* out_phase, void* ws, int64_t ws_bytes, void* stream);

int64_t ds_pretrain_workspace_bytes(const ds_system* sys, int64_t B);
int ds_pretrain_loss_vjp(ds_system* sys, const void* params, const void* x, int64_t B, const void* target_up,
                         const void* target_dn, void* out_loss, void* grad, void* ws, int64_t ws_bytes, void* stream);

typedef struct ds_kfac_block {
    int32_t kind, index;
    int32_t n_param_blocks;
    int32_t param_blocks[3];
    int32_t has_bias, d_in, d_out, repeats;
    int64_t a_offset, g_offset;
} ds_kfac_block;
int ds_kfac_block_count(const ds_system* sys);
int ds_kfac_layout(const ds_system* sys, ds_kfac_block* blocks, int max_blocks);
int64_t ds_kfac_workspace_bytes(const ds_system* sys, int64_t B);
int ds_kfac_factors(ds_system* sys, const void* params, const void* x, int64_t B, void* factors, void* grad_seed, void* ws,
                    int64_t ws_bytes, void* stream);

int64_t ds_kfac_step_workspace_bytes(const ds_system* sys);
int ds_kfac_inverses(ds_system* sys, const void* factors, double ema_weight, double damping, void* inverses, void* ws,
                     int64_t ws_bytes, void* stream);
int ds_kfac_precondition(ds_system* sys, const void* inverses, const void* v, void* out, double* sq_norm, void* ws,
                         int64_t ws_bytes, void* stream);
int64_t ds_kfac_inverses_sized_workspace_bytes(int n_blocks, const int32_t* d_in, const int32_t* d_out);
int ds_kfac_inverses_sized(int dtype, int n_blocks, const int32_t* d_in, const int32_t* d_out, const int32_t* repeats,
                           const void* factors, double ema_weight, double damping, void* inverses, void* ws, int64_t ws_bytes,
                           void* stream);

int ds_orbitals(ds_system* sys, const void* params, const void* x, int64_t B,
                void* out_up, void* out_dn, void* ws, int64_t ws_bytes, void* stream);

int ds_ewald(ds_system* sys, const void* x, int64_t B, void* out, void* stream);

int ds_local_energy(ds_system* sys, const void* params, const void* x, int64_t B,
                    void* out_ke, void* out_ewald, void* out_logabs, void* out_phase,
                    void* ws, int64_t ws_bytes, void* stream);

int ds_enforce_pbc(const double* latvec, int dtype, const void* x, int64_t n_elec, void* out_x,
                   void* out_wrap, void* stream);

int64_t ds_observables_workspace_bytes(int64_t B, int n_q);
int ds_observables(const double* recvec, int dtype, const void* x, int64_t B, int64_t n_elec, const int32_t* q_int, int n_q,
                   int pol_direction, double* out_sums, void* ws, int64_t ws_bytes, void* stream);

int ds_realspace_counts(const double* fold_inv, const int32_t* grid, const double* latvec, const double* latvec_inv, double r_max,
                        int n_r, int dtype, const void* x, int64_t B, int64_t n_elec, int64_t n_up, int64_t* dens, int64_t* pair,
                        void* stream);

int ds_mh_propose(ds_system* sys, const void* x1, const void* normal, double width, int64_t B,
                  void* x2, void* stream);
int ds_mh_accept(ds_system* sys, void* x1, void* lp1, const void* x2, const void* lp2,
                 const void* uniform, int64_t B, void* n_accept, void* stream);

int ds_mh_propose_ex(ds_system* sys, int mode, const void* x1, const void* normal, double width, const void* aux, int n_aux,
                     int64_t B, void* x2, void* scratch, void* stream);
int ds_mh_accept_ex(ds_system* sys, int mode, void* x1, void* lp1, const void* x2, const void* logabs2, const void* uniform,
                    const void* normal, double width, const void* aux1, const void* aux2, int n_aux, int64_t B,
                    void* n_accept, void* scratch, void* stream);

int64_t ds_mcmc_workspace_bytes(const ds_system* sys, int64_t B);
int ds_mcmc_step(ds_system* sys, const void* params, void* x, void* lp, int64_t B, int steps, double width,
                 uint64_t philox_seed, uint64_t philox_offset, const void* normals, const void* uniforms,
                 int lp_valid, void* n_accept, void* ws, int64_t ws_bytes, void* stream);
int ds_mcmc_step_one_electron(ds_system* sys, const void* params, void* x, void* lp, int64_t B, int moves, int first_electron,
                              double width, uint64_t philox_seed, uint64_t philox_offset, const void* normals,
                              const void* uniforms, int lp_valid, void* n_accept, void* ws, int64_t ws_bytes, void* stream);
int ds_mcmc_step_importance(ds_system* sys, const void* params, void* x, void* lp, int64_t B, int steps, double width,
                            uint64_t philox_seed, uint64_t philox_offset, const void* normals, const void* uniforms,
                            int lp_valid, void* n_accept, void* ws, int64_t ws_bytes, void* stream);
int ds_mcmc_step_asymmetric(ds_system* sys, const void* params, void* x, void* lp, int64_t B, int steps, double width,
                            const void* atoms, int n_atoms, uint64_t philox_seed, uint64_t philox_offset, const void* normals,
                            const void* uniforms, int lp_valid, void* n_accept, void* ws, int64_t ws_bytes, void* stream);
void ds_philox_host(uint64_t seed, uint64_t offset, uint64_t step, uint64_t index, int stream_id, uint32_t out[4]);

int64_t ds_one_body_workspace_bytes(const ds_system* sys, int64_t B, int n_samples);
int ds_one_body_ratios(ds_system* sys, const void* params, const void* x, int64_t B, int n_samples, int first_electron,
                       uint64_t philox_seed, uint64_t philox_offset, const void* shifts, const double* kvec, int n_k,
                       double* nk_sums, void* out_ratio, void* out_shift, int64_t* n_bad, void* ws, int64_t ws_bytes, void* stream);

int64_t ds_spin_exchange_workspace_bytes(const ds_system* sys, int64_t B, int n_pairs);
int ds_spin_exchange_ratios(ds_system* sys, const void* params, const void* x, int64_t B, int n_pairs, int first_pair,
                            double* sums, void* out_ratio, double* out_walker, int64_t* n_bad, void* ws, int64_t ws_bytes,
                            void* stream);

typedef struct ds_ecp ds_ecp;
typedef struct ds_ecp_desc {
    double a[9];
    int32_t n_atoms;
    const double* atoms;
    const int32_t* atom_species;
    int32_t n_species;
    const int32_t* n_l;
    const double* r_cut_loc;
    const double* r_cut_nl;
    const int32_t* term_offset;
    const int32_t* term_n;
    const double* term_zeta;
    const double* term_c;
    int32_t n_quad;
} ds_ecp_desc;
int ds_ecp_create(const ds_ecp_desc* desc, ds_ecp** out);
void ds_ecp_destroy(ds_ecp* ecp);
int64_t ds_ecp_workspace_bytes(const ds_system* sys, const ds_ecp* ecp, int64_t B, int64_t pair_capacity);
int ds_ecp_energy(ds_system* sys, const ds_ecp* ecp, const void* params, const void* x, int64_t B, uint64_t philox_seed,
                  uint64_t philox_offset, const double* rotations, int64_t pair_capacity, double* out_energy, int64_t* out_pairs,
                  void* out_ratio, double* out_rotation, void* ws, int64_t ws_bytes, void* stream);

int64_t ds_dmc_workspace_bytes(const ds_system* sys, int64_t B);
int ds_dmc_step(ds_system* sys, const void* params, void* x, void* logabs, void* phase, void* drift, double* eloc, double* weight,
                int64_t B, int steps, double tau, double tau_eff, double e_trial, double e_ref, double e_cut, int node_mode,
                int branch_every, uint64_t philox_seed, uint64_t philox_offset, const void* normals, const void* uniforms,
                const double* comb_uniforms, int state_valid, double* out_stats, int32_t* out_parents, void* ws, int64_t ws_bytes,
                void* stream);
int ds_dmc_noise(int dtype, int n_elec, int64_t B, int steps, uint64_t philox_seed, uint64_t philox_offset, void* normals,
                 void* uniforms, double* comb_uniforms, void* stream);
int64_t ds_dmc_branch_workspace_bytes(int dtype, int n_elec, int64_t B);
int ds_dmc_branch(int dtype, int n_elec, int64_t B, double xi, void* x, void* logabs, void* phase, void* drift, double* eloc,
                  double* weight, int32_t* out_parents, void* ws, int64_t ws_bytes, void* stream);

int ds_energy_stats(ds_system* sys, const void* ke, const void* ewald, int64_t B, double* out_stats, void* stream);

int64_t ds_debug_stage(ds_system* sys, const void* params, const void* x, int64_t B,
                       const char* stage, void* out, int64_t out_elems,
                       void* ws, int64_t ws_bytes, void* stream);

#define DS_PROF_FEATURES 0
#define DS_PROF_M2_EXPAND 1
#define DS_PROF_TWO_LAYER 2
#define DS_PROF_SINGLE_FIRST 3
#define DS_PROF_SINGLE_HIDDEN 4
#define DS_PROF_ORBITAL 5
#define DS_PROF_DET_INVERSE 6
#define DS_PROF_DET_TRACE 7
#define DS_PROF_COMBINE 8
#define DS_PROF_EWALD 9
#define DS_PROF_SHARED_TERM 10
#define DS_PROF_SINGLE_LR 11
#define DS_PROF_KINDS 12
int ds_profile_enable(ds_system* sys, int on);
// ... 38 lines not shown
```

Before: 67570 local-energy evals/s.

## Add quad-electron layer-1 low-rank kernel with fused per-quad sums for layer-2 means

```diff
diff --git a/deepsolid_amd/_lib.py b/deepsolid_amd/_lib.py
--- a/deepsolid_amd/_lib.py
+++ b/deepsolid_amd/_lib.py
@@ -63,6 +63,7 @@
     'ds_last_error': (C.c_char_p, []),
     'ds_param_count': (C.c_int64, [_VP]),
     'ds_int8_layers': (C.c_int, [_VP]),
+    'ds_debug_chain_plan': (C.c_int, [_VP, C.POINTER(C.c_int32), C.c_int32, C.POINTER(C.c_int32)]),
     'ds_param_layout': (C.c_int, [_VP, C.POINTER(ParamBlock), C.c_int]),
     'ds_workspace_bytes': (C.c_int64, [_VP, C.c_int64]),
     'ds_logpsi': (C.c_int, [_VP, _VP, _VP, C.c_int64, _VP, _VP, _VP, C.c_int64, _VP]),
diff --git a/deepsolid_amd/csrc/ds_api.hip b/deepsolid_amd/csrc/ds_api.hip
--- a/deepsolid_amd/csrc/ds_api.hip
+++ b/deepsolid_amd/csrc/ds_api.hip
@@ -362,6 +362,8 @@
     if (const char* e = getenv("DS_VAL_NB")) { const int v = atoi(e); s->val_nb = (v == 1 || v == 2 || v == 4) ? v : 0; }
     s->no_lu_wave = getenv("DS_NO_LU_WAVE") != nullptr;
     s->use_lr = getenv("DS_NO_LOWRANK") == nullptr;
+    s->use_quad = getenv("DS_NO_QUAD") == nullptr;
+    s->quad_sums = getenv("DS_QUAD_NO_SUMS") == nullptr;
     s->use_pm_skip = getenv("DS_NO_PM_SKIP") == nullptr;
     s->use_pair_expand = getenv("DS_NO_PAIR_EXPAND") == nullptr;
     s->use_g4 = getenv("DS_NO_G4") == nullptr;
diff --git a/deepsolid_amd/csrc/ds_chain.hip b/deepsolid_amd/csrc/ds_chain.hip
--- a/deepsolid_amd/csrc/ds_chain.hip
+++ b/deepsolid_amd/csrc/ds_chain.hip
@@ -43,6 +43,7 @@
     bool wide;
     bool pm_mask;
     bool pm_unwritten;
+    bool quad;
     int prof_kind;
     PairPlan pair;
 };
@@ -118,6 +119,16 @@
         lp.pm_unwritten = !dump && l >= 1 && !lp.wide &&
                           (lp.kind == LayerKind::LowRank1 ? s->use_pm_skip : (lp.pm_mask && ds::pm_instance<T>(ST)));
     }
+    if (p->lr_on && S.n_layers >= 3) {
+        LayerPlan& l1 = p->layer[1];
+        ds::LrArgs<T> la{};
+        la.K0loc = K0loc; la.K0sh = K0sh; la.Kh = S.h1[1];
+        const size_t lds = to->layer1_lr_quad_lds(p->lr_nc, s->res1[1], la);
+        constexpr size_t cu_lds = 160 * 1024;
+        const bool rows_idle = S.h1[2] <= S.h1[1] && !(2 < S.n_double && p->layer[2].pair.expand && S.h1[3] < S.h1[2]);
+        l1.quad = s->use_quad && l1.kind == LayerKind::LowRank1 && !l1.wide && s->res1[1] && S.n_up % 4 == 0 && S.n_dn % 4 == 0 && S.n_up >= 4 &&
+                  S.h1[2] % (16 * to->NB) == 0 && lds > 0 && 2 * lds <= cu_lds && rows_idle;
+    }
     const int Korb = S.h1[S.n_layers] + (s->use_last ? S.nch * S.h2[S.n_layers] : 0);
     if (Korb % 16) return fail("orbital head with K = %d: the GEMM's operand ring needs K %% 16 == 0", Korb);
     for (int sp = 0; sp < S.nch; ++sp) {
@@ -145,6 +156,9 @@
     const int NB = to->NB, ST = to->ST, lr_nc = plan.lr_nc;
     const bool lr_on = plan.lr_on;
     const int K0loc = S.h1[0] + S.nch * S.h2[0], K0sh = S.nch * S.h1[0];
+    s->last_n_layers = S.n_layers;
+    for (int l = 0; l < S.n_layers; ++l) s->last_kinds[l] = (int32_t)plan.layer[l].kind;
+    s->last_quad = lr_on && S.n_layers >= 3 && plan.layer[1].quad;
     {
         ProfScope ps(s, DS_PROF_FEATURES, st);
         size_t sh = (size_t)(9 * S.N) * sizeof(T) + (size_t)S.N * S.A * S.nf * sizeof(ds::Jet5<T>);
@@ -211,8 +225,9 @@
                     dim3 sblock; unsigned sgz;
                     gemm_geom(Nout, NB, &sblock, &sgz);
                     if (ST > 10 && sblock.x > 512) { sblock = dim3(512); sgz = (unsigned)((Nout / (16 * NB) + 7) / 8); }
-                    to->shared_term(dim3(1, (unsigned)Bc, sgz), sblock, 2 * 16 * S.P * sizeof(T), st, S, c.G[gi], blk(s->i_wsh[l]), Kh, Sl, Nout, S.P,
-                                    blk(s->i_b[l]), 0);
+                    const bool qs = l == 2 && plan.layer[1].quad && s->quad_sums;
+                    to->shared_term(dim3(1, (unsigned)Bc, sgz), sblock, 2 * 16 * S.P * sizeof(T), st, S, qs ? c.QS : c.G[gi], blk(s->i_wsh[l]), Kh, Sl, Nout, S.P,
+                                    blk(s->i_b[l]), 0, qs ? ds::mean_src_quads<T>(S) : ds::mean_src_electrons<T>(S));
                 }
             }
             ProfScope ps(s, lp.prof_kind, st);
@@ -229,8 +244,12 @@
             case LayerKind::LowRank1: {
                 const ds::LrArgs<T> la{c.XL, (size_t)S.N * K0loc * S.P, (size_t)K0loc * S.P, c.MEAN[0], (size_t)K0sh * S.P, K0loc, K0sh,
                                        (const T*)s->lr_w0t, c.G[gi], gws, gts, blk(s->i_wloc[l]), Kh, S.nch * K2, c.G[gi ^ 1], gws, gts, Sl,
-                                       Nout, S.P, S.N, c.YO, L.YO, blk(s->i_wloc[0]), c.ZB, s->dbg >> 8, S.n_up, S.nch};
-                if (lp.wide) to->layer1_lr_wide(lr_nc, s->res1[l], wgrid, wblock, st, la); else to->layer1_lr(lr_nc, s->res1[l], lgrid, block, st, la);
+                                       Nout, S.P, S.N, c.YO, L.YO, blk(s->i_wloc[0]), c.ZB, s->dbg >> 8, S.n_up, S.nch,
+                                       (lp.quad && s->quad_sums) ? c.QS : (T*)nullptr, gws, gts};
+                if (lp.quad && (c.QS == nullptr || c.QS != c.G[gi])) return fail("internal: quad sums without their rows in the layer-1 input buffer");
+                const dim3 qgrid((unsigned)(S.N / 4 * (Nout / (16 * NB))), (unsigned)Bc, 1);
+                if (lp.wide) to->layer1_lr_wide(lr_nc, s->res1[l], wgrid, wblock, st, la);
+                else to->layer1_lr(lr_nc, s->res1[l], lp.quad, lp.quad ? qgrid : lgrid, block, st, la);
                 break;
             }
             case LayerKind::L0Stats:
@@ -285,7 +304,7 @@
         if (s->use_last) {
             ProfScope ps(s, DS_PROF_SHARED_TERM, st);
             to->shared_term(dim3(1, (unsigned)Bc, gz), block, 2 * 16 * S.P * sizeof(T), st, S, c.G[gi], blk(s->i_wsh_orb[sp]), Kl, c.ZB, OC, S.P,
-                            (const T*)nullptr, 0);
+                            (const T*)nullptr, 0, ds::mean_src_electrons<T>(S));
         }
         ProfScope ps(s, DS_PROF_ORBITAL, st);
         const int ch = S.mat_ch[sp];
@@ -451,6 +470,14 @@
     return int8_energy_layers(s, false);
 }
 
+int ds_debug_chain_plan(const ds_system* s, int32_t* kinds, int32_t max_layers, int32_t* quad) {
+    if (!s) return -1;
+    for (int l = 0; l < s->last_n_layers && l < max_layers; ++l)
+        if (kinds) kinds[l] = s->last_kinds[l];
+    if (quad) *quad = s->last_quad ? 1 : 0;
+    return s->last_n_layers;
+}
+
 int ds_local_energy(ds_system* s, const void* params, const void* x, int64_t B, void* out_ke, void* out_ewald, void* out_logabs,
                     void* out_phase, void* ws, int64_t ws_bytes, void* stream) {
     if (s) ++s->call_seq;
diff --git a/deepsolid_amd/csrc/ds_gemm.h b/deepsolid_amd/csrc/ds_gemm.h
--- a/deepsolid_amd/csrc/ds_gemm.h
+++ b/deepsolid_amd/csrc/ds_gemm.h
@@ -598,16 +598,19 @@
     const T* W0; const T* S0;
     int dbg;
     int n_up, nch;
+    T* QS; size_t qs_ws, qs_ts;
 };
 template <int NB, int NC, int NG = 0> constexpr int lr_ncp() { return 16 * NC + 4 * NG + 1; }
-template <typename T, int NB, int NC, int NG = 0> inline size_t lr_lds_bytes(unsigned threads, int Kh) {
-    return ((size_t)2 * Kh + (size_t)(threads / 64) * 16 * NB * lr_ncp<NB, NC, NG>()) * sizeof(T);
-}
-
-template <typename T, int NB, int ST, int NC, bool RES, int NG = 0>
+template <typename T, int NB, int NC, int NG = 0> inline size_t lr_lds_bytes(unsigned threads, int Kh, int ne = 1) {
+    return ((size_t)2 * Kh * ne + (size_t)(threads / 64) * 16 * NB * lr_ncp<NB, NC, NG>()) * sizeof(T);
+}
+
+
+template <typename T, int NB, int ST, int NC, bool RES, int NG = 0, bool QUAD = false>
 __global__ void __launch_bounds__((ST > 5 ? 256 : 1024 / NB), (ST <= 10 ? 2 : 1)) k_layer1_lr(LrArgs<T> A) {
     typedef typename Acc4<T>::type acc_t;
     static_assert(NG == 0 || sizeof(T) == 8, "column groups: float64 only");
+    static_assert(!QUAD || (RES && NB == 4 && ST <= 5 && 16 * ST <= NB * lr_ncp<NB, NC, NG>()), "quad form: residual instances of the 64-feature x <= 5-tile wave tile");
     constexpr int NCP = lr_ncp<NB, NC, NG>(), LDW = 16 * (NC + (NG > 0 ? 1 : 0));
     int tile = blockIdx.x, w = blockIdx.y;
     if ((gridDim.y & 7) == 0) {
@@ -616,23 +619,31 @@
         tile = q % gridDim.x;
     }
     const int wave = __builtin_amdgcn_readfirstlane(threadIdx.x >> 6), lane = threadIdx.x & 63;
-    int zb = 0;
-    if (gridDim.x > (unsigned)A.n_tiles) {
+    int zb = 0, quad = 0;
+    if constexpr (QUAD) {
+        const int nfb = gridDim.x / (A.n_tiles / 4);
+        zb = tile % nfb;
+        quad = tile / nfb;
+        tile = 4 * quad + wave;
+    } else if (gridDim.x > (unsigned)A.n_tiles) {
         const int gzf = gridDim.x / A.n_tiles;
         zb = tile % gzf;
         tile /= gzf;
     }
-    const int lr = lane & 15, lq = lane >> 4, n0 = (zb * (blockDim.x >> 6) + wave) * 16 * NB;
+    const int lr = lane & 15, lq = lane >> 4, n0 = QUAD ? zb * 16 * NB : (zb * (blockDim.x >> 6) + wave) * 16 * NB;
     const int P = A.P, Nout = A.Nout, Kh = A.Kh, K0 = A.K0loc + A.K0sh;
+    constexpr int NE = QUAD ? 4 : 1;
     extern __shared__ __attribute__((aligned(16))) char lr_smem[];
-    T* yl = reinterpret_cast<T*>(lr_smem);
-    T* Cl = yl + 2 * Kh + (size_t)wave * (16 * NB * NCP);
+    T* yl0 = reinterpret_cast<T*>(lr_smem);
+    T* Cl0 = yl0 + 2 * Kh * NE;
+    T* yl = yl0 + (QUAD ? (size_t)wave * 2 * Kh : 0);
+    T* Cl = Cl0 + (size_t)wave * (16 * NB * NCP);
     const T* G1t = A.G1 + (size_t)w * A.g_ws + (size_t)tile * A.g_ts;
     {
         typedef T vec2 __attribute__((ext_vector_type(2)));
-        const T* yo = A.YO + (size_t)w * A.yo_ws + (size_t)tile * 2 * Kh;
-        for (int n = threadIdx.x; n < Kh; n += blockDim.x)
-            *reinterpret_cast<vec2*>(yl + 2 * n) = *reinterpret_cast<const vec2*>(yo + 2 * n);
+        const T* yo = A.YO + (size_t)w * A.yo_ws + (size_t)(QUAD ? 4 * quad : tile) * 2 * Kh;
+        for (int n = threadIdx.x; n < NE * Kh; n += blockDim.x)
+            *reinterpret_cast<vec2*>(yl0 + 2 * n) = *reinterpret_cast<const vec2*>(yo + 2 * n);
     }
     __syncthreads();
     if (n0 >= Nout) return;
@@ -858,11 +869,36 @@
 #pragma unroll
                     for (int s = 0; s < CWMAX; ++s)
                         if (s < cw) {
-                            T hv = d1 * racc[s][r];
-                            if (c0 + s == 0) hv = lr == 0 ? yo[0] : (lr == 1 ? yo[1] : hv);
-                            __builtin_nontemporal_store((hv + acc[a][c0 + s][r]) * rs2, &Got[(size_t)n * P + 16 * (c0 + s)]);
+                            T o;
+                            if (c0 + s == 0) {
+                                T hv = d1 * racc[s][r];
+                                hv = lr == 0 ? yo[0] : (lr == 1 ? yo[1] : hv);
+                                o = (hv + acc[a][c0 + s][r]) * rs2;
+                            } else
+                                o = fma(d1, racc[s][r], acc[a][c0 + s][r]) * rs2;
+                            __builtin_nontemporal_store(o, &Got[(size_t)n * P + 16 * (c0 + s)]);
+                            if constexpr (QUAD) acc[a][c0 + s][r] = o;
                         }
                 }
+            }
+            if (QUAD && A.QS != nullptr) {
+#pragma unroll
+                for (int r = 0; r < 4; ++r)
+#pragma unroll
+                    for (int s = 0; s < ST; ++s) Cl[(r * ST + s) * 64 + lane] = acc[a][s][r];
+                __syncthreads();
+                T* Qp = A.QS + (size_t)w * A.qs_ws + (size_t)quad * A.qs_ts + lr;
+#pragma unroll
+                for (int i = 0; i < (4 * ST + 3) / 4; ++i) {
+                    const int rs = 4 * i + wave;
+                    if (rs < 4 * ST) {
+                        const int r = rs / ST, s = rs - r * ST;
+                        const T* cp = Cl0 + rs * 64 + lane;
+                        const T sum = ((cp[0] + cp[16 * NB * NCP]) + cp[2 * 16 * NB * NCP]) + cp[3 * 16 * NB * NCP];
+                        Qp[(size_t)(n0 + 16 * a + acc_row<T>(lane, r)) * P + 16 * s] = sum;
+                    }
+                }
+                __syncthreads();
             }
         };
         layer_epilogue<T, NB, ST, 2, 0>(acc, (const T*)nullptr, Got, (const T*)nullptr, n0, lane, P, rf);
@@ -1043,10 +1079,20 @@
     W0T[idx] = c < K0loc ? Wloc0[(size_t)c * Kh + n] : (c < K0loc + K0sh ? Wsh0[(size_t)(c - K0loc) * Kh + n] : T(0));
 }
 
+template <typename T> struct MeanSrc {
+    int first[2], count[2];
+    T scale[2];
+};
+template <typename T> inline MeanSrc<T> mean_src_electrons(const SysDev<T>& S) {
+    return MeanSrc<T>{{0, S.n_up}, {S.n_up, S.n_dn}, {T(1) / T(S.n_up), S.n_dn > 0 ? T(1) / T(S.n_dn) : T(0)}};
+}
+template <typename T> inline MeanSrc<T> mean_src_quads(const SysDev<T>& S) {
+    return MeanSrc<T>{{0, S.n_up / 4}, {S.n_up / 4, S.n_dn / 4}, {T(1) / T(S.n_up), S.n_dn > 0 ? T(1) / T(S.n_dn) : T(0)}};
+}
 template <typename T, int NB, int ST>
 __global__ void __launch_bounds__((ST > 10 ? 512 : 1024 / NB), (NB == 4 ? 2 : 1))
 k_shared_term(SysDev<T> S, const T* __restrict__ G, const T* __restrict__ Wsh, int Kh, T* __restrict__ Sb, int Nout, int P,
-              const T* __restrict__ bias, int bias_all_slots) {
+              const T* __restrict__ bias, int bias_all_slots, MeanSrc<T> M) {
     typedef typename Acc4<T>::type acc_t;
     constexpr int KC = 16;
     extern __shared__ __attribute__((aligned(32))) char smem_raw[];
@@ -1063,8 +1109,8 @@
         for (int s = 0; s < ST; ++s) acc[a][s] = acc_t{0, 0, 0, 0};
     auto fill = [&](int c, T* dst) {
         const int sp = (c * KC) / Kh, k0 = (c * KC) % Kh;
-        const int i0 = sp == 0 ? 0 : S.n_up, ns = sp == 0 ? S.n_up : S.n_dn;
-        const T inv = T(1) / T(ns);
+        const int i0 = M.first[sp], ns = M.count[sp];
+        const T inv = M.scale[sp];
         const T* g0 = Gw + ((size_t)i0 * S.ldk + k0) * P;
         typedef T vec4 __attribute__((ext_vector_type(4)));
         for (int e = tid; e < KC * P / 4; e += nthr) {
@@ -1074,11 +1120,43 @@
             *reinterpret_cast<vec4*>(dst + 4 * e) = v * inv;
         }
     };
+    constexpr int NPRE = 3;
+    typedef T pvec4 __attribute__((ext_vector_type(4)));
+    constexpr bool PRE = sizeof(T) == 8 && NB == 4 && ST == 5;
+    const bool pre = PRE && M.count[0] <= NPRE && M.count[1] <= NPRE && KC * P <= 5 * nthr;
+    pvec4 pv[NPRE];
+    T pr[NPRE];
+    const int er = 4 * nthr + tid;
+    auto fill_load = [&](int c) {
+        const int sp = (c * KC) / Kh, k0 = (c * KC) % Kh;
+        const int ns = M.count[sp];
+        const T* g0 = Gw + ((size_t)M.first[sp] * S.ldk + k0) * P;
+#pragma unroll
+        for (int i = 0; i < NPRE; ++i)
+            if (i < ns) {
+                if (4 * tid < KC * P) pv[i] = *reinterpret_cast<const pvec4*>(g0 + (size_t)i * S.ldk * P + 4 * tid);
+                if (er < KC * P) pr[i] = g0[(size_t)i * S.ldk * P + er];
+            }
+    };
+    auto fill_store = [&](int c, T* dst) {
+        const int sp = (c * KC) / Kh, ns = M.count[sp];
+        const T inv = M.scale[sp];
+        pvec4 v = {0, 0, 0, 0};
+        T r = 0;
+#pragma unroll
+        for (int i = 0; i < NPRE; ++i)
+            if (i < ns) { v += pv[i]; r += pr[i]; }
+        if (4 * tid < KC * P) *reinterpret_cast<pvec4*>(dst + 4 * tid) = v * inv;
+        if (er < KC * P) dst[er] = r * inv;
+    };
     fill(0, mbuf);
     __syncthreads();
     for (int c = 0; c < nchunk; ++c) {
         const T* cur = mbuf + (c & 1) * KC * P;
-        if (c + 1 < nchunk) fill(c + 1, mbuf + ((c + 1) & 1) * KC * P);
+        if (c + 1 < nchunk) {
+            if constexpr (PRE) { if (pre) fill_load(c + 1); else fill(c + 1, mbuf + ((c + 1) & 1) * KC * P); }
+            else fill(c + 1, mbuf + ((c + 1) & 1) * KC * P);
+        }
         if (active) {
             const T* Wp = Wsh + (size_t)(c * KC + lq) * Nout + n0 + lr;
 #pragma unroll
@@ -1094,6 +1172,7 @@
                     for (int s = 0; s < ST; ++s) acc[a][s] = mfma16(av[a], bv[s], acc[a][s]);
             }
         }
+        if constexpr (PRE) { if (pre && c + 1 < nchunk) fill_store(c + 1, mbuf + ((c + 1) & 1) * KC * P); }
         __syncthreads();
     }
     if (!active) return;
diff --git a/deepsolid_amd/csrc/ds_host.h b/deepsolid_amd/csrc/ds_host.h
--- a/deepsolid_amd/csrc/ds_host.h
+++ b/deepsolid_amd/csrc/ds_host.h
@@ -64,6 +64,11 @@
     bool use_pair_expand = true;
     bool use_pm_skip = true;
     bool use_lr = true;
+    bool use_quad = true;
+    bool quad_sums = true;
+    int32_t last_kinds[DS_MAX_LAYERS] = {0};
+    int32_t last_n_layers = 0;
+    bool last_quad = false;
     void* lr_w0t = nullptr;
     int64_t val_i8_min_tiles = 512;
     bool use_i8_val = true;
@@ -121,7 +126,12 @@
 
 template <typename T> struct Carve {
     T *G[2], *MEAN[2], *ZB, *H2[2], *Q, *MOUT, *MINV, *DETS, *TR, *XL, *YO;
-};
+    T* QS;
+};
+inline size_t quad_sums_extent(const ds::SysDev<double>& S, size_t g_per_walker, int64_t Bc) {
+    if (S.n_layers < 3 || S.N < 4 || Bc < 1) return 0;
+    return (size_t)(Bc - 1) * g_per_walker + (size_t)(S.N / 4 - 1) * S.ldk * S.P + (size_t)S.h1[2] * S.P;
+}
 template <typename T> Carve<T> carve(const ds_system* s, Arena<T>& a, int64_t Bc) {
     const WsLayout& w = s->ws;
     Carve<T> c;
@@ -133,6 +143,9 @@
     c.MOUT = a.take(w.MOUT * Bc); c.MINV = a.take(w.MINV * Bc);
     c.DETS = a.take(w.DETS * Bc); c.TR = a.take(w.TR * Bc);
     c.XL = a.take(w.XL * Bc); c.YO = a.take(w.YO * Bc);
+    c.QS = nullptr;
+    if (const size_t n = quad_sums_extent(s->sd, w.G, Bc); n > 0 && s->sd.h1[2] <= s->sd.h1[1])
+        a.part(c.G[1], w.G * Bc, [&](Arena<T>& g) { c.QS = g.take(n); });
     return c;
 }
 
diff --git a/deepsolid_amd/csrc/ds_tiles.h b/deepsolid_amd/csrc/ds_tiles.h
--- a/deepsolid_amd/csrc/ds_tiles.h
+++ b/deepsolid_amd/csrc/ds_tiles.h
@@ -15,8 +15,9 @@
     void (*gemm)(int epi, dim3 grid, dim3 block, hipStream_t st, const GemmArgs<T>& a);
     void (*gemm_orb3)(dim3 grid, dim3 block, hipStream_t st, const GemmArgs<T>& a);
     void (*shared_term)(dim3 grid, dim3 block, size_t lds, hipStream_t st, const SysDev<T>& S, const T* G, const T* Wsh, int Kh, T* Sb,
-                        int Nout, int P, const T* bias, int bias_all_slots);
-    void (*layer1_lr)(int nc, bool res, dim3 grid, dim3 block, hipStream_t st, const LrArgs<T>& a);
+                        int Nout, int P, const T* bias, int bias_all_slots, const MeanSrc<T>& M);
+    void (*layer1_lr)(int nc, bool res, bool quad, dim3 grid, dim3 block, hipStream_t st, const LrArgs<T>& a);
+    size_t (*layer1_lr_quad_lds)(int nc, bool res, const LrArgs<T>& a);
     void (*layer0_stats)(int nks, dim3 grid, hipStream_t st, const SysDev<T>& S, const T* XL, size_t xl_ws, size_t xl_ts, const T* W0,
                          const T* S0, int Nout, int P, T* YO, T* MEAN1);
     void (*gemm_wide)(int epi, dim3 grid, dim3 block, hipStream_t st, const GemmArgs<T>& a);
diff --git a/deepsolid_amd/csrc/ds_tiles_inst.hip b/deepsolid_amd/csrc/ds_tiles_inst.hip
--- a/deepsolid_amd/csrc/ds_tiles_inst.hip
+++ b/deepsolid_amd/csrc/ds_tiles_inst.hip
@@ -76,10 +76,31 @@
                                a.zws, a.zts, a.Nout, a.P, a.Sb, a.bias, a.oe);
     }
     static void shared_term(dim3 grid, dim3 block, size_t lds, hipStream_t st, const SysDev<T>& S, const T* G, const T* Wsh, int Kh, T* Sb,
-                            int Nout, int P, const T* bias, int bias_all_slots) {
-        hipLaunchKernelGGL((k_shared_term<T, NB, ST>), grid, block, lds, st, S, G, Wsh, Kh, Sb, Nout, P, bias, bias_all_slots);
+                            int Nout, int P, const T* bias, int bias_all_slots, const MeanSrc<T>& M) {
+        hipLaunchKernelGGL((k_shared_term<T, NB, ST>), grid, block, lds, st, S, G, Wsh, Kh, Sb, Nout, P, bias, bias_all_slots, M);
     }
-    static void layer1_lr(int nc, bool res, dim3 grid, dim3 block, hipStream_t st, const LrArgs<T>& a) {
+    static constexpr bool HAS_QUAD = sizeof(T) == 8 && NB == 4 && ST <= 5;
+    static size_t layer1_lr_quad(bool launch, int nc, bool res, dim3 grid, hipStream_t st, const LrArgs<T>& a) {
+        if constexpr (HAS_QUAD) {
+            if (!res) return 0;
+            size_t lds = 0;
+#define DS_LRQ(NCV, NGV) do { lds = lr_lds_bytes<T, NB, NCV, NGV>(256, a.Kh, 4); \
+                              if (launch) hipLaunchKernelGGL((k_layer1_lr<T, NB, ST, NCV, true, NGV, true>), grid, dim3(256), lds, st, a); } while (0)
+            const int rem = a.K0loc + a.K0sh + 4 - 16 * (nc - 1);
+            if (nc >= 2 && nc <= 3 && (rem == 4 || rem == 8)) {
+                if (nc == 2) { if (rem == 4) DS_LRQ(1, 1); else DS_LRQ(1, 2); }
+                else { if (rem == 4) DS_LRQ(2, 1); else DS_LRQ(2, 2); }
+            } else if (nc <= 2) DS_LRQ(2, 0);
+            else if constexpr (ST < 5) { if (nc == 3) DS_LRQ(3, 0); else DS_LRQ(4, 0); }
+            else return 0;
+#undef DS_LRQ
+            return lds;
+        }
+        return 0;
+    }
+    static size_t layer1_lr_quad_lds(int nc, bool res, const LrArgs<T>& a) { return layer1_lr_quad(false, nc, res, dim3(), nullptr, a); }
+    static void layer1_lr(int nc, bool res, bool quad, dim3 grid, dim3 block, hipStream_t st, const LrArgs<T>& a) {
+        if (quad) { layer1_lr_quad(true, nc, res, grid, st, a); return; }
         if constexpr (sizeof(T) == 8 && ST <= 10) {
             const int rem = a.K0loc + a.K0sh + 4 - 16 * (nc - 1);
             if (nc >= 2 && nc <= 3 && (rem == 4 || rem == 8)) {
@@ -136,7 +157,7 @@
                                a.zts, a.Nout, a.P, a.Sb, a.oe);
     }
     static const TileOps<T>* ops() {
-        static const TileOps<T> o = {NB, ST, &gemm, (ST <= 5 ? &gemm_orb3 : nullptr), &shared_term, &layer1_lr, (ST <= 5 ? &layer0_stats : nullptr),
+        static const TileOps<T> o = {NB, ST, &gemm, (ST <= 5 ? &gemm_orb3 : nullptr), &shared_term, &layer1_lr, &layer1_lr_quad_lds, (ST <= 5 ? &layer0_stats : nullptr),
                                       (ST > 10 ? &gemm_wide : nullptr), (ST > 10 ? &layer1_lr_wide : nullptr),
                                       ((ST > 10 && sizeof(T) == 4) ? &orbital_lb : nullptr)};
         return &o;
diff --git a/deepsolid_amd/csrc/ds_value.hip b/deepsolid_amd/csrc/ds_value.hip
--- a/deepsolid_amd/csrc/ds_value.hip
+++ b/deepsolid_amd/csrc/ds_value.hip
@@ -154,7 +154,7 @@
         T* Sorb = vb.SORB[sp];
         if (s->use_last)
             hipLaunchKernelGGL((ds::k_shared_term<T, 4, 5>), dim3(1, (unsigned)ng, ogz), oblock, 2 * 16 * PV * sizeof(T), st, S, Gl,
-                               blk(s->i_wsh_orb[sp]), Kl, Sorb, OC, PV, (const T*)nullptr, 0);
+                               blk(s->i_wsh_orb[sp]), Kl, Sorb, OC, PV, (const T*)nullptr, 0, ds::mean_src_electrons<T>(S));
         if (vb.keep) {
             launch_gemm_plain<T>(dim3(ns, (unsigned)ng, ogz), oblock, st, Gl + (size_t)i0 * S.ldk * PV,
                                gws, gts, blk(s->i_worb[sp]), Korb, (const T*)nullptr, (size_t)0, (const T*)nullptr, 0, ns, vb.PHI[sp], (size_t)ns * OC * PV, (size_t)0,
diff --git a/deepsolid_amd/device.py b/deepsolid_amd/device.py
--- a/deepsolid_amd/device.py
+++ b/deepsolid_amd/device.py
@@ -614,6 +614,16 @@
     def int8_layers(self):
         return int(self.lib.ds_int8_layers(self.handle))
 
+    CHAIN_KINDS = ('dense', 'dense_res', 'l0_stats', 'l0_epi9_means', 'lowrank1', 'int8')
+
+    def chain_plan(self):
+        kinds = (C.c_int32 * 16)()
+        quad = C.c_int32(0)
+        n = int(self.lib.ds_debug_chain_plan(self.handle, kinds, 16, C.byref(quad)))
+        if n <= 0:
+            return None
+        return dict(kinds=[self.CHAIN_KINDS[kinds[l]] for l in range(min(n, 16))], quad=bool(quad.value))
+
     def profile_clock(self):
         cyc, ticks = C.c_double(0), C.c_double(0)
         _lib.check(self.lib.ds_profile_read_clock(self.handle, C.byref(cyc), C.byref(ticks)), 'ds_profile_read_clock')
diff --git a/include/deepsolid_hip.h b/include/deepsolid_hip.h
--- a/include/deepsolid_hip.h
+++ b/include/deepsolid_hip.h
@@ -64,6 +64,8 @@
 
 int ds_int8_layers(const ds_system* sys);
 
+int ds_debug_chain_plan(const ds_system* sys, int32_t* kinds, int32_t max_layers, int32_t* quad);
+
 int64_t ds_param_count(const ds_system* sys);
 int ds_param_layout(const ds_system* sys, ds_param_block* blocks, int max_blocks);
 
```

New measurement: 68090 local-energy evals/s (median of 6 runs). About the same (+0.8%).
